# xxayt/MGSV

Measured on AMD Instinct MI355X. Metric: video-music pairs/s fwd+bwd at B=64 (full training step); sub-objects: retrieval sim-matrix GB/s, eval forward pairs/s, higher is better.
Workload: dtype bf16; 1 GPU; BASELINE.json configs[2]: B=64/GPU, T_v=30, T_a=512, D=512, train mode (dropout on), f32 master weights + Adam, f32 gradient accumulation; global_batch=64, launch=tape

## Files before the change

include/made_hip.h:

```cpp
#ifndef MADE_HIP_H
#define MADE_HIP_H

#include <stdint.h>

#ifdef __cplusplus
extern "C" {
#endif

#define MADE_ABI_VERSION 8

enum MadeDtype { MADE_F32 = 0, MADE_BF16 = 1 };

enum MadeAct {
    MADE_ACT_NONE = 0,
    MADE_ACT_RELU = 1,
    MADE_ACT_GELU = 2,
    MADE_ACT_QUICKGELU = 3,
    MADE_ACT_SIGMOID = 4
};

enum MadeGate {
    MADE_GATE_NONE = 0,
    MADE_GATE_RELU_OUT = 1,
    MADE_GATE_GELU_Z = 2,
// ... 425 lines not shown
                       float* dgamma, float* dbeta, int64_t rows, int64_t D, float eps, const float* row_skip, void* stream);

int made_pool_bwd(const float* mean, const float* dvec, const float* mask,
                  const void* in1, int32_t in1_dtype, int64_t in1_bs, int64_t in1_ld,
                  const void* in2, int32_t in2_dtype, int64_t in2_bs, int64_t in2_ld,
                  void* out, int32_t out_dtype, int64_t out_bs, int64_t out_ld,
                  int64_t B, int64_t T, int64_t D, float eps, void* stream);

int made_l2norm_bwd(const void* x, int32_t x_dtype, int64_t ldx, const float* dy, int64_t lddy, int64_t dy_rows_per,
                    float* dx, int64_t lddx, int32_t accumulate, void* dx_alt, int32_t alt_dtype, int64_t lddxa,
                    int64_t rows, int64_t D, float eps, void* stream);

int made_clip_loss_bwd(const float* sims, int64_t ld, int64_t n, const float* logit_scale, float weight,
                       const float* upstream, float* lse_ws, float* dsims, float* dsims_t, int32_t accumulate,
                       float* d_logit_scale, const float* row_exclude, void* stream);

int made_xpool_tail_bwd(const void* y, int32_t y_dtype, int64_t ldy, const float* gamma, const float* beta,
                        const float* video, int64_t ld_video, const float* dsims, int64_t ld_dsims,
                        void* dy, int32_t dy_dtype, int64_t lddy, void* dy_drop, const MadeDropout* drop,
                        float* dgamma, float* dbeta, float* dvideo, int64_t ld_dvideo,
                        const float* dpool, int64_t ld_dpool, float dpool_scale,
                        int64_t Nm, int64_t Nv, int64_t D, float eps, void* stream);

int made_softmax_bwd(const float* S, int64_t ld_s, const float* dP, int64_t ld_dp, const float* mask, int64_t rows_per_mask,
                     const float* extra, float scale, const MadeDropout* drop,
                     void* Pd, void* dS, void* dSt, int32_t out_dtype, int64_t ldo, int64_t ldt,
                     int64_t out_batch_stride, int64_t t_batch_stride,
                     int64_t rows, int64_t rows_per_batch, int64_t L, void* stream);

int made_head_bias(void* x, int32_t x_dtype, int64_t ldx, const float* s, const float* bias, int64_t rows, int64_t H, int64_t hd,
                   void* stream);
int made_head_bias_bwd(const void* dy, int32_t dtype, int64_t ld, const float* s, const float* bias, float* dbias, float* ds,
                       int64_t rows, int64_t H, int64_t hd, void* stream);

int made_layernorm_bwd2(const void* xa, const float* gamma_a, int64_t ldxa, const void* xb, const float* gamma_b, int64_t ldxb,
                        const void* dy, int64_t lddy, const void* add, int64_t ld_add, void* dx, int64_t lddx,
                        void* dx_drop, int64_t lddxd, const MadeDropout* drop, int64_t drop_ld, int32_t dtype,
                        float* dgamma_a, float* dbeta_a, float* dgamma_b, float* dbeta_b, int64_t rows, int64_t D, float eps,
                        void* stream);

int made_gate_rows(const void* x, int32_t x_dtype, int64_t ldx, const void* G, int32_t g_dtype, int64_t ldg, int32_t gate,
                   float scale, const MadeDropout* drop, int64_t drop_ld, int64_t drop_col_div, void* out, int32_t out_dtype, int64_t ldo,
                   const float* row_skip, int64_t rows, int64_t cols, void* stream);
int made_add3(void* out, int32_t out_dtype, const void* a, int32_t a_dtype, const void* b, int32_t b_dtype,
              const void* c, int32_t c_dtype, int64_t n, int64_t b_mod, void* stream);
int made_colsum(const void* x, int32_t dtype, int64_t ld, int64_t rows, int64_t cols, float* out, void* stream);

int made_posbn_relu_fwd(const void* x, int32_t x_dtype, int64_t ldx, const float* weight, const float* bias,
                        float* running_mean, float* running_var, float momentum, float eps, int32_t batch_stats,
                        float* save_mean, float* save_rstd, void* y, int32_t y_dtype, int64_t ldy,
                        int64_t B, int64_t T, int64_t F, void* stream);
int made_posbn_relu_bwd(const void* x, int32_t x_dtype, int64_t ldx, const void* y, int32_t y_dtype, int64_t ldy,
                        const void* dy, int32_t dy_dtype, int64_t lddy, const float* weight, const float* save_mean,
                        const float* save_rstd, int32_t batch_stats, void* dx, int32_t dx_dtype, int64_t lddx,
                        float* dweight, float* dbias, int64_t B, int64_t T, int64_t F, void* stream);

int made_set_criterion_bwd(const float* pred_logits, const float* pred_spans, const float* targets,
                           const int64_t* pred_idx, const int64_t* tgt_idx, const int32_t* count,
                           const float* proj_queries, const float* vid_sum, const float* empty_weight,
                           int64_t n_layers, int64_t B, int64_t Q, int64_t G, int64_t Dc, int32_t fg_label,
                           float temperature, const float* weights, const float* upstream,
                           float* d_logits, float* d_spans, int64_t ld_out, int32_t through_sigmoid,
                           float* d_proj_queries, float* d_vid_sum, void* stream);

#define MADE_ADAM_MAX_GROUPS 4
#define MADE_ADAM_NORM_BLOCKS 1024
typedef struct MadeAdamGroup { int64_t begin, end; float lr; float max_norm; } MadeAdamGroup;
int made_adam_step(float* param, const float* grad, float* exp_avg, float* exp_avg_sq, int64_t n,
                   const MadeAdamGroup* groups, int32_t n_groups, float beta1, float beta2, float eps, int64_t step,
                   float grad_scale, float* norm_ws, void* stream);

typedef struct MadeAdamDeviceState { int64_t step; float lr[MADE_ADAM_MAX_GROUPS]; float bc1, bc2_sqrt; } MadeAdamDeviceState;
int made_adam_step_device(float* param, const float* grad, float* exp_avg, float* exp_avg_sq, int64_t n,
                          const MadeAdamGroup* groups, int32_t n_groups, float beta1, float beta2, float eps,
                          MadeAdamDeviceState* state_device, int32_t advance_state, float grad_scale, float* norm_ws, void* stream);

typedef struct MadeRepackDesc {
    const float* src; void* w; void* wt;
    int64_t rows, cols, wt_ld, tile_begin;
    int32_t dtype; int32_t _pad;
} MadeRepackDesc;
int made_repack(const MadeRepackDesc* descs_device, int32_t n_desc, int64_t total_tiles, void* stream);


int made_recall_ranks(const float* sims, int64_t ld, const int32_t* group_id, const int32_t* gt_group, int64_t Nv, int64_t Nm,
                      int64_t n_groups, int32_t* rank_out, int32_t* top1_out, void* stream);

int made_span_iou(const float* pred_logits, const float* pred_spans, const float* gt_moment, const float* m_duration,
                  int64_t N, int64_t Q, int32_t fg_label, float max_m_duration, float* iou_out, float* pred_out, void* stream);

int made_concat_cols(const float* a, int64_t cols_a, const float* c, int64_t cols_c, float* out, int64_t rows, void* stream);


int made_pooled_cosine(const float* anchor, int64_t lda, const void* pooled, int32_t pooled_dtype, float* out, int64_t sa, int64_t sp,
                       int64_t A, int64_t P, int64_t D, void* stream);
int made_scale_exp(const float* x, const float* logit_scale, float* out, int64_t n, void* stream);
int made_span_convert(const float* in, float* out, int64_t N, int32_t mode, void* stream);
int made_span_pairwise(const float* spans1, const float* spans2, float* iou, float* uni, float* giou, float* inter_over_2,
                       int64_t N, int64_t M, void* stream);
int made_span_iou_se(const float* pred_se, const float* gt_moment, const float* m_duration, int64_t N, float max_m_duration,
                     int32_t clamp_to_max, int32_t discounted, float* iou_out, void* stream);


int64_t made_topk_groups_ws_bytes(int64_t Nv, int64_t Nm, int64_t K);
int made_topk_groups(const float* sims, int64_t ld, const int32_t* group_id, int64_t Nv, int64_t Nm, int64_t n_groups,
                     int64_t K, int32_t* idx_out, float* score_out, void* ws, int64_t ws_bytes, void* stream);

int made_gather_pairs(const int32_t* vi, const int32_t* mi, int64_t P, int64_t Nv, int64_t Nm,
                      const void* v_tok, int64_t v_tok_stride, const float* v_mask, int64_t v_mask_stride,
                      const float* v_vec, int64_t v_vec_stride,
                      const void* m_tok, int64_t m_tok_stride, const float* m_mask, int64_t m_mask_stride,
                      const float* m_vec, int64_t m_vec_stride, int64_t Tv, int64_t Ta, int64_t D, int32_t dtype,
                      void* frame_out, int64_t frame_out_stride, void* seg_out, int64_t seg_out_stride,
                      float* fmask_out, float* smask_out, float* video_out, float* music_out, void* stream);


#define MADE_FRAMES_MAX (1 << 20)

typedef struct MadeFrameDesc {
    int64_t offset;
    int64_t coef;
    int32_t H, W;
    int32_t kh, kv;
} MadeFrameDesc;

int made_frames_preprocess(const uint8_t* frames, int64_t frames_bytes, const MadeFrameDesc* desc, int64_t n_frames,
                           const int32_t* coef, int64_t n_coef, void* patches, int32_t patch_dtype, int64_t ld_patch,
                           uint8_t* crop_out, void* stream);


#define MADE_AUDIO_TRACKS_MAX (1 << 16)
#define MADE_AUDIO_SEGS_MAX (1 << 20)
#define MADE_RESAMPLE_TILE 1024
#define MADE_RESAMPLE_SLAB 12288
#define MADE_AUDIO_ROWS 1024
#define MADE_AUDIO_MELS 128

typedef struct MadeResampleDesc {
    int64_t offset;
    int64_t n;
    int64_t taps;
    int32_t o, m;
    int32_t width;
    int32_t _pad;
} MadeResampleDesc;

int made_audio_resample(const float* pcm, int64_t pcm_len, const MadeResampleDesc* desc, int64_t n_tracks, const float* taps,
                        int64_t n_taps, float* out, int64_t out_len, void* stream);

typedef struct MadeAudioSegDesc {
    int64_t first;
    int64_t count;
} MadeAudioSegDesc;

int made_audio_fbank(const float* pcm, int64_t pcm_len, const MadeAudioSegDesc* segs, int64_t n_segs, const float* window,
                     const float* twiddle, const float* mel, int32_t mel_ld, float* spec, void* stream);

int made_ast_patches(const float* spec, int64_t n_segs, void* patches, int32_t patch_dtype, int64_t ld_patch, void* stream);

#ifdef __cplusplus
}
#endif
#endif
```

mgsv_amd/_lib.py:

```python
from __future__ import annotations

import ctypes as C
import os

_HERE = os.path.dirname(os.path.abspath(__file__))


def variant_env(name: str, default: str = "") -> str:
    if os.environ.get("MADE_DEBUG_VARIANTS", "0") in ("", "0"):
        return default
    return os.environ.get(name, default)


LIB_PATH = os.environ.get("MADE_LIB_PATH") or os.path.join(_HERE, "libmade_hip.so")
ABI_VERSION = 8

F32, BF16 = 0, 1
ACT_NONE, ACT_RELU, ACT_GELU, ACT_QUICKGELU, ACT_SIGMOID = 0, 1, 2, 3, 4
GATE_NONE, GATE_RELU_OUT, GATE_GELU_Z, GATE_QUICKGELU_Z, GATE_SIGMOID_OUT = 0, 1, 2, 3, 4

vp, i64, i32, f32 = C.c_void_p, C.c_int64, C.c_int32, C.c_float

WIDE_PLAN_HEAD, WIDE_PLAN_SAMPLE, WIDE_PLAN_SLOT, WIDE_PLAN_SLOT_BITS = 4, 4, 16, 8

# ... 80 lines not shown
                ("B", i64), ("H", i64), ("Lq", i64), ("Lk", i64),
                ("q_bs", i64), ("ldq", i64), ("k_bs", i64), ("ldk", i64), ("v_bs", i64), ("ldv", i64), ("o_bs", i64), ("ldo", i64),
                ("do_bs", i64), ("lddo", i64), ("dq_bs", i64), ("lddq", i64), ("dk_bs", i64), ("lddk", i64), ("dv_bs", i64), ("lddv", i64),
                ("key_mask", vp), ("q_skip_mask", vp), ("scale", f32), ("_pad", i32), ("drop", MadeDropout),
                ("batch_order", vp), ("keep_bits", vp), ("ld_bits", i64)]


class MadeXpoolFusedArgs(C.Structure):
    _fields_ = [("Q", vp), ("ldq", i64), ("K", vp), ("U", vp), ("k_bs", i64), ("ldk", i64), ("u_bs", i64), ("ldu", i64),
                ("key_mask", vp), ("ln2_g", vp), ("ln2_b", vp), ("Wl", vp), ("ldw", i64), ("bl", vp), ("ln3_g", vp), ("ln3_b", vp),
                ("vn", vp), ("ldvn", i64), ("sims", vp), ("ld_sims", i64),
                ("Nv", i64), ("Nm", i64), ("S", i64), ("D", i64), ("scale", f32), ("eps", f32), ("ws", vp), ("prepare_ws", i32), ("_pad", i32)]


class MadeXpoolAttnArgs(C.Structure):
    _fields_ = [("Q", vp), ("ldq", i64), ("K", vp), ("U", vp), ("k_bs", i64), ("ldk", i64), ("u_bs", i64), ("ldu", i64),
                ("key_mask", vp), ("out", vp), ("ldo", i64), ("Nv", i64), ("Nm", i64), ("S", i64), ("D", i64),
                ("scale", f32), ("eps", f32), ("normalize", i32), ("_pad", i32), ("ws", vp)]


class MadeXpoolSimsArgs(C.Structure):
    _fields_ = [("Q", vp), ("ldq", i64), ("K", vp), ("UU", vp), ("k_bs", i64), ("ldk", i64), ("u_bs", i64), ("ldu", i64),
                ("key_mask", vp), ("av", vp), ("bv", vp), ("ln3_g", vp), ("ln3_b", vp), ("vn", vp), ("ldvn", i64),
                ("sims", vp), ("ld_sims", i64), ("Nv", i64), ("Nm", i64), ("S", i64), ("D", i64),
                ("scale", f32), ("eps", f32), ("ws", vp), ("prepare_ws", i32), ("_pad", i32)]


class MadeXpoolInbatchArgs(C.Structure):
    _fields_ = [("Q", vp), ("ldq", i64), ("K", vp), ("U", vp), ("k_bs", i64), ("ldk", i64), ("u_bs", i64), ("ldu", i64),
                ("key_mask", vp), ("out", vp), ("out_dtype", i32), ("_pad", i32), ("o_bs", i64), ("ldo", i64),
                ("Nv", i64), ("Nm", i64), ("S", i64), ("D", i64), ("scale", f32), ("_pad2", i32), ("ws", vp)]


class MadeWideAttnArgs(C.Structure):
    _fields_ = [("Q", vp), ("K", vp), ("Kadd", vp), ("V", vp), ("O", vp), ("key_mask", vp),
                ("dtype", i32), ("o_dtype", i32),
                ("B", i64), ("NQ1", i64), ("NQ2", i64), ("L", i64), ("D", i64),
                ("q_bs", i64), ("q_s1", i64), ("q_s2", i64), ("k_bs", i64), ("ldk", i64), ("kadd_bs", i64), ("ldkadd", i64),
                ("v_bs", i64), ("ldv", i64), ("o_bs", i64), ("o_s1", i64), ("o_s2", i64),
                ("scale", f32), ("_pad", i32),
                ("n_split", i64), ("part_o", vp), ("part_ml", vp), ("drop", MadeDropout), ("sum_out", vp),
                ("lse_out", vp)]


class MadeWideAttnBwdArgs(C.Structure):
    _fields_ = ([(k, vp) for k in ("Q", "dO", "O", "K", "V", "key_mask", "lse", "ssum", "extra", "dattc")] + [("ld_dattc", i64), ("vbias", vp), ("hd", i64),
                ("Pd", vp), ("dS", vp), ("p_bs", i64), ("ld_p", i64), ("dQ", vp), ("dq_bs", i64), ("ld_dq", i64)] +
                [(k, i64) for k in ("B", "NQ", "L", "D", "q_bs", "ld_q", "do_bs", "ld_do", "o_bs", "ld_o", "k_bs", "ldk", "v_bs", "ldv")] +
                [("scale", f32), ("_pad", i32), ("n_split", i64), ("part_dq", vp), ("drop", MadeDropout)])


class MadeGemmTNArgs(C.Structure):
    _fields_ = [("A", vp), ("B", vp), ("C", vp), ("ab_dtype", i32), ("c_dtype", i32),
                ("M", i64), ("N", i64), ("K", i64), ("lda", i64), ("ldb", i64), ("ldc", i64),
                ("batch1", i64), ("batch2", i64),
                ("a_zs1", i64), ("a_zs2", i64), ("b_zs1", i64), ("b_zs2", i64), ("c_zs1", i64), ("c_zs2", i64),
                ("row_mask", vp), ("mask_zs1", i64), ("mask_zs2", i64),
                ("alpha", f32), ("accumulate", i32), ("split_m", i64),
                ("colsum", vp), ("colsum_zs1", i64), ("colsum_zs2", i64), ("row_group_valid", vp),
                ("row_index", vp), ("n_rows", vp)]


class MadeGemmTNProblem(C.Structure):
    _fields_ = [("A", vp), ("B", vp), ("C", vp), ("colsum", vp), ("N", i64), ("K", i64), ("lda", i64), ("ldb", i64), ("ldc", i64)]


class MadeGemmTNGroup(C.Structure):
    _fields_ = [("n_problems", i32), ("alpha", f32), ("M", i64), ("split_m", i64), ("row_index", vp), ("n_rows", vp),
                ("p", MadeGemmTNProblem * 8), ("tile_end", i32 * 8), ("tile_size", i32), ("_pad", i32),
                ("workspace", vp), ("workspace_bytes", i64)]


class MadeAdamGroup(C.Structure):
    _fields_ = [("begin", i64), ("end", i64), ("lr", f32), ("max_norm", f32)]


class MadeAdamDeviceState(C.Structure):
    _fields_ = [("step", i64), ("lr", f32 * 4), ("bc1", f32), ("bc2_sqrt", f32)]


class MadeRepackDesc(C.Structure):
    _fields_ = [("src", vp), ("w", vp), ("wt", vp), ("rows", i64), ("cols", i64), ("wt_ld", i64), ("tile_begin", i64),
                ("dtype", i32), ("_pad", i32)]


class MadeFrameDesc(C.Structure):
    _fields_ = [("offset", i64), ("coef", i64), ("H", i32), ("W", i32), ("kh", i32), ("kv", i32)]


class MadeResampleDesc(C.Structure):
    _fields_ = [("offset", i64), ("n", i64), ("taps", i64), ("o", i32), ("m", i32), ("width", i32), ("_pad", i32)]


class MadeAudioSegDesc(C.Structure):
    _fields_ = [("first", i64), ("count", i64)]


SIGNATURES = {
    "made_abi_version": (C.c_int, []),
    "made_set_f32_products": (C.c_int, [C.c_int]),
    "made_get_f32_products": (C.c_int, []),
    "made_last_error": (C.c_char_p, []),
    "made_device_info": (C.c_int, [C.c_char_p, C.c_int, C.POINTER(C.c_int), C.POINTER(C.c_int)]),
    "made_tape_begin": (C.c_int, []),
    "made_tape_end": (C.c_int, [C.POINTER(C.c_uint64)]),
    "made_tape_replay": (C.c_int, [C.c_uint64]),
    "made_tape_free": (C.c_int, [C.c_uint64]),
    "made_tape_interleave": (C.c_int, [C.c_uint64, i32]),
    "made_tape_count": (C.c_int, [C.c_uint64, C.POINTER(i64), C.POINTER(i64), C.POINTER(i64)]),
    "made_tape_replay_range": (C.c_int, [C.c_uint64, i64, i64]),
    "made_tape_op": (C.c_int, [C.c_uint64, i64, C.POINTER(i32), C.POINTER(C.c_uint64), C.POINTER(C.c_uint64), C.POINTER(C.c_uint32)]),
    "made_stream_wait": (C.c_int, [vp, vp]),
    "made_tape_event": (C.c_int, [i32, i32, vp]),
    "made_tape_callback": (C.c_int, [C.CFUNCTYPE(C.c_int, vp), vp]),
    "made_memset_async": (C.c_int, [vp, i32, i64, vp]),
    "made_copy_async": (C.c_int, [vp, vp, i64, vp]),
    "made_store_words": (C.c_int, [vp, vp, i32, vp]),
    "made_linear": (C.c_int, [C.POINTER(MadeLinearArgs), vp]),
    "made_splitk_finish": (C.c_int, [C.POINTER(MadeFinishArgs), vp]),
    "made_dec_stage": (C.c_int, [C.POINTER(MadeDecStageArgs), vp]),
    "made_dec_stage_bwd": (C.c_int, [C.POINTER(MadeDecStageBwdArgs), vp]),
    "made_attention": (C.c_int, [C.POINTER(MadeAttnArgs), vp]),
    "made_attention_wide": (C.c_int, [C.POINTER(MadeWideAttnArgs), vp]),
    "made_attention_wide_bwd": (C.c_int, [C.POINTER(MadeWideAttnBwdArgs), vp]),
    "made_wide_slice_plan": (C.c_int, [vp, i64, i64, i32, i32, vp, vp, i64, vp]),
    "made_attention_wide_planned": (C.c_int, [C.POINTER(MadeWideAttnArgs), vp, i32, vp]),
    "made_attention_wide_bwd_planned": (C.c_int, [C.POINTER(MadeWideAttnBwdArgs), vp, i32, vp]),
    "made_layernorm": (C.c_int, [vp, i32, i64, i64, i64, vp, vp, vp, i32, i64, i64, i64, f32, vp, vp]),
    "made_layernorm_add": (C.c_int, [vp, i32, i64, vp, vp, vp, i32, i64, vp, i32, i64, vp, i64, i64, i64, f32, vp, vp]),
    "made_cast_mask_rows": (C.c_int, [vp, i64, vp, vp, i32, i64, i64, i64, vp]),
    "made_pack_music_records": (C.c_int, [vp, i32, i64, vp, i64, vp, i64, vp, i32, i64, i64, i64, i64, i64, vp]),
    "made_masked_mean": (C.c_int, [vp, i32, i64, i64, vp, vp, i64, i64, i64, vp]),
    "made_l2norm_rows": (C.c_int, [vp, i32, i64, vp, vp, i32, i64, i64, i64, f32, vp]),
    "made_sine_pe": (C.c_int, [vp, vp, vp, i32, i64, i64, i64, vp]),
    "made_masked_softmax": (C.c_int, [vp, i64, vp, i64, vp, i32, i64, i64, i64, i64, i64, f32, vp]),
    "made_xpool_tail": (C.c_int, [vp, i32, i64, vp, vp, vp, i64, vp, vp, i64, i64, i64, i64, f32, vp]),
    "made_clip_loss": (C.c_int, [vp, i64, i64, vp, f32, i32, vp, vp, vp]),
    "made_hungarian_match": (C.c_int, [vp, vp, vp, i64, i64, i64, i64, i32, f32, f32, f32, vp, i32, vp, vp, vp, vp, vp]),
    "made_attention_bwd": (C.c_int, [C.POINTER(MadeAttnBwdArgs), vp]),
    "made_layernorm_bwd": (C.c_int, [vp, i32, i64, i64, i64, vp, vp, i32, i64, vp, i32, i64, vp, i32, i64, vp, i64,
                                     C.POINTER(MadeDropout), i64, vp, vp, i64, i64, f32, vp, vp]),
    "made_layernorm_bwd2": (C.c_int, [vp, vp, i64, vp, vp, i64, vp, i64, vp, i64, vp, i64, vp, i64, C.POINTER(MadeDropout), i64, i32,
                                      vp, vp, vp, vp, i64, i64, f32, vp]),
    "made_pool_bwd": (C.c_int, [vp, vp, vp, vp, i32, i64, i64, vp, i32, i64, i64, vp, i32, i64, i64, i64, i64, i64, f32, vp]),
    "made_l2norm_bwd": (C.c_int, [vp, i32, i64, vp, i64, i64, vp, i64, i32, vp, i32, i64, i64, i64, f32, vp]),
    "made_clip_loss_bwd": (C.c_int, [vp, i64, i64, vp, f32, vp, vp, vp, vp, i32, vp, vp, vp]),
    "made_xpool_tail_bwd": (C.c_int, [vp, i32, i64, vp, vp, vp, i64, vp, i64, vp, i32, i64, vp, C.POINTER(MadeDropout),
                                      vp, vp, vp, i64, vp, i64, f32, i64, i64, i64, f32, vp]),
    "made_softmax_bwd": (C.c_int, [vp, i64, vp, i64, vp, i64, vp, f32, C.POINTER(MadeDropout), vp, vp, vp, i32, i64, i64,
                                   i64, i64, i64, i64, i64, vp]),
    "made_head_bias": (C.c_int, [vp, i32, i64, vp, vp, i64, i64, i64, vp]),
    "made_head_bias_bwd": (C.c_int, [vp, i32, i64, vp, vp, vp, vp, i64, i64, i64, vp]),
    "made_add3": (C.c_int, [vp, i32, vp, i32, vp, i32, vp, i32, i64, i64, vp]),
    "made_colsum": (C.c_int, [vp, i32, i64, i64, i64, vp, vp]),
    "made_posbn_relu_fwd": (C.c_int, [vp, i32, i64, vp, vp, vp, vp, C.c_float, C.c_float, i32, vp, vp, vp, i32, i64, i64, i64, i64, vp]),
    "made_posbn_relu_bwd": (C.c_int, [vp, i32, i64, vp, i32, i64, vp, i32, i64, vp, vp, vp, i32, vp, i32, i64, vp, vp, i64, i64, i64, vp]),
    "made_set_criterion_bwd": (C.c_int, [vp, vp, vp, vp, vp, vp, vp, vp, vp, i64, i64, i64, i64, i64, i32, f32, vp, vp,
                                         vp, vp, i64, i32, vp, vp, vp]),
    "made_adam_step": (C.c_int, [vp, vp, vp, vp, i64, C.POINTER(MadeAdamGroup), i32, f32, f32, f32, i64, f32, vp, vp]),
    "made_adam_step_device": (C.c_int, [vp, vp, vp, vp, i64, C.POINTER(MadeAdamGroup), i32, f32, f32, f32, vp, i32, f32, vp, vp]),
    "made_repack": (C.c_int, [vp, i32, i64, vp]),
    "made_row_groups": (C.c_int, [vp, i64, vp, vp]),
    "made_row_index": (C.c_int, [vp, i64, vp, vp, vp]),
    "made_linear_variant": (C.c_int, [C.POINTER(MadeLinearArgs)]),
    "made_row_affine": (C.c_int, [vp, i32, i64, vp, vp, i64, i32, vp, i32, i64, i64, i64, vp]),
    "made_gate_rows": (C.c_int, [vp, i32, i64, vp, i32, i64, i32, f32, vp, i64, i64, vp, i32, i64, vp, i64, i64, vp]),
    "made_xpool_fused": (C.c_int, [C.POINTER(MadeXpoolFusedArgs), vp]),
    "made_xpool_attention": (C.c_int, [C.POINTER(MadeXpoolAttnArgs), vp]),
    "made_xpool_sims": (C.c_int, [C.POINTER(MadeXpoolSimsArgs), vp]),
    "made_xpool_sims_ws_bytes": (C.c_int64, [i64, i64, i64]),
    "made_xpool_inbatch": (C.c_int, [C.POINTER(MadeXpoolInbatchArgs), vp]),
    "made_xpool_inbatch_ws_bytes": (C.c_int64, [i64, i64]),
    "made_batch_order": (C.c_int, [vp, i64, i64, vp, vp]),
    "made_recall_ranks": (C.c_int, [vp, i64, vp, vp, i64, i64, i64, vp, vp, vp]),
    "made_span_iou": (C.c_int, [vp, vp, vp, vp, i64, i64, i32, f32, vp, vp, vp]),
    "made_gemm_tn": (C.c_int, [C.POINTER(MadeGemmTNArgs), vp]),
    "made_gemm_tn_grouped": (C.c_int, [C.POINTER(MadeGemmTNGroup), vp]),
    "made_gemm_tn_grouped_workspace": (i64, [C.POINTER(MadeGemmTNGroup)]),
    "made_concat_cols": (C.c_int, [vp, i64, vp, i64, vp, i64, vp]),
    "made_pooled_cosine": (C.c_int, [vp, i64, vp, i32, vp, i64, i64, i64, i64, i64, vp]),
    "made_scale_exp": (C.c_int, [vp, vp, vp, i64, vp]),
    "made_span_convert": (C.c_int, [vp, vp, i64, i32, vp]),
    "made_span_pairwise": (C.c_int, [vp, vp, vp, vp, vp, vp, i64, i64, vp]),
    "made_span_iou_se": (C.c_int, [vp, vp, vp, i64, f32, i32, i32, vp, vp]),
    "made_set_criterion": (C.c_int, [vp, vp, vp, vp, vp, vp, vp, vp, vp, i64, i64, i64, i64, i64, i32, f32, vp, vp, vp, vp]),
    "made_topk_groups_ws_bytes": (C.c_int64, [i64, i64, i64]),
    "made_topk_groups": (C.c_int, [vp, i64, vp, i64, i64, i64, i64, vp, vp, vp, i64, vp]),
    "made_gather_pairs": (C.c_int, [vp, vp, i64, i64, i64, vp, i64, vp, i64, vp, i64, vp, i64, vp, i64, vp, i64, i64, i64, i64, i32,
                                    vp, i64, vp, i64, vp, vp, vp, vp, vp]),
    "made_frames_preprocess": (C.c_int, [vp, i64, vp, i64, vp, i64, vp, i32, i64, vp, vp]),
    "made_audio_resample": (C.c_int, [vp, i64, vp, i64, vp, i64, vp, i64, vp]),
    "made_audio_fbank": (C.c_int, [vp, i64, vp, i64, vp, vp, vp, i32, vp, vp]),
    "made_ast_patches": (C.c_int, [vp, i64, vp, i32, i64, vp]),
}

_lib = None


class MadeError(RuntimeError):
    pass


def lib() -> C.CDLL:
    global _lib
    if _lib is None:
        if not os.path.isfile(LIB_PATH):
            raise MadeError(f"{LIB_PATH} not found: build the HIP library first (make -C mgsv_amd/csrc); "
                            "the MaDe hot path has no CPU fallback")
        l = C.CDLL(LIB_PATH)
        for name, (res, args) in SIGNATURES.items():
            fn = getattr(l, name)
            fn.restype = res
            fn.argtypes = args
        if l.made_abi_version() != ABI_VERSION:
            raise MadeError(f"ABI version mismatch: {LIB_PATH} is version {l.made_abi_version()}, this binding was written for {ABI_VERSION} "
                            "(rebuild: make -C mgsv_amd/csrc)")
        _lib = l
    return _lib


def check(status: int, what: str = "") -> None:
    if status != 0:
        msg = lib().made_last_error().decode("utf-8", "replace")
        raise MadeError(f"{what or 'libmade_hip'} failed (status {status}): {msg}")


def device_info():
    l = lib()
    name = C.create_string_buffer(64)
    cu, is950 = C.c_int(0), C.c_int(0)
    check(l.made_device_info(name, 64, C.byref(cu), C.byref(is950)), "made_device_info")
    return name.value.decode(), cu.value, bool(is950.value)
```

mgsv_amd/csrc/attention_wide.hip:

```cpp
#include "common.h"

#include <type_traits>

namespace {

constexpr int WQ = 32;
constexpr int WKEY = 32;
constexpr int NTHREADS = 256;

template <typename TC> struct Frag;
template <> struct Frag<float>  { typedef f32x4  type; };
template <> struct Frag<bf16_t> { typedef bf16x8 type; };


template <typename TC, int D, bool DB, int NSL, bool X3 = false, bool PLAN = false>
__global__ __launch_bounds__(NTHREADS) void attention_wide_kernel(const MadeWideAttnArgs a, const int32_t* __restrict__ plan) {
    static_assert(!PLAN || (DB && sizeof(TC) == 2 && NSL == 4 && !X3), "the planned launch: LDS-DMA variant, one query tile");
    typedef typename Frag<TC>::type frag_t;
    constexpr int SZ = (int)sizeof(TC);
    constexpr bool IS_BF16 = SZ == 2;
    constexpr int PER16 = 16 / SZ;
    constexpr int DS = D / NSL;
    constexpr int WQB = WQ * (4 / NSL);
    constexpr bool DMA = IS_BF16 && DB;
    constexpr int K_ROW = DMA ? D * SZ : D * SZ + 16;
    constexpr int V_ROW = DMA ? D * SZ : D * SZ + (IS_BF16 ? 64 : 16);
    constexpr int CPR = D * SZ / 16;
    constexpr int NCH = WKEY * CPR / NTHREADS;
    static_assert(WKEY * CPR % NTHREADS == 0, "staging split");
    constexpr int NQF = DS * SZ / 32;
    constexpr int NDT = DS / 32;
    constexpr int KV_STAGE = WKEY * K_ROW + WKEY * V_ROW;
    constexpr int NSTAGE = DB ? 2 : 1;

    extern __shared__ __attribute__((aligned(16))) unsigned char lds[];
    float* lds_s = (float*)(lds + NSTAGE * KV_STAGE);
    float* lds_bias_all = lds_s + 4 * 1024;
    uint32_t* lds_mbits = (uint32_t*)(lds_bias_all + NSTAGE * 32);

    const int tid = threadIdx.x, lane = tid & 63, wave = tid >> 6;
    const int r = lane & 31, hh = lane >> 5;
    const int sl = wave % NSL, qt = wave / NSL;
    int32_t pl[MADE_WIDE_PLAN_SLOT] = {};
    if constexpr (PLAN) {
        const u32x4* sp = (const u32x4*)(plan + MADE_WIDE_PLAN_HEAD + MADE_WIDE_PLAN_SAMPLE * a.B + (int64_t)MADE_WIDE_PLAN_SLOT * blockIdx.x);
#pragma unroll
        for (int i = 0; i < 4; ++i) {
            const u32x4 v = sp[i];
            pl[4 * i] = (int32_t)v[0]; pl[4 * i + 1] = (int32_t)v[1]; pl[4 * i + 2] = (int32_t)v[2]; pl[4 * i + 3] = (int32_t)v[3];
        }
        if (pl[0] < 0 || pl[0] >= a.B || pl[3] < 0 || pl[3] >= a.n_split || pl[1] < 0 || pl[2] < 0 || (int64_t)(pl[1] + pl[2]) * WKEY >= a.L + WKEY ||
            pl[4] < 0 || pl[4] >= a.L) return;
    }
    const bool batch_fast = gridDim.x == (unsigned)a.B && (a.NQ1 * a.NQ2 + WQB - 1) / WQB != (int64_t)a.B;
    const int64_t b = PLAN ? (int64_t)pl[0] : (batch_fast ? blockIdx.x : blockIdx.y);
    const int64_t nq_total = a.NQ1 * a.NQ2;
    const int64_t nq0 = PLAN ? (int64_t)qt * WQ : (int64_t)(batch_fast ? blockIdx.y : blockIdx.x) * WQB + qt * WQ;

    const TC* Kg = (const TC*)a.K + b * a.k_bs;
    const TC* Ag = a.Kadd ? (const TC*)a.Kadd + b * a.kadd_bs : nullptr;
    const TC* Vg = (const TC*)a.V + b * a.v_bs;
    const float* maskg = a.key_mask ? a.key_mask + b * a.L : nullptr;

    frag_t qf[NQF];
    int64_t my_q = nq0 + r;
    {
        int64_t q = my_q < nq_total ? my_q : nq_total - 1;
        const TC* qp = (const TC*)a.Q + b * a.q_bs + (q / a.NQ2) * a.q_s1 + (q % a.NQ2) * a.q_s2 + sl * DS;
#pragma unroll
        for (int ks = 0; ks < NQF; ++ks) qf[ks] = *(const frag_t*)(qp + ks * 2 * PER16 + hh * PER16);
    }

    frag_t rk[NCH], rv[NCH];
    int64_t rkey0 = 0;
    auto load_tile = [&](int64_t key0) __attribute__((always_inline)) {
        rkey0 = key0;
#pragma unroll
        for (int i = 0; i < NCH; ++i) {
            int c = tid + i * NTHREADS;
            int row = c / CPR, cc = c % CPR;
            int64_t key = key0 + row;
            const int64_t kcl = key < a.L ? key : a.L - 1;
            rk[i] = *(const frag_t*)(Kg + kcl * a.ldk + cc * PER16);
// ... 366 lines not shown
#pragma unroll
                    for (int j = 0; j < 4; ++j) acc[i][j] += t[sp][i][j] * w;
            }
        }
    } else {
        float M = -INFINITY;
        for (int64_t s = 0; s < ns; ++s) M = fmaxf(M, a.part_ml[((b * ns + s) * nq_total + q) * 4]);
        Muse = (M == -INFINITY) ? 0.f : M;
        for (int64_t s = 0; s < ns; ++s) {
            const int64_t prow = (b * ns + s) * nq_total + q;
            const float w = expf(a.part_ml[prow * 4] - Muse);
            Lsum += a.part_ml[prow * 4 + 1] * w;
            Dsum += a.part_ml[prow * 4 + 2] * w;
#pragma unroll
            for (int i = 0; i < 2; ++i) {
                int c = (i * 64 + lane) * 4;
                if (c < D) {
                    f32x4 tt = *(const f32x4*)(a.part_o + prow * D + c);
#pragma unroll
                    for (int j = 0; j < 4; ++j) acc[i][j] += tt[j] * w;
                }
            }
        }
    }
    const float inv = 1.f / Lsum;
    if (a.sum_out && lane == 0) a.sum_out[b * nq_total + q] = Dsum * inv;
    if (a.lse_out && lane == 0) a.lse_out[b * nq_total + q] = Muse + logf(Lsum);
    const int64_t obase = b * a.o_bs + (q / a.NQ2) * a.o_s1 + (q % a.NQ2) * a.o_s2;
#pragma unroll
    for (int i = 0; i < 2; ++i) {
        int c = (i * 64 + lane) * 4;
        if (c < D) {
            if (a.o_dtype == MADE_F32) {
                f32x4 pk; pk[0] = acc[i][0] * inv; pk[1] = acc[i][1] * inv; pk[2] = acc[i][2] * inv; pk[3] = acc[i][3] * inv;
                *(f32x4*)((float*)a.O + obase + c) = pk;
            } else {
                bf16x4 pk; pk[0] = (bf16_t)(acc[i][0] * inv); pk[1] = (bf16_t)(acc[i][1] * inv);
                pk[2] = (bf16_t)(acc[i][2] * inv); pk[3] = (bf16_t)(acc[i][3] * inv);
                *(bf16x4*)((bf16_t*)a.O + obase + c) = pk;
            }
        }
    }
}

template <typename TC, int D, bool DB, int NSL>
int launch_wide(const MadeWideAttnArgs& a, hipStream_t st) {
    constexpr int SZ = (int)sizeof(TC);
    constexpr bool DMA = SZ == 2 && DB;
    constexpr int K_ROW = DMA ? D * SZ : D * SZ + 16, V_ROW = DMA ? D * SZ : D * SZ + (SZ == 2 ? 64 : 16);
    constexpr int NSTAGE = DB ? 2 : 1;
    constexpr size_t kBase = (size_t)NSTAGE * (WKEY * K_ROW + WKEY * V_ROW) + 4 * 1024 * 4 + NSTAGE * 32 * 4;
    constexpr size_t kCap = kBase + 8192 < 160 * 1024 ? kBase + 8192 : 160 * 1024;
    const size_t lds_bytes = kBase + (size_t)((a.L + 63) / 64 * 2 + 2) * 4;
    if (lds_bytes > kCap) {
        made_set_error("made_attention_wide: L=%lld keys: the mask bit row does not fit in LDS beside the K / V stages", (long long)a.L);
        return MADE_ERR_UNSUPPORTED;
    }
    static bool attr_done = false;
    if (!attr_done) {
        hipError_t e = hipFuncSetAttribute((const void*)attention_wide_kernel<TC, D, DB, NSL>, hipFuncAttributeMaxDynamicSharedMemorySize, (int)kCap);
        if (e == hipSuccess && SZ == 4)
            e = hipFuncSetAttribute((const void*)attention_wide_kernel<TC, D, DB, NSL, SZ == 4>, hipFuncAttributeMaxDynamicSharedMemorySize, (int)kCap);
        if (e != hipSuccess) {
            made_set_error("made_attention_wide: cannot reserve %zu bytes of LDS: %s", kCap, hipGetErrorString(e));
            return MADE_ERR_HIP;
        }
        attr_done = true;
    }
    const int64_t nq = a.NQ1 * a.NQ2;
    const int64_t nsplit = a.n_split > 1 ? a.n_split : 1;
    constexpr int WQB = WQ * (4 / NSL);
    const int64_t qtiles = (nq + WQB - 1) / WQB;
    const bool batch_fast = qtiles > 1 && qtiles <= 8 && qtiles != a.B;
    dim3 grid((unsigned)(batch_fast ? a.B : qtiles), (unsigned)(batch_fast ? qtiles : a.B), (unsigned)nsplit), block(NTHREADS);
    if (SZ == 4 && g_made_f32_products) hipLaunchKernelGGL((attention_wide_kernel<TC, D, DB, NSL, SZ == 4>), grid, block, lds_bytes, st, a, (const int32_t*)nullptr);
    else hipLaunchKernelGGL((attention_wide_kernel<TC, D, DB, NSL>), grid, block, lds_bytes, st, a, (const int32_t*)nullptr);
    int rc = made_check_launch("made_attention_wide");
    if (rc != MADE_OK || nsplit == 1) return rc;
    const int64_t rows = a.B * nq;
    hipLaunchKernelGGL(attention_wide_combine_kernel, dim3((unsigned)((rows + 3) / 4)), dim3(NTHREADS), 0, st, a);
    return made_check_launch("made_attention_wide(combine)");
}

constexpr int PLAN_T = 1024;
__global__ __launch_bounds__(PLAN_T) void wide_slice_plan_kernel(const float* __restrict__ mask, int B, int L, int n_slots, int max_slices,
                                                                 const int32_t* __restrict__ order, int32_t* __restrict__ plan) {
    __shared__ int32_t s_tiles[PLAN_T], s_first[PLAN_T], s_ord[PLAN_T];
    __shared__ int32_t s_cap;
    extern __shared__ __attribute__((aligned(16))) unsigned char lds[];
    uint32_t* s_bits = (uint32_t*)lds;
    const int tid = threadIdx.x, lane = tid & 63, wave = tid >> 6;
    const int nch = (L + 63) / 64, wpr = 2 * nch;
    if (tid == 0) s_cap = 0x7fffffff;
    for (int b = wave; b < B; b += PLAN_T / 64) {
        const float* m = mask + (int64_t)b * L;
        int last = -1, first = -1;
        for (int c0 = 0; c0 < nch; c0 += 8) {
            float v[8];
#pragma unroll
            for (int j = 0; j < 8; ++j) {
                const int i = (c0 + j) * 64 + lane;
                v[j] = m[i < L ? i : L - 1];
            }
#pragma unroll
            for (int j = 0; j < 8; ++j) {
                const int i = (c0 + j) * 64 + lane;
                const unsigned long long bal = __ballot(i < L && v[j] != 0.f);
                if (c0 + j < nch) {
                    if (lane == 0) { s_bits[b * wpr + 2 * (c0 + j)] = (uint32_t)bal; s_bits[b * wpr + 2 * (c0 + j) + 1] = (uint32_t)(bal >> 32); }
                    if (bal) {
                        last = (c0 + j) * 64 + 63 - __clzll(bal);
                        if (first < 0) first = (c0 + j) * 64 + __ffsll(bal) - 1;
                    }
                }
            }
        }
        if (lane == 0) { s_tiles[b] = (last + 1 + 31) / 32; s_first[b] = first < 0 ? 0 : first; }
    }
    if (tid < B) {
        const int o = order ? order[tid] : tid;
        s_ord[tid] = o >= 0 && o < B ? o : tid;
    }
    __syncthreads();
    int tmax = 1;
    for (int b = 0; b < B; ++b) tmax = max(tmax, s_tiles[b]);
    for (int c = tid + 1; c <= tmax; c += PLAN_T) {
        const int n = made_wide_slice_count(s_tiles, 1, B, c, max_slices);
        if (n >= 0 && n <= n_slots) atomicMin(&s_cap, c);
    }
    __syncthreads();
    const int cap = s_cap <= tmax ? s_cap : tmax;
    int used = 0;
    for (int r = 0; r < B; ++r) { const int t = s_tiles[s_ord[r]]; used += t > cap ? (t + cap - 1) / cap : 1; }
    if (tid == 0) { plan[0] = cap; plan[1] = used; plan[2] = n_slots; plan[3] = max_slices; }
    int32_t* slots = plan + MADE_WIDE_PLAN_HEAD + MADE_WIDE_PLAN_SAMPLE * B;
    if (tid < B) {
        int slot0 = 0;
        for (int r = 0; r < tid; ++r) { const int t = s_tiles[s_ord[r]]; slot0 += t > cap ? (t + cap - 1) / cap : 1; }
        const int b = s_ord[tid], t = s_tiles[b], fv = s_first[b];
        const int n = t > cap ? (t + cap - 1) / cap : 1;
        int32_t* sm = plan + MADE_WIDE_PLAN_HEAD + MADE_WIDE_PLAN_SAMPLE * b;
        sm[0] = t; sm[1] = slot0; sm[2] = n; sm[3] = fv;
        for (int s = 0; s < n && slot0 + s < n_slots; ++s) {
            int32_t* sp = slots + (int64_t)MADE_WIDE_PLAN_SLOT * (slot0 + s);
            const int t0 = made_wide_slice_first(t, n, s), tn = made_wide_slice_len(t, n, s);
            sp[0] = b; sp[1] = t0; sp[2] = tn; sp[3] = s; sp[4] = fv; sp[5] = n; sp[6] = t; sp[7] = 0;
            for (int i = 0; i < MADE_WIDE_PLAN_SLOT_BITS; ++i) sp[8 + i] = i < tn ? (int32_t)s_bits[b * wpr + t0 + i] : 0;
        }
    }
    for (int w = used + tid; w < n_slots; w += PLAN_T) {
        int32_t* sp = slots + (int64_t)MADE_WIDE_PLAN_SLOT * w;
        sp[0] = -1;
        for (int i = 1; i < MADE_WIDE_PLAN_SLOT; ++i) sp[i] = 0;
    }
}

__global__ __launch_bounds__(NTHREADS) void attention_wide_combine_planned_kernel(const MadeWideAttnArgs a, const int32_t* __restrict__ plan) {
    constexpr int MAXS = 8;
    const int lane = threadIdx.x & 63;
    const int64_t nq_total = a.NQ1 * a.NQ2;
    const int64_t row = (int64_t)blockIdx.x * (NTHREADS / 64) + (threadIdx.x >> 6);
    if (row >= a.B * nq_total) return;
    const int64_t b = row / nq_total, q = row % nq_total;
    const int D = (int)a.D;
    const int cap = (int)a.n_split;
    int ns = plan[MADE_WIDE_PLAN_HEAD + MADE_WIDE_PLAN_SAMPLE * b + 2];
    ns = ns < 1 ? 1 : (ns > MAXS ? MAXS : ns);
    ns = ns > cap ? cap : ns;
    float Lsum = 0.f, Dsum = 0.f;
    f32x4 acc[2];
#pragma unroll
    for (int i = 0; i < 2; ++i) { acc[i][0] = acc[i][1] = acc[i][2] = acc[i][3] = 0.f; }
    f32x4 t[MAXS][2];
    float ml[MAXS][3];
#pragma unroll
    for (int sp = 0; sp < MAXS; ++sp) {
        const int64_t pr = (b * cap + (sp < ns ? sp : ns - 1)) * nq_total + q;
        ml[sp][0] = a.part_ml[pr * 4]; ml[sp][1] = a.part_ml[pr * 4 + 1]; ml[sp][2] = a.part_ml[pr * 4 + 2];
#pragma unroll
        for (int i = 0; i < 2; ++i) {
            const int c = (i * 64 + lane) * 4;
            t[sp][i] = *(const f32x4*)(a.part_o + pr * D + (c < D ? c : 0));
        }
    }
    float M = -INFINITY;
#pragma unroll
    for (int sp = 0; sp < MAXS; ++sp) if (sp < ns) M = fmaxf(M, ml[sp][0]);
    const float Muse = (M == -INFINITY) ? 0.f : M;
#pragma unroll
    for (int sp = 0; sp < MAXS; ++sp) {
        if (sp < ns) {
            const float w = expf(ml[sp][0] - Muse);
            Lsum += ml[sp][1] * w;
            Dsum += ml[sp][2] * w;
#pragma unroll
            for (int i = 0; i < 2; ++i)
#pragma unroll
                for (int j = 0; j < 4; ++j) acc[i][j] += t[sp][i][j] * w;
        }
    }
    const float inv = 1.f / Lsum;
    if (a.sum_out && lane == 0) a.sum_out[b * nq_total + q] = Dsum * inv;
    if (a.lse_out && lane == 0) a.lse_out[b * nq_total + q] = Muse + logf(Lsum);
    const int64_t obase = b * a.o_bs + (q / a.NQ2) * a.o_s1 + (q % a.NQ2) * a.o_s2;
#pragma unroll
    for (int i = 0; i < 2; ++i) {
        int c = (i * 64 + lane) * 4;
        if (c < D) {
            if (a.o_dtype == MADE_F32) {
                f32x4 pk; pk[0] = acc[i][0] * inv; pk[1] = acc[i][1] * inv; pk[2] = acc[i][2] * inv; pk[3] = acc[i][3] * inv;
                *(f32x4*)((float*)a.O + obase + c) = pk;
            } else {
                bf16x4 pk; pk[0] = (bf16_t)(acc[i][0] * inv); pk[1] = (bf16_t)(acc[i][1] * inv);
                pk[2] = (bf16_t)(acc[i][2] * inv); pk[3] = (bf16_t)(acc[i][3] * inv);
                *(bf16x4*)((bf16_t*)a.O + obase + c) = pk;
            }
        }
    }
}

template <int D>
int launch_wide_planned(const MadeWideAttnArgs& a, const int32_t* plan, int n_slots, hipStream_t st) {
    constexpr size_t kBase = (size_t)2 * (WKEY * D * 2 + WKEY * D * 2) + 4 * 1024 * 4 + 2 * 32 * 4;
    constexpr size_t kCap = kBase + 8192 < 160 * 1024 ? kBase + 8192 : 160 * 1024;
    const size_t lds_bytes = kBase + (size_t)((a.L + 63) / 64 * 2 + 2) * 4;
    if (lds_bytes > kCap) {
        made_set_error("made_attention_wide_planned: L=%lld keys: the mask bit row does not fit in LDS beside the K / V stages", (long long)a.L);
        return MADE_ERR_UNSUPPORTED;
    }
    static bool attr_done = false;
    if (!attr_done) {
        hipError_t e = hipFuncSetAttribute((const void*)attention_wide_kernel<bf16_t, D, true, 4, false, true>, hipFuncAttributeMaxDynamicSharedMemorySize, (int)kCap);
        if (e != hipSuccess) {
            made_set_error("made_attention_wide_planned: cannot reserve %zu bytes of LDS: %s", kCap, hipGetErrorString(e));
            return MADE_ERR_HIP;
        }
        attr_done = true;
// ... 86 lines not shown
```

mgsv_amd/csrc/gemm_tn.hip:

```cpp
#include "common.h"

namespace {

__device__ const float kOne = 1.f;

constexpr int TBN = 128, TBK = 128, TNT = 256;

template <typename TC> struct TnCfg;
template <> struct TnCfg<bf16_t> { static constexpr int BM = 64, ROW = 128 * 2 + 64, CPR = 16; typedef bf16x8 frag_t; };
template <> struct TnCfg<float>  { static constexpr int BM = 32, ROW = 128 * 4 + 128, CPR = 32; typedef f32x4 frag_t; };

template <typename TC, bool X3 = false>
__global__ __launch_bounds__(TNT) void gemm_tn_kernel(const MadeGemmTNArgs a) {
    typedef TnCfg<TC> Cfg;
    typedef typename Cfg::frag_t frag_t;
    constexpr int BM = Cfg::BM, ROW = Cfg::ROW, CPR = Cfg::CPR;
    constexpr int PER16 = 16 / (int)sizeof(TC);
    constexpr int NCH = BM * CPR / TNT;
    constexpr bool IS_BF16 = sizeof(TC) == 2;

    __shared__ __attribute__((aligned(16))) unsigned char lds[2 * BM * ROW];
    unsigned char* lds_a = lds;
    unsigned char* lds_b = lds + BM * ROW;

    const int tid = threadIdx.x, lane = tid & 63, wave = tid >> 6;
    const int r = lane & 31, hh = lane >> 5;
    const int wn = wave >> 1, wk = wave & 1;
    const int tiles_k = (int)((a.K + TBK - 1) / TBK);
    const int tile_n = blockIdx.x / tiles_k, tile_k = blockIdx.x % tiles_k;
    const int64_t n0 = (int64_t)tile_n * TBN, k0 = (int64_t)tile_k * TBK;
    const int64_t z = blockIdx.z, z1 = z / a.batch2, z2 = z % a.batch2;

    const TC* Ag = (const TC*)a.A + z1 * a.a_zs1 + z2 * a.a_zs2;
    const TC* Bg = (const TC*)a.B + z1 * a.b_zs1 + z2 * a.b_zs2;
    const float* maskg = a.row_mask ? a.row_mask + z1 * a.mask_zs1 + z2 * a.mask_zs2 : nullptr;

    int64_t Mv = a.M;
    if (a.n_rows) { const int64_t nv = *a.n_rows; Mv = nv < a.M ? nv : a.M; }
    const int64_t nslab = (Mv + BM - 1) / BM;
    const int64_t sstep = a.split_m;
    const int64_t s_begin = 0;
    const int64_t s_end = nslab > (int64_t)blockIdx.y ? (nslab - blockIdx.y + sstep - 1) / sstep : 0;
    if (s_begin >= s_end) return;
    auto gslab = [&](int64_t i) __attribute__((always_inline)) { return (int64_t)blockIdx.y + i * sstep; };

    uint64_t slab_bits = ~0ull;
    if (a.row_group_valid && (s_end - s_begin) <= 64 && a.batch1 * a.batch2 == 1) {
        const int64_t sl = lane < s_end ? gslab(lane) : nslab;
        bool any = false;
        if (lane < s_end) {
            constexpr int GP = BM / 32;
            const int64_t ngroups = (a.M + 31) / 32;
#pragma unroll
            for (int g = 0; g < GP; ++g) {
                const int64_t gi = sl * GP + g;
                any = any || (gi < ngroups && a.row_group_valid[gi] != 0.f);
            }
        }
        slab_bits = __ballot(any);
    }
    auto slab_live = [&](int64_t i) __attribute__((always_inline)) { return i >= 64 || ((slab_bits >> i) & 1ull) != 0; };

    frag_t ra[NCH], rb[NCH];
    int64_t prow[NCH];
    auto load_rows = [&](int64_t slab) __attribute__((always_inline)) {
#pragma unroll
        for (int i = 0; i < NCH; ++i) {
            const int c = tid + i * TNT;
            const int64_t m = slab * BM + c / CPR;
            const int64_t ml = m < Mv ? m : Mv - 1;
            prow[i] = a.row_index ? (int64_t)a.row_index[ml] : ml;
        }
    };
    float rmk[NCH];
    int64_t rslab = 0;
    const float* mrow = maskg ? maskg : &kOne;
    const int64_t mstride = maskg ? 1 : 0;
    auto load_slab = [&](int64_t slab) __attribute__((always_inline)) {
        rslab = slab;
#pragma unroll
        for (int i = 0; i < NCH; ++i) {
            const int c = tid + i * TNT;
            const int cc = c % CPR;
// ... 157 lines not shown
    }
    if (!active) return;
    const int64_t co = z1 * a.c_zs1 + z2 * a.c_zs2 + n * a.ldc + k;
    if (a.c_dtype == MADE_F32) {
        if (a.accumulate) unsafeAtomicAdd((float*)a.C + co, acc * a.alpha); else ((float*)a.C)[co] = acc * a.alpha;
    } else {
        ((bf16_t*)a.C)[co] = (bf16_t)(acc * a.alpha);
    }
    if (a.colsum && k == 0) unsafeAtomicAdd(a.colsum + z1 * a.colsum_zs1 + z2 * a.colsum_zs2 + n, cs * a.alpha);
}

}

int made_gemm_tn_fast(const MadeGemmTNArgs& a, hipStream_t st);

extern "C" int made_gemm_tn(const MadeGemmTNArgs* args, void* stream) {
    MADE_REQUIRE(args != nullptr, "made_gemm_tn: null args");
    MadeGemmTNArgs a = *args;
    MADE_REQUIRE(a.A && a.B && a.C, "made_gemm_tn: null tensor");
    MADE_REQUIRE(a.M >= 0 && a.N > 0 && a.K > 0, "made_gemm_tn: bad dims");
    MADE_REQUIRE(a.ab_dtype == MADE_F32 || a.ab_dtype == MADE_BF16, "made_gemm_tn: bad operand dtype %d", a.ab_dtype);
    MADE_REQUIRE(a.c_dtype == MADE_F32 || a.c_dtype == a.ab_dtype, "made_gemm_tn: C must be f32 or the operand dtype");
    if (a.batch1 <= 0) a.batch1 = 1;
    if (a.batch2 <= 0) a.batch2 = 1;
    if (a.split_m <= 0) a.split_m = 1;
    const int64_t nz = a.batch1 * a.batch2;
    MADE_REQUIRE(a.split_m == 1 || a.accumulate, "made_gemm_tn: split_m > 1 needs accumulate = 1 (partials are added atomically)");
    MADE_REQUIRE(!a.accumulate || a.c_dtype == MADE_F32, "made_gemm_tn: accumulation needs an f32 C");
    MADE_UNSUPPORTED(nz < 65536 && a.split_m < 65536, "made_gemm_tn: batch / split too large for the grid");
    MADE_REQUIRE(a.row_group_valid == nullptr || a.row_mask != nullptr, "made_gemm_tn: row_group_valid without row_mask");
    MADE_REQUIRE((a.row_index == nullptr) == (a.n_rows == nullptr), "made_gemm_tn: row_index and n_rows come together");
    MADE_UNSUPPORTED(a.row_index == nullptr || nz == 1, "made_gemm_tn: row gather is for unbatched calls");
    if (a.row_index) a.row_group_valid = nullptr;
    if (a.M == 0) return MADE_OK;
    hipStream_t st = (hipStream_t)stream;
    const int per16 = a.ab_dtype == MADE_F32 ? 4 : 8;
    const int64_t n_up = (a.N + per16 - 1) / per16 * per16, k_up = (a.K + per16 - 1) / per16 * per16;
    const bool aligned = a.lda % per16 == 0 && a.ldb % per16 == 0 && n_up <= a.lda && k_up <= a.ldb &&
                         a.a_zs1 % per16 == 0 && a.a_zs2 % per16 == 0 && a.b_zs1 % per16 == 0 && a.b_zs2 % per16 == 0 &&
                         ((uintptr_t)a.A % 16) == 0 && ((uintptr_t)a.B % 16) == 0;
    if (!aligned) {
        MADE_UNSUPPORTED(a.N * a.K <= (1 << 20), "made_gemm_tn: unaligned operands are only supported for small outputs");
        int sy = (int)a.split_m;
        if (!a.accumulate) sy = 1;
        dim3 grid((unsigned)((a.N * a.K + 255) / 256), (unsigned)sy, (unsigned)nz);
        hipLaunchKernelGGL(gemm_tn_small_kernel, grid, dim3(256), 0, st, a);
        return made_check_launch("made_gemm_tn(small)");
    }
    const int64_t tiles = ((a.N + TBN - 1) / TBN) * ((a.K + TBK - 1) / TBK);
    MADE_UNSUPPORTED(tiles < (1LL << 31), "made_gemm_tn: too many tiles");
    {
        const int rc = made_gemm_tn_fast(a, st);
        if (rc != 1) return rc;
    }
    dim3 grid((unsigned)tiles, (unsigned)a.split_m, (unsigned)nz);
    if (a.ab_dtype == MADE_BF16) hipLaunchKernelGGL(gemm_tn_kernel<bf16_t>, grid, dim3(TNT), 0, st, a);
    else if (g_made_f32_products) hipLaunchKernelGGL((gemm_tn_kernel<float, true>), grid, dim3(TNT), 0, st, a);
    else hipLaunchKernelGGL(gemm_tn_kernel<float>, grid, dim3(TNT), 0, st, a);
    return made_check_launch("made_gemm_tn");
}

namespace {
__global__ __launch_bounds__(256) void row_groups_kernel(const float* mask, int64_t M, float* out) {
    const int lane = threadIdx.x & 63;
    const int64_t g = ((int64_t)blockIdx.x * 256 + threadIdx.x) >> 5;
    const int64_t ngroups = (M + 31) / 32;
    const int64_t row = g * 32 + (lane & 31);
    const bool v = g < ngroups && row < M && mask[row] != 0.f;
    const uint64_t bal = __ballot(v);
    const uint32_t half = (lane >> 5) ? (uint32_t)(bal >> 32) : (uint32_t)bal;
    if ((lane & 31) == 0 && g < ngroups) out[g] = half != 0 ? 1.f : 0.f;
}
}

extern "C" int made_row_groups(const float* mask, int64_t M, float* out, void* stream) {
    MADE_REQUIRE(mask && out && M > 0, "made_row_groups: bad arguments");
    const int64_t ngroups = (M + 31) / 32;
    hipLaunchKernelGGL(row_groups_kernel, dim3((unsigned)((ngroups * 32 + 255) / 256)), dim3(256), 0, (hipStream_t)stream, mask, M, out);
    return made_check_launch("made_row_groups");
}

namespace {
__global__ __launch_bounds__(1024) void row_index_kernel(const float* mask, int64_t M, int32_t* row_index, int32_t* n_rows) {
    constexpr int NB = 16;
    __shared__ int wsum[16];
    __shared__ int wlast[16];
    const int lane = threadIdx.x & 63, wave = threadIdx.x >> 6;
    const int64_t per = ((M + 15) / 16 + 63) / 64 * 64;
    const int64_t b = (int64_t)wave * per, e = b + per < M ? b + per : M;
    uint64_t bal[NB];
    auto ballots = [&](int64_t i0) __attribute__((always_inline)) {
        float v[NB];
        const float* p = mask + i0 + lane;
        if (i0 + NB * 64 <= e) {
#pragma unroll
            for (int j = 0; j < NB; ++j) v[j] = p[j * 64];
        } else {
#pragma unroll
            for (int j = 0; j < NB; ++j) v[j] = i0 + j * 64 + lane < e ? p[j * 64] : 0.f;
        }
#pragma unroll
        for (int j = 0; j < NB; ++j) bal[j] = __ballot(v[j] != 0.f);
    };
    int cnt = 0, last = -1;
    for (int64_t i0 = b; i0 < e; i0 += NB * 64) {
        ballots(i0);
#pragma unroll
        for (int j = 0; j < NB; ++j) {
            cnt += __popcll(bal[j]);
            if (bal[j]) last = (int)(i0 + j * 64) + 63 - __clzll(bal[j]);
        }
    }
    if (lane == 0) { wsum[wave] = cnt; wlast[wave] = last; }
    __syncthreads();
    int base = 0, total = 0, lastv = 0;
    for (int w = 0; w < 16; ++w) {
        if (w < wave) base += wsum[w];
        total += wsum[w];
        if (wlast[w] >= 0) lastv = wlast[w];
    }
    for (int64_t i0 = b; i0 < e; i0 += NB * 64) {
        ballots(i0);
#pragma unroll
        for (int j = 0; j < NB; ++j) {
            if ((bal[j] >> lane) & 1ull) row_index[base + __popcll(bal[j] & ((1ull << lane) - 1ull))] = (int32_t)(i0 + j * 64 + lane);
            base += __popcll(bal[j]);
        }
    }
    if (threadIdx.x == 0) n_rows[0] = total;
    for (int64_t i = total + threadIdx.x; i < M; i += 1024) row_index[i] = lastv;
}

__global__ __launch_bounds__(1024) void batch_order_kernel(const float* mask, int B, int64_t T, int32_t* order) {
    __shared__ int len[8192];
    const int lane = threadIdx.x & 63, wave = threadIdx.x >> 6;
    for (int b0 = wave; b0 < B; b0 += 64) {
        int cnt[4] = {0, 0, 0, 0};
        for (int64_t i0 = 0; i0 < T; i0 += 512) {
            float v[4][8];
#pragma unroll
            for (int s4 = 0; s4 < 4; ++s4) {
                const int b = b0 + 16 * s4;
                const float* m = mask + (int64_t)(b < B ? b : B - 1) * T;
#pragma unroll
                for (int j = 0; j < 8; ++j) {
                    const int64_t i = i0 + j * 64 + lane;
                    v[s4][j] = i < T ? m[i] : 0.f;
                }
            }
#pragma unroll
            for (int s4 = 0; s4 < 4; ++s4)
#pragma unroll
                for (int j = 0; j < 8; ++j) cnt[s4] += __popcll(__ballot(v[s4][j] != 0.f));
        }
#pragma unroll
        for (int s4 = 0; s4 < 4; ++s4)
            if (lane == 0 && b0 + 16 * s4 < B) len[b0 + 16 * s4] = cnt[s4];
    }
    __syncthreads();
    for (int b = threadIdx.x; b < B; b += 1024) {
        const int mine = len[b];
        int rank = 0;
        for (int j = 0; j < B; ++j) {
            const int l = len[j];
            rank += (l > mine || (l == mine && j < b)) ? 1 : 0;
        }
        order[rank] = b;
    }
}
}

extern "C" int made_batch_order(const float* mask, int64_t B, int64_t T, int32_t* order, void* stream) {
    MADE_REQUIRE(mask && order && B > 0 && T > 0, "made_batch_order: bad arguments");
    MADE_UNSUPPORTED(B <= 8192, "made_batch_order: B=%lld exceeds the single-workgroup table (8192)", (long long)B);
    hipLaunchKernelGGL(batch_order_kernel, dim3(1), dim3(1024), 0, (hipStream_t)stream, mask, (int)B, T, order);
    return made_check_launch("made_batch_order");
}

extern "C" int made_row_index(const float* mask, int64_t M, int32_t* row_index, int32_t* n_rows, void* stream) {
    MADE_REQUIRE(mask && row_index && n_rows && M > 0, "made_row_index: bad arguments");
    MADE_UNSUPPORTED(M <= (1 << 22), "made_row_index: M=%lld too large for the single-workgroup scan", (long long)M);
    hipLaunchKernelGGL(row_index_kernel, dim3(1), dim3(1024), 0, (hipStream_t)stream, mask, M, row_index, n_rows);
    return made_check_launch("made_row_index");
}
```

mgsv_amd/csrc/optimizer.hip:

```cpp
#include "common.h"

namespace {

constexpr int OT = 256;

struct AdamArgs {
    float* param; const float* grad; float* m; float* v; int64_t n;
    MadeAdamGroup g[MADE_ADAM_MAX_GROUPS]; int n_groups;
    float beta1, beta2, eps, bc1, bc2_sqrt, grad_scale;
    float* norm_sq;
    const MadeAdamDeviceState* st;
};

__device__ __forceinline__ int group_of(const AdamArgs& a, int64_t i) {
    int gi = -1;
#pragma unroll
    for (int k = 0; k < MADE_ADAM_MAX_GROUPS; ++k)
        if (k < a.n_groups && i >= a.g[k].begin && i < a.g[k].end) gi = k;
    return gi;
}

__global__ __launch_bounds__(OT) void grad_norm_kernel(const AdamArgs a) {
    __shared__ float red[MADE_ADAM_MAX_GROUPS][OT / 64];
    float acc[MADE_ADAM_MAX_GROUPS];
#pragma unroll
    for (int k = 0; k < MADE_ADAM_MAX_GROUPS; ++k) acc[k] = 0.f;
    for (int64_t i = ((int64_t)blockIdx.x * OT + threadIdx.x) * 4; i < a.n; i += (int64_t)gridDim.x * OT * 4) {
        if (group_of(a, i) < 0 && group_of(a, i + 3) < 0) continue;
        const f32x4 g4 = *(const f32x4*)(a.grad + i);
#pragma unroll
        for (int j = 0; j < 4; ++j) {
            const int gi = group_of(a, i + j);
            const float g = g4[j] * a.grad_scale;
#pragma unroll
            for (int k = 0; k < MADE_ADAM_MAX_GROUPS; ++k) acc[k] += (gi == k) ? g * g : 0.f;
        }
    }
    const int lane = threadIdx.x & 63, wave = threadIdx.x >> 6;
#pragma unroll
    for (int k = 0; k < MADE_ADAM_MAX_GROUPS; ++k) {
        const float s = wave_sum(acc[k]);
        if (lane == 0) red[k][wave] = s;
    }
    __syncthreads();
    if (threadIdx.x < MADE_ADAM_MAX_GROUPS) {
        float s = 0.f;
        for (int w = 0; w < OT / 64; ++w) s += red[threadIdx.x][w];
        a.norm_sq[MADE_ADAM_MAX_GROUPS + (int64_t)blockIdx.x * MADE_ADAM_MAX_GROUPS + threadIdx.x] = s;
    }
}

__global__ __launch_bounds__(OT) void norm_finish_kernel(float* norm_ws, int nblocks, MadeAdamDeviceState* st, float beta1, float beta2, int advance) {
    __shared__ float red[OT];
    if (st && advance && threadIdx.x == 0) {
        const int64_t step = ++st->step;
        st->bc1 = (float)(1.0 - pow((double)beta1, (double)step));
        st->bc2_sqrt = (float)sqrt(1.0 - pow((double)beta2, (double)step));
    }
    for (int k = 0; k < MADE_ADAM_MAX_GROUPS; ++k) {
        float s = 0.f;
        for (int b = threadIdx.x; b < nblocks; b += OT) s += norm_ws[MADE_ADAM_MAX_GROUPS + (int64_t)b * MADE_ADAM_MAX_GROUPS + k];
        red[threadIdx.x] = s;
        __syncthreads();
        for (int o = OT / 2; o > 0; o >>= 1) {
            if (threadIdx.x < o) red[threadIdx.x] += red[threadIdx.x + o];
            __syncthreads();
        }
        if (threadIdx.x == 0) norm_ws[k] = red[0];
        __syncthreads();
    }
}

__global__ __launch_bounds__(OT) void adam_update_kernel(const AdamArgs a) {
    float coef[MADE_ADAM_MAX_GROUPS];
#pragma unroll
    for (int k = 0; k < MADE_ADAM_MAX_GROUPS; ++k) {
        coef[k] = 1.f;
        if (k < a.n_groups && a.g[k].max_norm > 0.f) {
            const float c = a.g[k].max_norm / (sqrtf(a.norm_sq[k]) + 1e-6f);
            coef[k] = c < 1.f ? c : 1.f;
        }
    }
    float lrs[MADE_ADAM_MAX_GROUPS];
#pragma unroll
    for (int k = 0; k < MADE_ADAM_MAX_GROUPS; ++k) lrs[k] = a.st ? a.st->lr[k] : a.g[k].lr;
    const float bc1 = a.st ? a.st->bc1 : a.bc1, bc2_sqrt = a.st ? a.st->bc2_sqrt : a.bc2_sqrt;
    for (int64_t i = ((int64_t)blockIdx.x * OT + threadIdx.x) * 4; i < a.n; i += (int64_t)gridDim.x * OT * 4) {
        const int g0 = group_of(a, i), g3 = group_of(a, i + 3);
        if (g0 < 0 && g3 < 0) continue;
        f32x4 g4 = *(const f32x4*)(a.grad + i), m4 = *(const f32x4*)(a.m + i), v4 = *(const f32x4*)(a.v + i), p4 = *(const f32x4*)(a.param + i);
#pragma unroll
        for (int j = 0; j < 4; ++j) {
            const int gi = group_of(a, i + j);
            if (gi < 0) continue;
            float cf = 1.f, lr = 0.f;
#pragma unroll
            for (int k = 0; k < MADE_ADAM_MAX_GROUPS; ++k)
                if (gi == k) { cf = coef[k]; lr = lrs[k]; }
            const float g = g4[j] * a.grad_scale * cf;
            m4[j] = a.beta1 * m4[j] + (1.f - a.beta1) * g;
            v4[j] = a.beta2 * v4[j] + (1.f - a.beta2) * g * g;
            const float denom = sqrtf(v4[j]) / bc2_sqrt + a.eps;
            p4[j] -= (lr / bc1) * (m4[j] / denom);
        }
        *(f32x4*)(a.m + i) = m4; *(f32x4*)(a.v + i) = v4; *(f32x4*)(a.param + i) = p4;
    }
}

constexpr int RPT = 64;
__global__ __launch_bounds__(OT) void repack_kernel(const MadeRepackDesc* descs, int n_desc) {
    __shared__ float tile[RPT][RPT + 1];
    __shared__ int s_desc;
    const int64_t t = blockIdx.x;
    for (int i = threadIdx.x; i < n_desc; i += OT) {
        const int64_t b = descs[i].tile_begin;
        const int64_t e = i + 1 < n_desc ? descs[i + 1].tile_begin : INT64_MAX;
        if (b <= t && t < e) s_desc = i;
    }
    __syncthreads();
    const MadeRepackDesc d = descs[s_desc];
    const int64_t local = t - d.tile_begin;
    const int64_t tc_n = (d.cols + RPT - 1) / RPT;
    const int64_t r0 = (local / tc_n) * RPT, c0 = (local % tc_n) * RPT;
    const int tx = threadIdx.x & 15, ty = threadIdx.x >> 4;
    const bool bf = d.dtype == MADE_BF16;
#pragma unroll
    for (int k = 0; k < RPT / 16; ++k) {
        const int rr = ty + 16 * k;
        const int64_t r = r0 + rr, c = c0 + 4 * tx;
        float v[4] = {0.f, 0.f, 0.f, 0.f};
        if (r < d.rows && c < d.cols) {
            const float* sp = d.src + r * d.cols + c;
            if (c + 4 <= d.cols && (((uintptr_t)sp & 15) == 0)) {
                const f32x4 q = *(const f32x4*)sp;
                v[0] = q[0]; v[1] = q[1]; v[2] = q[2]; v[3] = q[3];
            } else {
#pragma unroll
                for (int j = 0; j < 4; ++j) if (c + j < d.cols) v[j] = sp[j];
            }
            if (d.w) {
                if (bf && c + 4 <= d.cols && (((r * d.cols + c) & 3) == 0)) {
                    bf16x4 o; o[0] = (bf16_t)v[0]; o[1] = (bf16_t)v[1]; o[2] = (bf16_t)v[2]; o[3] = (bf16_t)v[3];
                    *(bf16x4*)((bf16_t*)d.w + r * d.cols + c) = o;
                } else {
#pragma unroll
                    for (int j = 0; j < 4; ++j) if (c + j < d.cols) store_from_f32(d.w, d.dtype, r * d.cols + c + j, v[j]);
                }
            }
        }
#pragma unroll
        for (int j = 0; j < 4; ++j) tile[rr][4 * tx + j] = v[j];
    }
    __syncthreads();
    if (d.wt) {
#pragma unroll
        for (int k = 0; k < RPT / 16; ++k) {
            const int cc = ty + 16 * k;
            const int64_t c = c0 + cc, r = r0 + 4 * tx;
            if (c < d.cols && r < d.rows) {
                float v[4];
#pragma unroll
                for (int j = 0; j < 4; ++j) v[j] = tile[4 * tx + j][cc];
                if (bf && r + 4 <= d.rows && (((c * d.wt_ld + r) & 3) == 0)) {
                    bf16x4 o; o[0] = (bf16_t)v[0]; o[1] = (bf16_t)v[1]; o[2] = (bf16_t)v[2]; o[3] = (bf16_t)v[3];
                    *(bf16x4*)((bf16_t*)d.wt + c * d.wt_ld + r) = o;
                } else {
#pragma unroll
                    for (int j = 0; j < 4; ++j) if (r + j < d.rows) store_from_f32(d.wt, d.dtype, c * d.wt_ld + r + j, v[j]);
                }
            }
        }
    }
}

}

static int adam_launch(float* param, const float* grad, float* exp_avg, float* exp_avg_sq, int64_t n, const MadeAdamGroup* groups,
                       int32_t n_groups, float beta1, float beta2, float eps, int64_t step, MadeAdamDeviceState* state_device, int advance,
                       float grad_scale, float* norm_ws, void* stream, const char* what) {
    AdamArgs a;
    a.param = param; a.grad = grad; a.m = exp_avg; a.v = exp_avg_sq; a.n = n; a.n_groups = n_groups;
    for (int k = 0; k < MADE_ADAM_MAX_GROUPS; ++k) {
        if (k < n_groups) a.g[k] = groups[k];
        else { a.g[k].begin = a.g[k].end = 0; a.g[k].lr = 0.f; a.g[k].max_norm = 0.f; }
    }
    a.beta1 = beta1; a.beta2 = beta2; a.eps = eps; a.grad_scale = grad_scale;
    a.bc1 = state_device ? 1.f : (float)(1.0 - pow((double)beta1, (double)step));
    a.bc2_sqrt = state_device ? 1.f : (float)sqrt(1.0 - pow((double)beta2, (double)step));
    a.norm_sq = norm_ws;
    a.st = state_device;
    hipStream_t st = (hipStream_t)stream;
    int64_t nb = (n / 4 + OT - 1) / OT;
    if (nb > MADE_ADAM_NORM_BLOCKS) nb = MADE_ADAM_NORM_BLOCKS;
    hipLaunchKernelGGL(grad_norm_kernel, dim3((unsigned)nb), dim3(OT), 0, st, a);
    hipLaunchKernelGGL(norm_finish_kernel, dim3(1), dim3(OT), 0, st, norm_ws, (int)nb, state_device, beta1, beta2, advance);
    hipLaunchKernelGGL(adam_update_kernel, dim3((unsigned)nb), dim3(OT), 0, st, a);
    return made_check_launch(what);
}

extern "C" int made_adam_step(float* param, const float* grad, float* exp_avg, float* exp_avg_sq, int64_t n,
                              const MadeAdamGroup* groups, int32_t n_groups, float beta1, float beta2, float eps, int64_t step,
                              float grad_scale, float* norm_ws, void* stream) {
    MADE_REQUIRE(param && grad && exp_avg && exp_avg_sq && groups && norm_ws, "made_adam_step: null pointer");
    MADE_REQUIRE(n_groups >= 1 && n_groups <= MADE_ADAM_MAX_GROUPS, "made_adam_step: n_groups=%d out of range", n_groups);
    MADE_REQUIRE(n > 0 && n % 4 == 0 && step >= 1, "made_adam_step: n must be a positive multiple of 4 and step >= 1");
    return adam_launch(param, grad, exp_avg, exp_avg_sq, n, groups, n_groups, beta1, beta2, eps, step, nullptr, 0, grad_scale, norm_ws, stream,
                       "made_adam_step");
}

extern "C" int made_adam_step_device(float* param, const float* grad, float* exp_avg, float* exp_avg_sq, int64_t n,
                                     const MadeAdamGroup* groups, int32_t n_groups, float beta1, float beta2, float eps,
                                     MadeAdamDeviceState* state_device, int32_t advance_state, float grad_scale, float* norm_ws, void* stream) {
    MADE_REQUIRE(param && grad && exp_avg && exp_avg_sq && groups && norm_ws && state_device, "made_adam_step_device: null pointer");
    MADE_REQUIRE(n_groups >= 1 && n_groups <= MADE_ADAM_MAX_GROUPS, "made_adam_step_device: n_groups=%d out of range", n_groups);
    MADE_REQUIRE(n > 0 && n % 4 == 0, "made_adam_step_device: n must be a positive multiple of 4");
    return adam_launch(param, grad, exp_avg, exp_avg_sq, n, groups, n_groups, beta1, beta2, eps, 0, state_device, advance_state != 0, grad_scale, norm_ws, stream,
                       "made_adam_step_device");
}

extern "C" int made_repack(const MadeRepackDesc* descs_device, int32_t n_desc, int64_t total_tiles, void* stream) {
    MADE_REQUIRE(descs_device != nullptr && n_desc >= 1 && total_tiles >= 1, "made_repack: bad arguments");
    MADE_UNSUPPORTED(total_tiles < (1LL << 31), "made_repack: too many tiles");
    hipLaunchKernelGGL(repack_kernel, dim3((unsigned)total_tiles), dim3(OT), 0, (hipStream_t)stream, descs_device, (int)n_desc);
    return made_check_launch("made_repack");
}
```

mgsv_amd/ops.py:

```python
from __future__ import annotations

import ctypes as C
import math
from dataclasses import dataclass
from typing import NamedTuple, Optional, Sequence

import torch

from . import _lib, tape as _tape
from ._lib import (ACT_GELU, ACT_NONE, ACT_QUICKGELU, ACT_RELU, ACT_SIGMOID, BF16, F32,
                   MadeAttnArgs, MadeDecStageArgs, MadeFinishArgs, MadeLinearArgs, MadeLinearSeg, MadeWideAttnArgs, check, lib)

Tensor = torch.Tensor


def dt_of(t: Tensor) -> int:
    if t.dtype == torch.float32:
        return F32
    if t.dtype == torch.bfloat16:
        return BF16
    raise TypeError(f"unsupported dtype {t.dtype}")


def torch_dtype(code: int):
# ... 139 lines not shown
        a.a2_replace = 1 if a2_replace else 0
    a.a_row_mask = _p(_f32(a_row_mask, "a_row_mask"))
    a.W, a.ldw = _p(W), W.stride(0)
    a.bias = _p(_f32(bias, "bias"))
    a.M, a.N, a.K = M, N, K
    a.batch, a.a_z_stride, a.w_z_stride = batch, a_z_stride, w_z_stride
    a.act = act
    if R is not None:
        assert R.dim() == 2 and R.stride(1) == 1
        a.R, a.r_dtype, a.ldr, a.r_row_mod = _p(R), dt_of(R), R.stride(0), r_row_mod
    a.out_row_mask = _p(_f32(out_row_mask, "out_row_mask"))
    a.tile_skip_mask = _p(_f32(tile_skip_mask, "tile_skip_mask"))
    if gate:
        assert G is not None and G.dim() == 2 and G.stride(1) == 1
        a.G, a.g_dtype, a.gate, a.ldg, a.gate_scale = _p(G), dt_of(G), gate, G.stride(0), float(gate_scale)
    if Zout is not None:
        assert Zout.dim() == 2 and Zout.stride(1) == 1
        a.Zout, a.z_dtype, a.ldz = _p(Zout), dt_of(Zout), Zout.stride(0)
    if drop is not None and drop[2] > 0.0:
        set_drop(a.drop, drop)
        a.drop_ld = N if drop_ld is None else drop_ld
        a.drop_col_div = int(drop_col_div)
    if rows is not None:
        a.row_index, a.n_rows = _p(rows[0]), _p(rows[1])
    if bias_row_scale is not None:
        assert tuple(bias_row_scale.shape) == (M, batch)
        a.bias_row_scale, a.bias_z_stride = _p(_f32(bias_row_scale, "bias_row_scale")), bias_z_stride
    if segs is None:
        if out is None:
            out = torch.empty((M, N) if batch == 1 else (batch, M, N), device=A.device,
                              dtype=out_dtype or W.dtype)
        segs = [Seg(out=out, out_z_stride=(out.stride(0) if (batch > 1 and out.dim() == 3) else 0))]
    a.nseg = len(segs)
    for i, s in enumerate(segs):
        sg = a.seg[i]
        sg.col_begin, sg.out, sg.out_dtype = s.col_begin, _p(s.out), dt_of(s.out)
        sg.transposed = 1 if s.transposed else 0
        sg.ldo = s.ldo if s.ldo is not None else s.out.stride(-2)
        sg.rows_per_batch, sg.out_batch_stride, sg.out_z_stride = s.rows_per_batch, s.out_batch_stride, s.out_z_stride
        sg.use_a2 = 1 if s.use_a2 else 0
    esz = 4 if a.w_dtype == F32 else 2
    kind = "linear_" + ("f32" if a.w_dtype == F32 else ("bf16" if a.a_dtype == BF16 else "f32in_bf16"))
    if _timer is not None and kind == "linear_bf16":
        kind = LINEAR_VARIANTS[lib().made_linear_variant(C.byref(a))]
    elif _timer is not None and kind == "linear_f32" and lib().made_linear_variant(C.byref(a)) >= 11:
        kind = LINEAR_VARIANTS[lib().made_linear_variant(C.byref(a))]
    flops = 2.0 * M * N * K * batch
    nbytes = batch * (M * K * (4 if a.a_dtype == F32 else 2) + N * K * esz + M * N * esz)
    desc = f"M={M} N={N} K={K} z={batch} nseg={len(segs)} a2={int(A2 is not None)} R={int(R is not None)} act={act} tr={int(any(s_.transposed for s_ in segs))}"
    if LINEAR_LOG is not None:
        LINEAR_LOG.append((LINEAR_VARIANTS.get(lib().made_linear_variant(C.byref(a)), "?") if kind in ("linear_bf16", "linear_f32") else kind, M, N, K, batch,
                           f"nseg={len(segs)} a2={int(A2 is not None)}/{int(bool(a2_replace))} R={None if R is None else str(R.dtype)[6:]}/{r_row_mod} act={act} gate={gate} "
                           f"G={None if G is None else str(G.dtype)[6:]} Z={None if Zout is None else str(Zout.dtype)[6:]} "
                           f"drop={0 if drop is None else drop[2]}/{drop_col_div} rows={int(rows is not None)} orm={int(out_row_mask is not None)} "
                           f"arm={int(a_row_mask is not None)} out={str(segs[0].out.dtype)[6:]} rpb={segs[0].rows_per_batch} tr={int(any(s_.transposed for s_ in segs))}"))
    _timed(kind, flops, nbytes, lambda: check(lib().made_linear(C.byref(a), _stream()), "made_linear"),
           ("rows", rows[1], M) if rows is not None else ((desc, tile_skip_mask, 128) if tile_skip_mask is not None else desc))
    return segs[0].out


def row_index(mask: Tensor, out=None):
    m = mask.reshape(-1)
    M = m.numel()
    if out is not None:
        idx, n = out
        assert idx.dtype == torch.int32 and idx.numel() >= M and n.dtype == torch.int32
    else:
        idx = torch.empty(M, device=m.device, dtype=torch.int32)
        n = torch.empty(1, device=m.device, dtype=torch.int32)
    check(lib().made_row_index(_p(_f32(m, "mask")), M, _p(idx), _p(n), _stream()), "made_row_index")
    return idx, n


def batch_order(mask: Tensor, out: Optional[Tensor] = None) -> Tensor:
    assert mask.dim() == 2
    B, T = mask.shape
    if out is None:
        out = torch.empty(B, device=mask.device, dtype=torch.int32)
    assert out.dtype == torch.int32 and out.numel() == B
    check(lib().made_batch_order(_p(_f32(mask.contiguous(), "mask")), B, T, _p(out), _stream()), "made_batch_order")
    return out


def linear_splitk(A: Tensor, W: Tensor, bias: Optional[Tensor], ws: Tensor, split_k: int, *, A2: Optional[Tensor] = None,
                  a2_row_mod: int = 0, act: int = ACT_NONE, R: Optional[Tensor] = None, r_row_mod: int = 0,
                  out: Optional[Tensor] = None, ln1=None, ln1_out: Optional[Tensor] = None, ln2=None,
                  ln2_out: Optional[Tensor] = None, eps: float = 1e-5) -> None:
    assert A.dim() == 2 and W.dim() == 2 and A.stride(1) == 1 and W.stride(1) == 1
    M, K = A.shape
    N = W.shape[0]
    assert ws.dtype == torch.float32 and ws.is_contiguous() and ws.numel() >= split_k * M * N
    a = MadeLinearArgs()
    a.A, a.a_dtype, a.w_dtype, a.lda = _p(A), dt_of(A), dt_of(W), A.stride(0)
    use_a2 = A2 is not None
    if use_a2:
        a.A2, a.lda2, a.a2_row_mod = _p(A2), A2.stride(0), a2_row_mod
    a.W, a.ldw = _p(W), W.stride(0)
    a.M, a.N, a.K = M, N, K
    a.batch = 1
    a.nseg, a.split_k, a.split_ws = 1, max(split_k, 2), _p(ws)
    sg = a.seg[0]
    sg.col_begin, sg.out, sg.out_dtype, sg.ldo, sg.use_a2 = 0, _p(ws), F32, N, 1 if use_a2 else 0
    esz = 4 if a.w_dtype == F32 else 2
    _timed("linear_splitk_f32" if a.w_dtype == F32 else "linear_kernel<bf16,bf16>", 2.0 * M * N * K, M * K * esz + N * K * esz + M * N * 4 * a.split_k,
           lambda: check(lib().made_linear(C.byref(a), _stream()), "made_linear(split_k)"), f"M={M} N={N} K={K} split={a.split_k}")
    splitk_finish(ws, a.split_k, M, N, bias, act=act, R=R, r_row_mod=r_row_mod, out=out, ln1=ln1, ln1_out=ln1_out, ln2=ln2, ln2_out=ln2_out,
                  eps=eps)


def splitk_finish(ws: Tensor, split_k: int, M: int, N: int, bias: Optional[Tensor], *, act: int = ACT_NONE, R: Optional[Tensor] = None,
                  r_row_mod: int = 0, out: Optional[Tensor] = None, ln1=None, ln1_out: Optional[Tensor] = None, ln2=None,
                  ln2_out: Optional[Tensor] = None, eps: float = 1e-5) -> None:
    assert ws.dtype == torch.float32 and ws.is_contiguous() and ws.numel() >= split_k * M * N
    f = MadeFinishArgs()
    f.ws, f.split_k, f.M, f.N = _p(ws), split_k, M, N
    f.bias, f.act = _p(_f32(bias, "bias")), act
    if R is not None:
        assert R.dim() == 2 and R.stride(1) == 1
        f.R, f.r_dtype, f.ldr, f.r_row_mod = _p(R), dt_of(R), R.stride(0), r_row_mod
    if out is not None:
        f.out, f.out_dtype, f.ldo = _p(out), dt_of(out), out.stride(0)
    if ln1 is not None:
        f.ln1_g, f.ln1_b = _p(_f32(ln1[0], "ln1.g")), _p(_f32(ln1[1], "ln1.b"))
        if ln1_out is not None:
            f.ln1_out, f.ln1_dtype, f.ln1_ld = _p(ln1_out), dt_of(ln1_out), ln1_out.stride(0)
    if ln2 is not None:
        f.ln2_g, f.ln2_b = _p(_f32(ln2[0], "ln2.g")), _p(_f32(ln2[1], "ln2.b"))
        f.ln2_out, f.ln2_dtype, f.ln2_ld = _p(ln2_out), dt_of(ln2_out), ln2_out.stride(0)
    f.eps = eps
    check(lib().made_splitk_finish(C.byref(f), _stream()), "made_splitk_finish")


def dec_stage(Zin: Tensor, W: Tensor, bias: Optional[Tensor], out: Tensor, *, ln=None, ln2=None, x2_out: Optional[Tensor] = None,
              add: Optional[Tensor] = None, x_out: Optional[Tensor] = None, R: Optional[Tensor] = None, res_from_x: bool = False,
              act: int = ACT_NONE, eps: float = 1e-5, a_out: Optional[Tensor] = None, drop=None, drop_ld: Optional[int] = None,
              drop_col_div: int = 1) -> Tensor:
    assert Zin.dim() == 2 and W.dim() == 2 and out.dim() == 2 and W.dtype == torch.bfloat16
    assert Zin.stride(1) == 1 and W.stride(1) == 1 and out.stride(1) == 1
    M, K = Zin.shape
    N = W.shape[0]
    assert W.shape[1] == K and tuple(out.shape) == (M, N)
    a = MadeDecStageArgs()
    a.Zin, a.ldz, a.zin_dtype = _p(Zin), Zin.stride(0), dt_of(Zin)
    if ln is not None:
        a.ln_g, a.ln_b = _p(_f32(ln[0], "ln.g")), _p(_f32(ln[1], "ln.b"))
    if ln2 is not None:
        assert x2_out is not None and x2_out.dtype == torch.bfloat16 and x2_out.stride(1) == 1
        a.ln2_g, a.ln2_b, a.x2_out, a.ldx2 = _p(_f32(ln2[0], "ln2.g")), _p(_f32(ln2[1], "ln2.b")), _p(x2_out), x2_out.stride(0)
    if add is not None:
        assert add.dim() == 2 and add.dtype == torch.bfloat16 and add.is_contiguous() and add.shape[1] == K
        a.add, a.add_row_mod = _p(add), add.shape[0]
    if x_out is not None:
        assert x_out.dtype == torch.bfloat16 and x_out.stride(1) == 1 and tuple(x_out.shape) == (M, K)
        a.x_out, a.ldx = _p(x_out), x_out.stride(0)
    if a_out is not None:
        assert a_out.dtype == torch.bfloat16 and a_out.stride(1) == 1 and tuple(a_out.shape) == (M, K) and Zin.dtype == torch.bfloat16
        a.a_out, a.lda_out = _p(a_out), a_out.stride(0)
    if drop is not None and drop[2] > 0.0:
        assert Zin.dtype == torch.bfloat16
        set_drop(a.drop, drop)
        a.drop_ld = N if drop_ld is None else drop_ld
        a.drop_col_div = int(drop_col_div)
    a.W, a.ldw, a.bias = _p(W), W.stride(0), _p(_f32(bias, "bias"))
    if R is not None:
        assert R.dtype == torch.bfloat16 and R.stride(1) == 1 and tuple(R.shape) == (M, N)
        a.R, a.ldr = _p(R), R.stride(0)
# ... 532 lines not shown
```

mgsv_amd/trainer.py:

```python
from __future__ import annotations

import math
import os
from typing import Dict, List, Optional, Tuple

import numpy as np
import torch

from . import _lib, dropout as dr, ops, ops_train as tr, tape as _tape
from .config import MadeConfig
from .engine import MadeEngine
from .ops import Seg, round_up

WIDE_SLICES = 8

Tensor = torch.Tensor
XA = "video_guided_to_music_pooling_cross_transformer"


HEAD_PAD = 64


class MadeTrainer(MadeEngine):
    def __init__(self, cfg: MadeConfig, state_dict: Dict[str, object], device="cuda:0", dtype: str = "f32"):
        if dtype == "f32x3":
            raise ValueError('dtype "f32x3" (split-bf16 products) is an inference mode: it meets the forward\'s 1e-4 gate, its gradients do not meet '
                             'the f32 training path\'s (measured up to 3e-2 relative per tensor); train in "f32" or "bf16"')
        super().__init__(cfg, state_dict, device, dtype)
        self._check_train_supported()
        self._init_master(state_dict)
        self.repack()
        self._tws: Dict[tuple, Dict[str, Tensor]] = {}
        self.generation = 0
        self.seed = 0
        self.training_dropout = True
        self._bits = dtype == "bf16" and _lib.variant_env("MADE_ATTN_BITS", "1") != "0"

    def _check_train_supported(self):
        c = self.cfg
        bad = []
        if "concat" not in c.mml_fusion and "CA" not in c.mml_fusion:
            bad.append(f"mml_fusion={c.mml_fusion}")
        if c.moment_query_type not in ("video", "music", "zero", "random", "xpool"):
            bad.append(f"moment_query_type={c.moment_query_type}")
        if c.moment_query_type == "xpool" and "music" not in c.vmr_fusion:
            bad.append("moment_query_type=xpool without the music-pooling tower (the reference fails there too)")
        if c.vmr_fusion not in ("XA-music", "XA-video", "XA-video-music", "XA-music-video"):
            bad.append(f"vmr_fusion={c.vmr_fusion}")
        if c.vmr_loss == "dual_single_feature_fuse" and "music" not in c.vmr_fusion:
            bad.append("vmr_loss=dual_single_feature_fuse without the music-pooling tower (the reference fails there too)")
        if c.agg_module != "mlp" and c.with_cls_token and (c.video_transformer_depth < 1 or c.audio_transformer_depth < 1):
            bad.append("with_cls_token without a temporal block")
        if "detr" not in c.mml_localization and "regression" not in c.mml_localization:
            bad.append(f"mml_localization={c.mml_localization}")
        if c.audio_short_cut and c.contrastive_align_loss and c.contrastive_hdim != c.D:
            bad.append("audio_short_cut with contrastive_dim != D (the reference's own add would not broadcast)")
        if c.D not in (128, 256, 512):
            bad.append(f"dim_input={c.D} (the kernels are built for 128, 256 and 512; 128 trains through the chain of separate launches)")
        if bad:
            raise NotImplementedError("MadeTrainer (HIP training path) does not cover yet: " + "; ".join(bad))

    def _towers(self) -> List[Tuple[str, str]]:
        t = []
        if "music" in self.cfg.vmr_fusion:
            t.append(("xa", XA))
        if "video" in self.cfg.vmr_fusion:
            t.append(("xav", "music_guided_to_video_pooling_cross_transformer"))
        return t

    def _mlp_towers(self):
        c = self.cfg
        return (("video_mlp", "Video_encoder_projection", c.max_v_frames), ("audio_mlp", "Music_encoder_projection", c.max_snippet_num))

    def _table(self) -> Tuple[List[Tuple[str, object]], List[Tuple[str, object]]]:
        c = self.cfg
        mats: List[Tuple[str, object]] = []
        vecs: List[Tuple[str, object]] = []

        def lin(key, name):
            mats.append((key + ".w", name + ".weight")); vecs.append((key + ".b", name + ".bias"))

        def ln(key, name):
            vecs.append((key + ".g", name + ".weight")); vecs.append((key + ".b", name + ".bias"))

        lin("vit_proj", "vit_proj"); lin("ast_proj", "ast_proj")
        if c.with_cls_token and c.agg_module != "mlp":
            vecs.append(("cls_video", "video_cls_token")); vecs.append(("cls_audio", "audio_cls_token"))
        share = bool(c.transformer_is_share) and c.video_transformer_depth == c.audio_transformer_depth and c.video_transformer_depth > 0
        if c.agg_module == "mlp":
            for key, mod, _ in self._mlp_towers():
                lin(key + ".0", mod + ".net.0"); lin(key + ".3", mod + ".net.3"); lin(key + ".6", mod + ".net.6")
                for bn in ("1", "4"):
                    vecs.append((f"{key}.{bn}.g", f"{mod}.net.{bn}.weight")); vecs.append((f"{key}.{bn}.beta", f"{mod}.net.{bn}.bias"))
        for mod, depth in (() if c.agg_module == "mlp" else (("video_transformer", c.video_transformer_depth), ("audio_transformer", c.audio_transformer_depth))):
            src = "share_transformer" if share else mod
            for l in range(depth):
                p, q = f"{mod}.layers.{l}", f"{src}.layers.{l}"
                ln(p + ".ln1", q + ".0")
                mats.append((p + ".in.w", q + ".1.in_proj_weight")); vecs.append((p + ".in.b", q + ".1.in_proj_bias"))
                lin(p + ".out", q + ".1.out_proj"); ln(p + ".ln2", q + ".2")
                lin(p + ".ff1", q + ".3.0"); lin(p + ".ff2", q + ".3.3")
            lin(mod + ".final", src + ".final_linear")
        for key, xa in self._towers():
# ... 27 lines not shown
        ln("dec.norm", "detr_transformer.decoder.norm")
        mats.append(("query_embed", "decoder_query_embed.weight"))
        if "regression" in c.mml_localization:
            for i in range(3):
                lin(f"reg_mlp.{i}", f"reg_mlp.layers.{i}")
            return mats, vecs
        lin("class_embed", "class_embed")
        for i in range(3):
            lin(f"span_embed.{i}", f"span_embed.layers.{i}")
        if c.contrastive_align_loss:
            lin("proj_q", "contrastive_align_projection_query"); lin("proj_v", "contrastive_align_projection_vid")
        if c.moment_loss:
            for i in range(3):
                lin(f"moment_embed.{i}", f"moment_embed.layers.{i}")
        return mats, vecs

    def _init_master(self, sd: Dict[str, object]):
        dev = self.device
        BUF = (".running_mean", ".running_var", ".num_batches_tracked")
        names = [k for k in sd if not k.endswith(".pe") and k != "criterion.empty_weight" and not k.endswith(BUF)]
        self.buffers: Dict[str, Tensor] = {}
        for k in sd:
            if k.endswith(BUF):
                t = sd[k].detach() if isinstance(sd[k], torch.Tensor) else torch.from_numpy(np.asarray(sd[k]))
                self.buffers[k] = t.to(dev, torch.int64 if k.endswith(".num_batches_tracked") else torch.float32).clone()
        XAV = "music_guided_to_video_pooling_cross_transformer"
        pair_after = {}
        for xa in (XA, XAV):
            pair_after[xa + ".cross_attn.k_proj.weight"] = xa + ".cross_attn.v_proj.weight"
            pair_after[xa + ".cross_attn.k_proj.bias"] = xa + ".cross_attn.v_proj.bias"
        def group_of(k: str) -> int:
            if k.startswith(("vit_proj.", "ast_proj.", "video_transformer.", "audio_transformer.", "share_transformer.",
                             "video_cls_token", "audio_cls_token", "Video_encoder_projection.", "Music_encoder_projection.")):
                return 0
            if k.startswith((XA + ".", XAV + ".")) or k == "logit_scale":
                return 1
            if "regression" in self.cfg.mml_localization:
                if k.startswith(("video_music_fusion_cross_transformer.", "reg_mlp.")):
                    return 2
                return 3
            if k.startswith(("detr_transformer.", "span_embed.", "class_embed.", "contrastive_align_projection_", "moment_embed.",
                             "video_music_fusion_cross_transformer.")):
                return 2
            return 3
        names = sorted(names, key=group_of)
        order: List[str] = []
        for k in names:
            if k in pair_after.values():
                continue
            order.append(k)
            if k in pair_after:
                order.append(pair_after[k])
        shapes = {k: tuple(np.asarray(sd[k].detach().cpu() if isinstance(sd[k], torch.Tensor) else sd[k]).shape) for k in order}
        offs, off = {}, 0
        for k in order:
            offs[k] = off
            n = int(np.prod(shapes[k])) if len(shapes[k]) else 1
            off += n if k in pair_after else round_up(n, 64)
            if k in pair_after:
                assert n % 64 == 0
        self.flat_param = torch.zeros(off, device=dev, dtype=torch.float32)
        self.flat_grad = torch.zeros(off, device=dev, dtype=torch.float32)
        self.master: Dict[str, Tensor] = {}
        self.grad: Dict[str, Tensor] = {}
        for k in order:
            n = int(np.prod(shapes[k])) if len(shapes[k]) else 1
            self.master[k] = self.flat_param[offs[k]:offs[k] + n].view(shapes[k])
            self.grad[k] = self.flat_grad[offs[k]:offs[k] + n].view(shapes[k])
            v = sd[k]
            t = v.detach() if isinstance(v, torch.Tensor) else torch.from_numpy(np.asarray(v))
            self.master[k].copy_(t.to(dev, torch.float32))
        self.param_names = order
        self._offs = offs
        self.group_ranges = []
        for gi in range(3):
            ks = [k for k in order if group_of(k) == gi]
            b = offs[ks[0]]
            last = ks[-1]
            e = offs[last] + round_up(int(np.prod(shapes[last])) if len(shapes[last]) else 1, 64)
            self.group_ranges.append((b, e))
        self.exp_avg = torch.zeros_like(self.flat_param)
        self.exp_avg_sq = torch.zeros_like(self.flat_param)
        self.opt_step = 0
        self._norm_ws = torch.zeros(2 * 4 * (1 + 1024), device=dev, dtype=torch.float32)

    def _view(self, store: Dict[str, Tensor], ref) -> Tensor:
        if isinstance(ref, tuple):
            a, b = store[ref[0]], store[ref[1]]
            flat = self.flat_param if store is self.master else self.flat_grad
            o = self._offs[ref[0]]
            rows = a.shape[0] + b.shape[0]
            return flat[o:o + a.numel() + b.numel()].view((rows,) + tuple(a.shape[1:]))
        return store[ref]

    def repack(self, part: Optional[str] = None):
        import ctypes as C
        if getattr(self, "_pack_desc", None) is None:
            P, tc, dev = self.P, self.tc, self.device
            mats, vecs = self._table()
            self.G: Dict[str, Tensor] = {}
            for key, ref in vecs:
                v = self._view(self.master, ref)
                P[key] = v.view(-1) if v.dim() != 1 else v
                g = self._view(self.grad, ref)
                self.G[key] = g.view(-1) if g.dim() != 1 else g
            descs = []
            tiles = 0
            cut = self.group_ranges[0][1]
            part_of = []
            for key, ref in mats:
                m = self._view(self.master, ref)
                self.G[key] = self._view(self.grad, ref)
                rows, cols = m.shape
                w = None
                if tc == torch.float32:
                    P[key] = m
                else:
                    w = torch.empty(rows, cols, device=dev, dtype=tc)
                    P[key] = w
                wt = None
                if key not in ("query_embed", "vit_proj.w", "ast_proj.w"):
                    base = key[:-2] if key.endswith(".w") else key
                    wt = torch.zeros(cols, max(rows, HEAD_PAD), device=dev, dtype=tc)
                    P[base + ".wt"] = wt
                if w is None and wt is None:
                    continue
                d = _lib.MadeRepackDesc()
                d.src, d.w, d.wt = m.data_ptr(), (w.data_ptr() if w is not None else None), (wt.data_ptr() if wt is not None else None)
                d.rows, d.cols, d.wt_ld, d.tile_begin = rows, cols, (wt.shape[1] if wt is not None else 0), tiles
                d.dtype = ops.dt_of(wt if wt is not None else w)
                tiles += ((rows + 63) // 64) * ((cols + 63) // 64)
                descs.append(d)
                part_of.append("rest" if (m.data_ptr() - self.flat_param.data_ptr()) // 4 < cut else "early")

            def pack(ds):
                t0, out = 0, []
                for d in ds:
                    e = _lib.MadeRepackDesc()
                    C.memmove(C.byref(e), C.byref(d), C.sizeof(e))
                    e.tile_begin = t0
                    t0 += ((e.rows + 63) // 64) * ((e.cols + 63) // 64)
                    out.append(e)
                if not out:
                    return None
                arr = (_lib.MadeRepackDesc * len(out))(*out)
                return torch.from_numpy(np.frombuffer(bytes(arr), dtype=np.uint8).copy()).to(dev), len(out), t0
            self._pack_desc = {None: pack(descs), "early": pack([d for d, q in zip(descs, part_of) if q == "early"]),
                               "rest": pack([d for d, q in zip(descs, part_of) if q == "rest"])}
        pk = self._pack_desc[part]
        if pk is not None:
            _lib.check(_lib.lib().made_repack(pk[0].data_ptr(), pk[1], pk[2], torch.cuda.current_stream().cuda_stream), "made_repack")
        if self.cfg.agg_module == "mlp" and part != "early":
            P = self.P
            for key, mod, _ in self._mlp_towers():
                for bn in ("1", "4"):
                    sc, sh = P[f"{key}.{bn}.scale"], P[f"{key}.{bn}.shift"]
                    torch.add(self.buffers[f"{mod}.net.{bn}.running_var"], 1e-5, out=sc)
                    sc.rsqrt_().mul_(P[f"{key}.{bn}.g"])
                    torch.mul(self.buffers[f"{mod}.net.{bn}.running_mean"], sc, out=sh)
                    sh.neg_().add_(P[f"{key}.{bn}.beta"])

    def optimizer_step(self, lr_temporal: float, lr_matching: float, lr_detection: float, max_grad_norm: float = 1.0,
                       betas=(0.9, 0.999), eps: float = 1e-8, grad_scale: float = 1.0, device_state: Optional[Tensor] = None,
                       part: Optional[str] = None) -> None:
        import ctypes as C
        assert part in (None, "early", "rest")
        if part != "rest":
            self.opt_step += 1
            self.generation += 1
        groups = (_lib.MadeAdamGroup * 3)()
        for i, lr in enumerate((lr_temporal, lr_matching, lr_detection)):
            groups[i].begin, groups[i].end = self.group_ranges[i]
            if (part == "early" and i == 0) or (part == "rest" and i != 0):
                groups[i].end = groups[i].begin
            groups[i].lr, groups[i].max_norm = float(lr), float(max_grad_norm)
        ws = self._norm_ws[:self._norm_ws.numel() // 2] if part != "early" else self._norm_ws[self._norm_ws.numel() // 2:]
        if device_state is not None:
            _lib.check(_lib.lib().made_adam_step_device(self.flat_param.data_ptr(), self.flat_grad.data_ptr(), self.exp_avg.data_ptr(),
                                                        self.exp_avg_sq.data_ptr(), self.flat_param.numel(), groups, 3, float(betas[0]),
                                                        float(betas[1]), float(eps), device_state.data_ptr(), 0 if part == "rest" else 1,
                                                        float(grad_scale), ws.data_ptr(), torch.cuda.current_stream().cuda_stream),
                       "made_adam_step_device")
            self.repack(part)
            return
        _lib.check(_lib.lib().made_adam_step(self.flat_param.data_ptr(), self.flat_grad.data_ptr(), self.exp_avg.data_ptr(),
                                             self.exp_avg_sq.data_ptr(), self.flat_param.numel(), groups, 3, float(betas[0]), float(betas[1]),
                                             float(eps), self.opt_step, float(grad_scale), ws.data_ptr(),
                                             torch.cuda.current_stream().cuda_stream), "made_adam_step")
        self.repack(part)

    def train_step(self, frame_feats, segment_feats, frame_masks, segment_masks, spans_target, seed: int, lrs=(1e-4, 1e-4, 1e-4),
                   max_grad_norm: float = 1.0, w_ret: Optional[Tensor] = None, w_loc: Optional[Tensor] = None, dist=None,
                   music_ids=None, v_duration: Optional[Tensor] = None) -> Dict[str, Tensor]:
        self._zero_grad_in_forward = True
        try:
            out = self.forward_train(frame_feats, segment_feats, frame_masks, segment_masks, spans_target, seed=seed, music_ids=music_ids,
                                     v_duration=v_duration)
        finally:
            self._zero_grad_in_forward = False
        scale = 1.0
        if dist is not None and dist.get_world_size() > 1:
            cut = self.group_ranges[0][1]
            works = []
            self.backward(w_ret, w_loc, grad_sync=lambda: works.append(dist.all_reduce(self.flat_grad[cut:], async_op=True)))
            works.append(dist.all_reduce(self.flat_grad[:cut], async_op=True))
            for w in works:
                w.wait()
            scale = 1.0 / dist.get_world_size()
        elif self._early_opt_ok():
            self.backward(w_ret, w_loc, early_opt=lambda: self.optimizer_step(*lrs, max_grad_norm=max_grad_norm, part="early"))
            self.optimizer_step(*lrs, max_grad_norm=max_grad_norm, part="rest")
            return out
        else:
            self.backward(w_ret, w_loc)
        self.optimizer_step(*lrs, max_grad_norm=max_grad_norm, grad_scale=scale)
        return out

    def _early_opt_ok(self) -> bool:
        return _lib.variant_env("MADE_EARLY_OPT", "0") == "1" and "regression" not in self.cfg.mml_localization

    def capture_train_step(self, frame_feats, segment_feats, frame_masks, segment_masks, spans_target, *, max_grad_norm: float = 1.0,
                           music_ids=None, v_duration: Optional[Tensor] = None, dist=None, mode: str = "graph") -> "TrainStepGraph":
        return TrainStepGraph(self, frame_feats, segment_feats, frame_masks, segment_masks, spans_target, max_grad_norm=max_grad_norm,
                              music_ids=music_ids, v_duration=v_duration, dist=dist, mode=mode)

    def state_dict_numpy(self) -> Dict[str, np.ndarray]:
        sd = {k: v.detach().cpu().numpy().copy() for k, v in self.master.items()}
        sd.update({k: v.detach().cpu().numpy().copy() for k, v in self.buffers.items()})
        return sd

    def grads_numpy(self) -> Dict[str, np.ndarray]:
        torch.cuda.synchronize()
        return {k: v.detach().cpu().numpy().copy() for k, v in self.grad.items()}

    def _drop(self, site: str, p: float):
        if not self.training_dropout or p <= 0.0:
            return None
        seed_dev = getattr(self, "_seed_dev", None)
        return (seed_dev if seed_dev is not None else self.seed, dr.site_id(site), float(p))

    def _train_buffers(self, B: int, Tv: int, Ta: int) -> Dict[str, Tensor]:
        key = (B, Tv, Ta)
        ws = self._tws.get(key)
        if ws is not None:
            return ws
        c, dev, tc = self.cfg, self.device, self.tc
        concat = "concat" in c.mml_fusion
        D, L, Q, H = c.D, (Tv + Ta if concat else Ta), c.num_moment_queries, c.detr_nheads
        Ft, Fd, nd, ne = c.temporal_ffn_dim, c.detr_dim_feedforward, c.detr_dec_layers, c.detr_enc_layers
        Hh = c.SA_temporal_heads
        f32 = torch.float32

        def E(*shape, dtype=None):
            return torch.empty(shape, device=dev, dtype=dtype or tc)

        def Z(*shape, dtype=None):
            return torch.zeros(shape, device=dev, dtype=dtype or tc)

        ws = {}
# ... 50 lines not shown
            h1=E(nd * B * Q, D), h2=E(nd * B * Q, D), hg1=E(nd * B * Q, D), hg2=E(nd * B * Q, D),
            dlogsp=Z(2, nd * B * Q, HEAD_PAD, dtype=f32), dlogsp_c=Z(2, nd * B * Q, HEAD_PAD),
        )
        ws["dlog"], ws["dsp"], ws["dlog_c"], ws["dsp_c"] = ws["dlogsp"][0], ws["dlogsp"][1], ws["dlogsp_c"][0], ws["dlogsp_c"][1]
        ws["dvideo"], ws["dmusic"] = ws["dclip"][:B * D].view(B, D), ws["dclip"][B * D:2 * B * D].view(B, D)
        if "video" in c.vmr_fusion:
            Svp = round_up(Tv, 8)
            ws.update(
                yv1=E(B, D), yq=E(B, D), ys1=E(B * Tv, D), yk=E(B * Tv, D), yu=E(B * Tv, D), yo=E(B * B, D), ya2=E(B * B, D),
                ya3=E(B * B, D), yy=E(B * B, D), yg1=E(B * B, D), yg2=E(B * B, D), yg3=E(B * B, D),
                yS=E(B * B, Svp, dtype=f32), ydP=E(B * B, Svp, dtype=f32), yP=E(B * B, Svp), ydS=E(B * B, Svp), ydSt=E(B, Tv, B),
                ydkv=E(B * Tv, 2 * D), yds1=E(B * Tv, D), ydseg=E(B * Tv, D), ydq32=E(B, D, dtype=f32), ydq=E(B, D), ydv1=E(B, D),
                dframe_sum=E(B * Tv, D))
        for l in range(ne):
            ws.update({f"e.{l}.src": E(rows, D), f"e.{l}.srcpos": E(rows, D), f"e.{l}.qkv": E(rows, 3 * D), f"e.{l}.att": E(rows, D),
                       f"e.{l}.lse": E(B * H * L, dtype=f32), f"e.{l}.kbits": E(*ops.attention_bits_shape(B, H, L, L), dtype=torch.int32), f"e.{l}.x": E(rows, D), f"e.{l}.s1": E(rows, D), f"e.{l}.h": E(rows, Fd),
                       f"e.{l}.x2": E(rows, D)})
        ws.update(mem=E(rows, D), mempos=E(rows, D))
        if not concat:
            inner, ra, rv = c.ca_heads * c.ca_dim_head, B * Ta, B * Tv
            ws.update(c_nx=E(ra, D), c_nc=E(rv, D), c_q=E(ra, inner), c_kv=E(rv, 2 * inner), c_att=E(ra, inner), c_lse=E(B * c.ca_heads * Ta, dtype=f32),
                      c_ax=E(ra, D), c_nf=E(ra, D), c_z1=E(ra, c.ca_ffn_dim), c_h=E(ra, c.ca_ffn_dim), c_y=E(ra, D),
                      c_g1=E(ra, D), c_g2=E(ra, D), c_g3=E(ra, D), c_gf=E(ra, c.ca_ffn_dim), c_gq=E(ra, inner), c_gkv=E(rv, 2 * inner),
                      c_gatt=E(ra, inner), c_delta=E(B * c.ca_heads * Ta, dtype=f32), c_dseg=E(ra, D), c_dframe=E(rv, D), c_gnc=E(rv, D))
        i32 = torch.int32
        ws.update(rows_v=(E(B * Tv, dtype=i32), E(1, dtype=i32)), rows_a=(E(B * Ta, dtype=i32), E(1, dtype=i32)), rows_f=(E(rows, dtype=i32), E(1, dtype=i32)),
                  order_v=E(B, dtype=i32), order_a=E(B, dtype=i32), order_f=E(B, dtype=i32))
        ws.update(wide_plan=E(_lib.wide_plan_words(B, self._wide_slots()), dtype=i32))
        BQ = B * Q
        stacks = dict(tgt=E(nd + 1, BQ, D), tq=E(nd + 1, BQ, D), qkv=E(nd, BQ, 3 * D), att=E(nd, BQ, D), t_a=E(nd, BQ, D), t1=E(nd, BQ, D),
                      t1q=E(nd, BQ, D), qc=E(nd, BQ, D), pooled=E(nd, BQ, H * D), attc=E(nd, BQ, D), t_b=E(nd, BQ, D), t2=E(nd, BQ, D),
                      h=E(nd, BQ, Fd), t_c=E(nd, BQ, D),
                      **({"n1": E(nd, BQ, D)} if c.detr_pre_norm else {}),
                      g_ffn=E(nd, BQ, D), g_z=E(nd, BQ, Fd), g_ca=E(nd, BQ, D), g_attc=E(nd, BQ, D), g_q=E(nd, B, HQ, D), g_qc=E(nd, BQ, D),
                      g_sa=E(nd, BQ, D), g_qkv=E(nd, BQ, 3 * D), dt1q=E(nd, BQ, D))
        ws["dstack"] = stacks
        ws["s_stack"] = E(nd, BQ, H, dtype=f32)
        ws["ca_lse"] = E(nd, B * HQ, dtype=f32)
        for l in range(nd):
            ws.update({f"d.{l}.{k}": v[l] for k, v in stacks.items() if not k.startswith("g_")})
            ws.update({f"d.{l}.lse": E(B * H * Q, dtype=f32), f"d.{l}.s": ws["s_stack"][l], f"d.{l}.t3": stacks["tgt"][l + 1]})
        if c.contrastive_align_loss:
            Dc = c.contrastive_hdim
            if c.audio_short_cut:
                ws.update(pq_n0=E(nd * B * Q, Dc, dtype=f32), pq_s1=E(nd * B * Q, Dc, dtype=f32), pq_s2=E(nd * B * Q, Dc, dtype=f32),
                          dpq_s=E(nd * B * Q, Dc, dtype=f32), dpq_s2=E(nd * B * Q, Dc, dtype=f32))
            ws.update(dpq=E(nd * B * Q, Dc, dtype=f32), dvid_sum=ws["dclip"][2 * B * D:2 * B * D + B * Dc].view(B, Dc), dpq_raw=E(nd * B * Q, Dc), dpv_raw=E(B * Tv, Dc),
                      dframe_x=E(B * Tv, D))
        self._tws[key] = ws
        return ws

    @torch.no_grad()
    def same_music_exclusion(self, music_ids) -> Optional[Tensor]:
        c = self.cfg
        if music_ids is None or c.vmr_loss != "dual_single_loss_fuse":
            return None
        ids = list(music_ids)
        code = {}
        idx = torch.tensor([code.setdefault(str(i), len(code)) for i in ids])
        ex = (idx[:, None] == idx[None, :]).float()
        ex.fill_diagonal_(0.0)
        return ex.to(self.device)

    def forward_train(self, frame_feats: Tensor, segment_feats: Tensor, frame_masks: Tensor, segment_masks: Tensor,
                      spans_target: Tensor, seed: int = 0, music_ids=None, v_duration: Optional[Tensor] = None) -> Dict[str, Tensor]:
        c, P = self.cfg, self.P
        self._set_products()
        if c.predict_center == 1 and v_duration is None:
            raise ValueError("predict_center=1 needs v_duration (reference model/model_Uni.py:280-282)")
        self.seed = int(seed)
        B, Tv, _ = frame_feats.shape
        Ta = segment_feats.shape[1]
        concat = "concat" in c.mml_fusion
        D, L, Q, nd, H = c.D, (Tv + Ta if concat else Ta), c.num_moment_queries, c.detr_dec_layers, c.detr_nheads
        ws, tw = self._buffers(B, Tv, Ta), self._train_buffers(B, Tv, Ta)
        fm, sm = frame_masks.contiguous(), segment_masks.contiguous()
        pd = float(c.detr_dropout)
        self._shape = (B, Tv, Ta)
        self._inputs = (frame_feats.contiguous(), segment_feats.contiguous(), fm, sm, spans_target.contiguous())

        fus, fus_mask = ws["fus"], ws["fus_mask"]
        self._groups = {}
        cur, side = torch.cuda.current_stream(), self._side_stream()
        side.wait_stream(cur)
        self._rows = {sm.data_ptr(): ops.row_index(sm, out=tw["rows_a"])}
        self._order = {sm.data_ptr(): ops.batch_order(sm, out=tw["order_a"])}
        with torch.cuda.stream(side):
            ops.concat_cols(fm if concat else None, sm, fus_mask)
            self._rows[fm.data_ptr()] = ops.row_index(fm, out=tw["rows_v"])
            self._order[fm.data_ptr()] = ops.batch_order(fm, out=tw["order_v"])
            self._rows[fus_mask.data_ptr()] = ops.row_index(fus_mask, out=tw["rows_f"])
            self._order[fus_mask.data_ptr()] = ops.batch_order(fus_mask, out=tw["order_f"])
            self._wide_plan = (ops.wide_slice_plan(fus_mask, n_slots=self._wide_slots(), max_slices=WIDE_SLICES,
                                                   order=self._order[fus_mask.data_ptr()], out=tw["wide_plan"])
                               if "regression" not in c.mml_localization and self._wide_planned_ok(B, H * Q, D) else None)
            pos = ops.sine_pe(fus_mask, P["dim_t"], out=ws["pos"])
            self._encode_train(self._inputs[0], fm, "video", ws, tw, 0)
        self._encode_train(self._inputs[1], sm, "audio", ws, tw, Tv)
        cur.wait_stream(side)
        rows_f = self._rows[fus_mask.data_ptr()]
        if concat:
            frame, seg = fus[:, :Tv], fus[:, Tv:]
        else:
            frame, seg = ws["frame_buf"], ws["seg_buf"]
            self._ca_fusion_train(ws, tw, frame, seg, fm, sm, B, Tv, Ta)
        self._views = (frame, seg)
        video, music = ws["video"], ws["music"]
        out: Dict[str, Tensor] = dict(video_feats=video, music_feats=music, frame_feats=frame, segment_feats=seg)

        qp = P["query_embed"]
        hd = D // H
        ca_scale = 1.0 / math.sqrt(hd)
        GQ = tw.get("GQ")
        regression = "regression" in c.mml_localization

        def dec_fill_tgt() -> None:
            tgt = tw["d.0.tgt"]
            if c.moment_query_type in ("video", "music", "xpool"):
                if c.moment_query_type == "xpool":
                    cur.wait_stream(side)
                src_vec = video if c.moment_query_type == "video" else (music if c.moment_query_type == "music" else tw["xpool_q"])
                if Q == 1:
                    tr.add3(tgt, src_vec)
                else:
                    tgt.view(B, Q, D).copy_(src_vec[:, None, :].expand(B, Q, D))
            else:
                _tape.zero_(tgt)
            if Q > 1 and not c.detr_pre_norm:
                tr.add3(tw["d.0.tq"], tgt, qp, b_mod=Q * D)

        stage = self._dec_stage_chain()

        def dec_query_side(l: int) -> None:
            p, d = f"detr_transformer.decoder.layers.{l}", f"d.{l}"
            tgt, tq = tw[d + ".tgt"], tw[d + ".tq"]
            qkv = tw[d + ".qkv"]
            Win, bin_ = P[p + ".ca.in.w"], P[p + ".ca.in.b"]
            Wt = P[p + ".ca.in.wt"]
            if c.detr_pre_norm:
                n1 = tw[d + ".n1"]
                qp_rows = qp.expand(B * Q, D) if Q == 1 else qp.repeat(B, 1)
                if Q == 1:
                    Wsa, bsa = P[p + ".sa.in.w"], P[p + ".sa.in.b"]
                    ops.layernorm(tgt, P[p + ".ln1.g"], P[p + ".ln1.b"], out=n1)
                    ops.linear(n1, Wsa[2 * D:], bsa[2 * D:], out=tw[d + ".att"], drop=self._drop(f"dec.{l}" + ".sa_attn", pd), drop_ld=H, drop_col_div=hd)
                else:
                    ops.layernorm_add(tgt, P[p + ".ln1.g"], P[p + ".ln1.b"], qp_rows, n1, tq)
                    ops.linear(n1, P[p + ".sa.in.w"], P[p + ".sa.in.b"], A2=tq, a2_replace=True,
                               segs=[Seg(out=qkv, col_begin=0, use_a2=True), Seg(out=qkv[:, 2 * D:], col_begin=2 * D, ldo=qkv.stride(0))])
                    q3 = qkv.view(B, Q, 3 * D)
                    ops.attention(q3[:, :, :D], q3[:, :, D:2 * D], q3[:, :, 2 * D:], tw[d + ".att"].view(B, Q, D), H, lse=tw[d + ".lse"],
                                  drop=self._drop(f"dec.{l}" + ".sa_attn", pd))
                ta = ops.linear(tw[d + ".att"], P[p + ".sa.out.w"], P[p + ".sa.out.b"], R=tgt, out=tw[d + ".t_a"], drop=self._drop(f"dec.{l}" + ".drop1", pd))
                ops.layernorm_add(ta, P[p + ".ln2.g"], P[p + ".ln2.b"], qp_rows, tw[d + ".t1"], tw[d + ".t1q"])
                qc = ops.linear(tw[d + ".t1q"], Win[:D], bin_[:D], out=tw[d + ".qc"])
            elif stage:
                Wsa, bsa = P[p + ".sa.in.w"], P[p + ".sa.in.b"]
                sa_drop = dict(drop=self._drop(f"dec.{l}" + ".sa_attn", pd), drop_ld=H, drop_col_div=hd)
                if l == 0:
                    ops.dec_stage(tgt, Wsa[2 * D:], bsa[2 * D:], tw[d + ".att"], **sa_drop)
                else:
                    q_ = f"detr_transformer.decoder.layers.{l - 1}"
                    ops.dec_stage(tw[f"d.{l - 1}.t_c"], Wsa[2 * D:], bsa[2 * D:], tw[d + ".att"], ln=(P[q_ + ".ln3.g"], P[q_ + ".ln3.b"]),
                                  x_out=tgt, **sa_drop)
                ta = ops.linear(tw[d + ".att"], P[p + ".sa.out.w"], P[p + ".sa.out.b"], R=tgt, out=tw[d + ".t_a"], drop=self._drop(f"dec.{l}" + ".drop1", pd))
                qc = ops.dec_stage(ta, Win[:D], bin_[:D], tw[d + ".qc"], ln=(P[p + ".ln1.g"], P[p + ".ln1.b"]), add=qp,
                                   x_out=tw[d + ".t1"], a_out=tw[d + ".t1q"])
            else:
                if Q == 1:
                    Wsa, bsa = P[p + ".sa.in.w"], P[p + ".sa.in.b"]
                    ops.linear(tgt, Wsa[2 * D:], bsa[2 * D:], out=tw[d + ".att"], drop=self._drop(f"dec.{l}" + ".sa_attn", pd), drop_ld=H, drop_col_div=hd)
                else:
                    ops.linear(tgt, P[p + ".sa.in.w"], P[p + ".sa.in.b"], A2=tq, a2_replace=True,
                               segs=[Seg(out=qkv, col_begin=0, use_a2=True), Seg(out=qkv[:, 2 * D:], col_begin=2 * D, ldo=qkv.stride(0))])
                    q3 = qkv.view(B, Q, 3 * D)
                    ops.attention(q3[:, :, :D], q3[:, :, D:2 * D], q3[:, :, 2 * D:], tw[d + ".att"].view(B, Q, D), H, lse=tw[d + ".lse"],
                                  drop=self._drop(f"dec.{l}" + ".sa_attn", pd))
                ta = ops.linear(tw[d + ".att"], P[p + ".sa.out.w"], P[p + ".sa.out.b"], R=tgt, out=tw[d + ".t_a"], drop=self._drop(f"dec.{l}" + ".drop1", pd))
# ... 432 lines not shown
        inv_keep = 1.0 / (1.0 - pd) if (self.training_dropout and pd > 0) else 1.0
        fus, fus_mask = ws["fus"], ws["fus_mask"]
        fskip = fus_mask.view(-1)
        qskip = fus_mask
        regression = "regression" in c.mml_localization
        if regression:
            fskip = qskip = None
        rows = B * L
        if zero_grad and not getattr(self, "_grads_zeroed", False):
            _tape.zero_(self.flat_grad)
        self._grads_zeroed = False
        dvideo, dmusic = tw["dvideo"], tw["dmusic"]
        _tape.zero_(tw["dclip"])
        video, music = ws["video"], ws["music"]
        frame, seg_view = self._views
        cur, side = torch.cuda.current_stream(), self._side_stream()
        xq = c.moment_query_type == "xpool" and not regression
        side.wait_stream(cur)
        ret_done = None
        ret_gen = None
        if not xq:
            ret_main = _lib.variant_env("MADE_RET_BWD_MAIN", "0") == "1"
            ret_split = (_lib.variant_env("MADE_RET_SPLIT", "1") != "0" and not ret_main and not regression
                         and _lib.variant_env("MADE_RET_HANDOFF", "") == "" and _lib.variant_env("MADE_RET_HANDOFF_REV", "") == "")
            with torch.cuda.stream(cur if ret_main else side):
                self._ret_main_stream = cur
                try:
                    self._ret_ck(0)
                    if ret_split:
                        ret_gen = self._retrieval_bwd_gen(ws, tw, g_ret, B, Ta, sm)
                        if next(ret_gen, "done") == "done":
                            ret_gen = None
                    else:
                        self._retrieval_bwd(ws, tw, g_ret, B, Ta, sm)
                    on_main = torch.cuda.current_stream() == cur
                finally:
                    self._ret_main_stream = None
                if ret_gen is None:
                    ret_done = torch.cuda.Event()
                    ret_done.record(cur if on_main else side)

        if regression:
            dmem, dtgt0 = self._regression_bwd(ws, tw, g_loc, B, L), None
        else:
            logits, spans = ws["logits"], ws["spans"]
            pi, ti, cnt = self._match
            pq = ws["pq"] if c.contrastive_align_loss else None
            vid_sum = ws["vid_sum"] if c.contrastive_align_loss else None
            tr.set_criterion_bwd(logits, spans, tg, pi, ti, cnt, pq, vid_sum, P["empty_weight"], c.foreground_label, P["crit_weights"], g_loc,
                                 tw["dlog"], tw["dsp"], tw["dpq"] if pq is not None else None, tw["dvid_sum"] if pq is not None else None,
                                 ld_out=HEAD_PAD, through_sigmoid=True)
            hs2 = ws["hs"].view(nd * B * Q, D)
            dhs = tw["dhs"]
            dlog, dsp = tw["dlog"], tw["dsp"]
            if self.tc != torch.float32:
                tr.add3(tw["dlogsp_c"], tw["dlogsp"])
                dlog, dsp = tw["dlog_c"], tw["dsp_c"]
            heads_dw: list = []
            heads_dw.append(lambda: tr.gemm_tn(dlog[:, :2], hs2, G["class_embed.w"], accumulate=True, colsum=G["class_embed.b"]))
            ops.linear(dlog, P["class_embed.wt"], None, out=dhs)
            n_span = 1 if c.predict_center == 1 else 2
            heads_dw.append(lambda: tr.gemm_tn(dsp[:, :n_span], tw["h2"], G["span_embed.2.w"], accumulate=True, colsum=G["span_embed.2.b"]))
            dz2 = ops.linear(dsp, P["span_embed.2.wt"], None, out=tw["hg1"], gate=_lib.GATE_RELU_OUT, G=tw["h2"])
            dz1 = self._lin_bwd(dz2, tw["h1"], "span_embed.1", dx_out=tw["hg2"], gate=_lib.GATE_RELU_OUT, G=tw["h1"], later=heads_dw)
            self._lin_bwd(dz1, hs2, "span_embed.0", dx_out=dhs, R=dhs, later=heads_dw)
            if c.contrastive_align_loss:
                Dc = pq.shape[-1]
                dn = tw["dpq"]
                if c.audio_short_cut:
                    if c.aux_loss and nd > 1:
                        n_aux = (nd - 1) * B * Q
                        ds2 = tw["dpq_s2"][:n_aux]
                        tr.l2norm_bwd(tw["pq_s2"][:n_aux], dn[:n_aux], dx=ds2)
                        dmusic.add_(ds2.view(nd - 1, B, Q, D).sum((0, 2)))
                        dn[:n_aux].copy_(ds2)
                    tr.l2norm_bwd(tw["pq_s1"], dn, dx=tw["dpq_s"])
                    dmusic.add_(tw["dpq_s"].view(nd, B, Q, D).sum((0, 2)))
                    dn = tw["dpq_s"]
                tr.l2norm_bwd(ws["pq_raw"], dn, dx_alt=tw["dpq_raw"])
                self._lin_bwd(tw["dpq_raw"], hs2, "proj_q", dx_out=dhs, R=dhs, later=heads_dw)
                tr.l2norm_bwd(ws["pv_raw"], tw["dvid_sum"], dx_alt=tw["dpv_raw"], dy_rows_per=Tv)
                heads_dw.append(lambda: tr.gemm_tn(tw["dpv_raw"][:Tv], frame[0], G["proj_v.w"], accumulate=True, colsum=G["proj_v.b"], batch=(B, 1),
                                                   a_zs=(Tv * Dc, 0), b_zs=(frame.stride(0), 0), colsum_zs=(0, 0)))
                ops.linear(tw["dpv_raw"], P["proj_v.wt"], None, out=tw["dframe_x"])

            qp = P["query_embed"]
            mem3, mempos3 = tw["mem"].view(B, L, D), tw["mempos"].view(B, L, D)
            Lp = tw["PdS"].shape[-1]
            GQ, PdS = tw["GQ"], tw["PdS"]
            ca_scale = 1.0 / math.sqrt(hd)
            st = tw["dstack"]
            dtgt = None
            stage = self._dec_stage_chain()
            pre = bool(c.detr_pre_norm)
            S_all = tw["dS_S"]
            if not stage:
                ops.linear(GQ[0, 1].reshape(nd * HQ, D), mempos3[0], None, M=nd * HQ, N=L, K=D, batch=B, a_z_stride=GQ.stride(0), w_z_stride=L * D,
                           segs=[Seg(out=S_all, ldo=Lp, rows_per_batch=HQ, out_batch_stride=B * HQ * Lp, out_z_stride=HQ * Lp)])
            n_split_b = int(_lib.variant_env("MADE_WIDE_NSPLIT", "0")) or max(1, min(8, 256 // max(B, 1)))
            wplan = self._wide_plan if HQ <= 8 and _lib.variant_env("MADE_WIDE_PLANNED", "1") != "0" else None
            if wplan is not None:
                n_split_b = WIDE_SLICES
            if stage:
                gN = tw["dgN"]
                tr.layernorm_bwd(tw["dstack"]["tgt"][1:].reshape(nd * B * Q, D), P["dec.norm.g"], dhs, gN, dgamma=G["dec.norm.g"], dbeta=G["dec.norm.b"])
            for l in range(nd - 1, -1, -1):
                p, d = f"detr_transformer.decoder.layers.{l}", f"d.{l}"
                g1, g2, g4 = tw["dg1"], tw["dg2"], tw["dg4"]
                if stage and _lib.variant_env("MADE_CHAIN_BUFS", "1") != "0":
                    ch = tw["dchain"][l]
                    g1a, g1b, g2a, g2b, g2c, dt_out = ch[0], ch[1], ch[2], ch[3], ch[4], ch[5]
                else:
                    g1a = g1b = g1
                    g2a = g2b = g2c = g2
                    dt_out = tw["dtgt"]
                Win, Wt = P[p + ".ca.in.w"], P[p + ".ca.in.wt"]
                g_ffn, g_z, g_ca, g_attc, g_q, g_qc, g_sa, gqkv = (st[k][l] for k in ("g_ffn", "g_z", "g_ca", "g_attc", "g_q", "g_qc", "g_sa", "g_qkv"))
                if stage:
                    tr.dec_stage_bwd(tw[d + ".t_c"], P[p + ".ln3.g"], gN[l * B * Q:(l + 1) * B * Q], P[p + ".ff2.wt"], g_z,
                                     dgamma_a=G[p + ".ln3.g"], dbeta_a=G[p + ".ln3.b"], add=dtgt, dx_out=g2a, a_out=g_ffn,
                                     drop_a=self._drop(f"dec.{l}" + ".drop3", pd), G=tw[d + ".h"], gate_scale=inv_keep)
                elif pre:
                    tr.layernorm_bwd(tw[d + ".t3"], P["dec.norm.g"], dhs[l * B * Q:(l + 1) * B * Q], g1, dgamma=G["dec.norm.g"], dbeta=G["dec.norm.b"], add=dtgt)
                    tr.gate_rows(g1, g_ffn, drop=self._drop(f"dec.{l}" + ".drop3", pd))
                else:
                    tr.layernorm_bwd(tw[d + ".t3"], P["dec.norm.g"], dhs[l * B * Q:(l + 1) * B * Q], g1, dgamma=G["dec.norm.g"], dbeta=G["dec.norm.b"], add=dtgt)
                    tr.layernorm_bwd(tw[d + ".t_c"], P[p + ".ln3.g"], g1, g2, dgamma=G[p + ".ln3.g"], dbeta=G[p + ".ln3.b"],
                                     dx_drop=g_ffn, drop=self._drop(f"dec.{l}" + ".drop3", pd))
                if not stage:
                    ops.linear(g_ffn, P[p + ".ff2.wt"], None, out=g_z, gate=_lib.GATE_RELU_OUT, G=tw[d + ".h"], gate_scale=inv_keep)
                if pre:
                    dn3 = ops.linear(g_z, P[p + ".ff1.wt"], None, out=g4)
                    tr.layernorm_bwd(tw[d + ".t_b"], P[p + ".ln3.g"], dn3, g2, dgamma=G[p + ".ln3.g"], dbeta=G[p + ".ln3.b"], add=g1,
                                     dx_drop=g_ca, drop=self._drop(f"dec.{l}" + ".drop2", pd))
                    dattc = ops.linear(g_ca, P[p + ".ca.out.wt"], None, out=g_attc)
                else:
                    dt2 = ops.linear(g_z, P[p + ".ff1.wt"], None, out=g1a, R=g2a)
                if pre:
                    pass
                elif stage:
                    dattc = tr.dec_stage_bwd(tw[d + ".t_b"], P[p + ".ln2.g"], dt2, P[p + ".ca.out.wt"], g_attc, dgamma_a=G[p + ".ln2.g"],
                                             dbeta_a=G[p + ".ln2.b"], dx_out=g2b, a_out=g_ca, drop_a=self._drop(f"dec.{l}" + ".drop2", pd))
                else:
                    tr.layernorm_bwd(tw[d + ".t_b"], P[p + ".ln2.g"], dt2, g2, dgamma=G[p + ".ln2.g"], dbeta=G[p + ".ln2.b"],
                                     dx_drop=g_ca, drop=self._drop(f"dec.{l}" + ".drop2", pd))
                    dattc = ops.linear(g_ca, P[p + ".ca.out.wt"], None, out=g_attc)
                dpooled = GQ[:, 0, l]
                qprime = GQ[:, 1, l]
                if stage:
                    ops.linear(dattc[:, :hd], Wt[:, 2 * D:2 * D + hd], None, M=B * Q, N=D, K=hd, batch=H, a_z_stride=hd, w_z_stride=hd,
                               segs=[Seg(out=dpooled, ldo=D, rows_per_batch=Q, out_batch_stride=dpooled.stride(0), out_z_stride=Q * D)])
                    tr.attention_wide_bwd(qprime, dpooled, tw[d + ".pooled"].view(B, HQ, D), mempos3, mem3, tw["ca_lse"][l].view(B, HQ),
                                          PdS[:, 0, l], PdS[:, 1, l], g_q, scale=ca_scale, key_mask=fus_mask, ssum=tw[d + ".s"].view(B, HQ),
                                          dattc=dattc, vbias=P[p + ".ca.in.b"][2 * D:], hd=hd, drop=self._drop(f"dec.{l}" + ".ca_attn", pd),
                                          n_split=n_split_b, part_dq=ws["part_o"], plan=wplan)
                else:
                    tr.head_bias_bwd(dattc, tw[d + ".s"], P[p + ".ca.in.b"][2 * D:], G[p + ".ca.in.b"][2 * D:], tw["d_ds"], H)
                    d_ds = tw["d_ds"]
                    if Q > 1:
                        tw["dds_raw"].view(B, H, Q).copy_(d_ds.view(B, Q, H).permute(0, 2, 1))
                        d_ds = tw["dds_raw"]
                    ops.linear(dattc[:, :hd], Wt[:, 2 * D:2 * D + hd], None, M=B * Q, N=D, K=hd, batch=H, a_z_stride=hd, w_z_stride=hd,
                               segs=[Seg(out=dpooled, ldo=D, rows_per_batch=Q, out_batch_stride=dpooled.stride(0), out_z_stride=Q * D)])
                    S, dP = S_all[l], tw["dS_dP"]
                    ops.linear(dpooled[0], mem3[0], None, M=HQ, N=L, K=D, batch=B, a_z_stride=dpooled.stride(0), w_z_stride=L * D,
                               segs=[Seg(out=dP, ldo=Lp, out_z_stride=HQ * Lp)])
                    tr.softmax_bwd(S, dP, fus_mask, HQ, ca_scale, PdS[:, 0, l], PdS[:, 1, l], tw["dSt"], HQ, L, extra=d_ds.view(-1),
# ... 148 lines not shown
                    pend.append((gq[:, :2 * D], n1pos, gW[:2 * D], gb[:2 * D]))
                    pend.append((gq[:, 2 * D:], n1, gW[2 * D:], gb[2 * D:]))
                else:
                    tr.gemm_tn(gq[:, :2 * D], n1pos, gW[:2 * D], accumulate=True, colsum=gb[:2 * D], rows=self._rw(fskip))
                    tr.gemm_tn(gq[:, 2 * D:], n1, gW[2 * D:], accumulate=True, colsum=gb[2 * D:], rows=self._rw(fskip))
                dn1 = ops.linear(gq, P[p + ".in.wt"], None, out=g2, rows=self._rw(fskip))
                nxt = tw["dfus"] if dx is tw["eg1"] else tw["eg1"]
                dsrc = tr.layernorm_bwd(xin, P[p + ".ln1.g"], dn1, nxt, dgamma=G[p + ".ln1.g"], dbeta=G[p + ".ln1.b"], add=dx, row_skip=fskip)
                if enc_dw_side:
                    side.wait_stream(cur)
                    with torch.cuda.stream(side):
                        self._flush_dw(pend, fskip)
                        enc_dw_done[l & 1] = torch.cuda.Event()
                        enc_dw_done[l & 1].record(side)
                else:
                    self._flush_dw(pend, fskip)
                continue
            src = fus.view(rows, D) if l == 0 else tw[e + ".src"]
            srcpos = tw[e + ".srcpos"]
            tr.layernorm_bwd(tw[e + ".x2"], P[p + ".ln2.g"], dsrc, g2, dgamma=G[p + ".ln2.g"], dbeta=G[p + ".ln2.b"], dx_drop=g3,
                             drop=self._drop(f"enc.{l}" + ".drop2", pd), row_skip=fskip)
            dz = self._lin_bwd(g3, tw[e + ".h"], p + ".ff2", dx_out=gf, row_mask=fskip, skip=fskip, gate=_lib.GATE_RELU_OUT, G=tw[e + ".h"],
                               gate_scale=inv_keep, defer=pend)
            ds1 = self._lin_bwd(dz, tw[e + ".s1"], p + ".ff1", dx_out=g3b, row_mask=fskip, skip=fskip, R=g2, defer=pend)
            dx = tw["eg1"] if dsrc is not tw["eg1"] else tw["dfus"]
            tr.layernorm_bwd(tw[e + ".x"], P[p + ".ln1.g"], ds1, dx, dgamma=G[p + ".ln1.g"], dbeta=G[p + ".ln1.b"], dx_drop=g2b,
                             drop=self._drop(f"enc.{l}" + ".drop1", pd), row_skip=fskip)
            datt = self._lin_bwd(g2b, tw[e + ".att"], p + ".out", dx_out=g3c, row_mask=fskip, skip=fskip, defer=pend)
            qkv = tw[e + ".qkv"]
            q3, gq3 = qkv.view(B, L, 3 * D), gq.view(B, L, 3 * D)
            tr.attention_bwd(q3[:, :, :D], q3[:, :, D:2 * D], q3[:, :, 2 * D:], tw[e + ".att"].view(B, L, D), datt.view(B, L, D),
                             gq3[:, :, :D], gq3[:, :, D:2 * D], gq3[:, :, 2 * D:], tw[e + ".lse"], tw["e_delta"], H,
                             key_mask=fus_mask, q_skip_mask=qskip, drop=self._drop(f"enc.{l}" + ".attn", pd),
                             order=self._order[fus_mask.data_ptr()], keep_bits=tw[e + ".kbits"] if self._bits else None)
            gW, gb = G[p + ".in.w"], G[p + ".in.b"]
            if self._groupable(gq, srcpos, gW[:2 * D]) and self._rw(fskip) is not None:
                pend.append((gq[:, :2 * D], srcpos, gW[:2 * D], gb[:2 * D]))
                pend.append((gq[:, 2 * D:], src, gW[2 * D:], gb[2 * D:]))
            else:
                tr.gemm_tn(gq[:, :2 * D], srcpos, gW[:2 * D], accumulate=True, colsum=gb[:2 * D], rows=self._rw(fskip))
                tr.gemm_tn(gq[:, 2 * D:], src, gW[2 * D:], accumulate=True, colsum=gb[2 * D:], rows=self._rw(fskip))
            nxt = tw["dfus"] if dx is tw["eg1"] else tw["eg1"]
            dsrc = ops.linear(gq, P[p + ".in.wt"], None, R=dx, out=nxt, rows=self._rw(fskip))
            if enc_dw_side:
                side.wait_stream(cur)
                with torch.cuda.stream(side):
                    self._flush_dw(pend, fskip)
                    enc_dw_done[l & 1] = torch.cuda.Event()
                    enc_dw_done[l & 1].record(side)
            else:
                self._flush_dw(pend, fskip)
        dfus = dsrc.view(B, L, D)
        if concat:
            dl_v, dl_a = dfus[:, :Tv], dfus[:, Tv:]
        else:
            self._ca_fusion_bwd(ws, tw, dsrc, frame, seg_view, fm, sm, B, Tv, Ta)
            dl_v, dl_a = tw["c_dframe"].view(B, Tv, D), tw["c_dseg"].view(B, Ta, D)

        if ret_done is not None and grad_sync is None and _lib.variant_env("MADE_BWD_EVENT_JOIN", "1") != "0":
            cur.wait_event(ret_done)
        else:
            cur.wait_stream(side)
        if xq:
            dq = tw["dxpool_q"]
            tr.add3(dq, dtgt0.view(B, D) if Q == 1 else dtgt0.view(B, Q, D).float().sum(dim=1).contiguous())
            self._retrieval_bwd(ws, tw, g_ret, B, Ta, sm, dpool=dq)
        if c.moment_query_type in ("video", "music") and not regression:
            dq_vec = dvideo if c.moment_query_type == "video" else dmusic
            tr.add3(dq_vec, dq_vec, dtgt0.view(B, D) if Q == 1 else dtgt0.view(B, Q, D).float().sum(dim=1))

        if grad_sync is not None:
            grad_sync()
        opt_st = None
        if early_opt is not None:
            opt_st = self._opt_stream()
            e_main, e_side = torch.cuda.Event(), torch.cuda.Event()
            e_main.record(cur); e_side.record(side)
            opt_st.wait_event(e_main); opt_st.wait_event(e_side)
            with torch.cuda.stream(opt_st):
                early_opt()
        side.wait_stream(cur)
        with torch.cuda.stream(side):
            dxv = tw["dframe_x"] if (c.contrastive_align_loss and not regression) else None
            if "video" in c.vmr_fusion:
                dxv = tw["ydseg"] if dxv is None else tr.add3(tw["dframe_sum"], dxv, tw["ydseg"])
            self._encode_bwd("video", ws, tw, dl_v, dxv.view(B, Tv, D) if dxv is not None else None, dvideo, fm, feats_v)
        self._encode_bwd("audio", ws, tw, dl_a, tw["xdseg"].view(B, Ta, D), dmusic, sm, feats_a,
                         dw_stream=side if _lib.variant_env("MADE_AUDIO_DW_SIDE", "0") != "0" else None)
        cur.wait_stream(side)
        if opt_st is not None:
            cur.wait_stream(opt_st)

    def _regression_train(self, out, ws, tw, mem3: Tensor, fus_mask: Tensor, v_duration, cur, side) -> Dict[str, Tensor]:
        c, P = self.cfg, self.P
        B = mem3.shape[0]
        cnt = fus_mask.sum(dim=1, keepdim=True)
        fx = (ops.masked_mean(mem3, None) / cnt).to(self.tc)
        h1 = ops.linear(fx, P["reg_mlp.0.w"], P["reg_mlp.0.b"], act=ops.ACT_RELU)
        h2 = ops.linear(h1, P["reg_mlp.1.w"], P["reg_mlp.1.b"], act=ops.ACT_RELU)
        spans = torch.empty(B, 2, device=self.device, dtype=torch.float32)
        if c.predict_center == 1:
            ops.linear(h2, P["reg_mlp.2.w"], P["reg_mlp.2.b"], act=ops.ACT_SIGMOID, segs=[Seg(out=spans, ldo=2)])
            spans[:, 1] = v_duration.to(self.device, torch.float32) / c.max_m_duration
        else:
            ops.linear(h2, P["reg_mlp.2.w"], P["reg_mlp.2.b"], act=ops.ACT_SIGMOID, out=spans)
        tg = self._inputs[4].to(torch.float32)
        assert tg.shape == (B, 1, 2), f"spans_target.shape {tuple(tg.shape)} must equal to src_spans.shape {(B, 1, 2)}"
        l1 = (spans.view(B, 1, 2) - tg).abs().mean()
        self._reg = (fx, h1, h2, spans, cnt, tg)
        out.update(pred_spans=spans.view(B, 1, 2), regression_loss_span=l1, localization_loss=(l1 * 20).view(1))
        cur.wait_stream(side)
        return out

    def _regression_bwd(self, ws, tw, g_loc: Optional[Tensor], B: int, L: int) -> Tensor:
        c, P, G, D = self.cfg, self.P, self.G, self.cfg.D
        fx, h1, h2, spans, cnt, tg = self._reg
        n = 1 if c.predict_center == 1 else 2
        scale = 20.0 / (B * 2)
        g = torch.sign(spans - tg.view(B, 2)) * scale
        if g_loc is not None:
            g = g * g_loc.to(torch.float32).view(())
        dz = torch.zeros(B, HEAD_PAD, device=self.device, dtype=self.tc)
        dz[:, :n] = (g * spans * (1.0 - spans))[:, :n].to(self.tc)
        tr.gemm_tn(dz[:, :n], h2, G["reg_mlp.2.w"], accumulate=True, colsum=G["reg_mlp.2.b"])
        dh2 = ops.linear(dz, P["reg_mlp.2.wt"], None, out=torch.empty_like(h2), gate=_lib.GATE_RELU_OUT, G=h2)
        dh1 = self._lin_bwd(dh2, h1, "reg_mlp.1", dx_out=torch.empty_like(h1), gate=_lib.GATE_RELU_OUT, G=h1)
        dfx = self._lin_bwd(dh1, fx, "reg_mlp.0", dx_out=torch.empty(B, D, device=self.device, dtype=self.tc))
        dmem = tw["eg1"]
        dmem.view(B, L, D).copy_((dfx.float() / cnt)[:, None, :].expand(B, L, D))
        return dmem

    def _retrieval_bwd(self, *a, **k) -> None:
        for _ in self._retrieval_bwd_gen(*a, **k):
            pass

    def _retrieval_bwd_gen(self, ws, tw, g_ret: Optional[Tensor], B: int, S: int, sm: Tensor, dpool: Optional[Tensor] = None):
        c, P, G, D = self.cfg, self.P, self.G, self.cfg.D
        video, music = ws["video"], ws["music"]
        dvideo, dmusic = tw["dvideo"], tw["dmusic"]
        ls, gls = P["logit_scale"], G["logit_scale"]
        wgt = float(c.dual_single_loss_weight)
        ds_s, ds_d, ds_dt, cws = tw["dsims_s"], tw["dsims_d"], tw["dsims_dt"], tw["clip_ws"]
        ds_st = tw["dsims_st"] if "video" in c.vmr_fusion else None
        single = dual = False
        fuse_dz = None
        if c.vmr_loss == "dual":
            tr.clip_loss_bwd(ws["sims_dual"], ls, wgt, g_ret, cws, ds_d, ds_dt, gls); dual = True
        elif c.vmr_loss == "single":
            tr.clip_loss_bwd(ws["sims_single"], ls, wgt, g_ret, cws, ds_s, ds_st, gls); single = True
        elif c.vmr_loss == "dual_single_loss_fuse":
            tr.clip_loss_bwd(ws["sims_dual"], ls, 1.0, g_ret, cws, ds_d, ds_dt, gls, row_exclude=getattr(self, "_row_exclude", None))
            tr.clip_loss_bwd(ws["sims_single"], ls, 1.0, g_ret, cws, ds_s, ds_st, gls)
            single = dual = True
        elif c.vmr_loss == "dual_single_feature_fuse":
            fused, fn, vn = ws["ff_fused"], ws["ff_fn"], ws["ff_vn"]
            tr.clip_loss_bwd(ws["sims_fused"], ls, wgt, g_ret, cws, ds_s, None, gls)
            dfn = (ds_s.t().reshape(B * B, 1) * vn.repeat(B, 1)).contiguous()
            dvn = torch.einsum("nm,mnd->nd", ds_s, fn.view(B, B, D)).contiguous()
            dfused = torch.empty(B * B, D, device=self.device, dtype=torch.float32)
            tr.l2norm_bwd(fused, dfn, dfused)
            tr.l2norm_bwd(video, dvn, dvideo, accumulate=True)
            dmusic.add_(dfused.view(B, B, D).sum(dim=1))
            fuse_dz = dfused
        else:
            both = tr.add3(tw["sims_both"], ws["sims_dual"], ws["sims_single"])
            tr.clip_loss_bwd(both, ls, wgt, g_ret, cws, ds_d, ds_dt, gls)
# ... 434 lines not shown
```

Before: 14120 pairs/s.

## Fuse mask prep into one batched kernel, fuse Adam with repack, defer proj_v dx

Replaces the separate row_index, batch_order and wide_slice_plan launches for the audio, video and fused masks with a single multi-job batch_prep kernel, one block per job, reading the split masks directly. Adds a fused Adam+repack kernel that updates params and writes the bf16/transposed weight copies in the same pass, with optional norm folding. It also moves the proj_v dx GEMM onto the side stream next to the video encoder backward. The aim is fewer launches and less memory traffic, at the cost of more complex kernels and a serial single-block prep.

```diff
diff --git a/include/made_hip.h b/include/made_hip.h
--- a/include/made_hip.h
+++ b/include/made_hip.h
@@ -531,6 +531,27 @@
 } MadeRepackDesc;
 int made_repack(const MadeRepackDesc* descs_device, int32_t n_desc, int64_t total_tiles, void* stream);
 
+#define MADE_PREP_ROWS 0
+#define MADE_PREP_ORDER 1
+#define MADE_PREP_PLAN 2
+#define MADE_BATCH_PREP_MAX_JOBS 8
+typedef struct MadeBatchPrepJob {
+    int32_t kind, n_slots, max_slices, _pad;
+    const float* mask1; const float* mask2;
+    int64_t B, T1, T;
+    int32_t* out; int32_t* out2;
+    int64_t out_words;
+} MadeBatchPrepJob;
+int made_batch_prep(const MadeBatchPrepJob* jobs, int32_t n_jobs, void* stream);
+
+#define MADE_ADAM_WS_FLOATS (MADE_ADAM_MAX_GROUPS * (1 + MADE_ADAM_NORM_BLOCKS) + 4)
+typedef struct MadeAdamVecDesc { int64_t begin, end, chunk_begin; } MadeAdamVecDesc;
+int made_adam_repack_step(float* param, const float* grad, float* exp_avg, float* exp_avg_sq, int64_t n,
+                          const MadeAdamGroup* groups, int32_t n_groups, float beta1, float beta2, float eps, int64_t step,
+                          MadeAdamDeviceState* state_device, int32_t advance_state, float grad_scale, float* norm_ws,
+                          const MadeRepackDesc* descs_device, int32_t n_desc, int64_t total_tiles,
+                          const MadeAdamVecDesc* vecs_device, int32_t n_vec, int64_t total_chunks, int32_t fold_finish, void* stream);
+
 
 int made_recall_ranks(const float* sims, int64_t ld, const int32_t* group_id, const int32_t* gt_group, int64_t Nv, int64_t Nm,
                       int64_t n_groups, int32_t* rank_out, int32_t* top1_out, void* stream);
diff --git a/mgsv_amd/_lib.py b/mgsv_amd/_lib.py
--- a/mgsv_amd/_lib.py
+++ b/mgsv_amd/_lib.py
@@ -186,6 +186,21 @@
 class MadeRepackDesc(C.Structure):
     _fields_ = [("src", vp), ("w", vp), ("wt", vp), ("rows", i64), ("cols", i64), ("wt_ld", i64), ("tile_begin", i64),
                 ("dtype", i32), ("_pad", i32)]
+
+
+ADAM_WS_FLOATS = 4 * (1 + 1024) + 4
+
+
+class MadeAdamVecDesc(C.Structure):
+    _fields_ = [("begin", i64), ("end", i64), ("chunk_begin", i64)]
+
+
+PREP_ROWS, PREP_ORDER, PREP_PLAN, BATCH_PREP_MAX_JOBS = 0, 1, 2, 8
+
+
+class MadeBatchPrepJob(C.Structure):
+    _fields_ = [("kind", i32), ("n_slots", i32), ("max_slices", i32), ("_pad", i32), ("mask1", vp), ("mask2", vp),
+                ("B", i64), ("T1", i64), ("T", i64), ("out", vp), ("out2", vp), ("out_words", i64)]
 
 
 class MadeFrameDesc(C.Structure):
@@ -264,6 +279,9 @@
     "made_adam_step": (C.c_int, [vp, vp, vp, vp, i64, C.POINTER(MadeAdamGroup), i32, f32, f32, f32, i64, f32, vp, vp]),
     "made_adam_step_device": (C.c_int, [vp, vp, vp, vp, i64, C.POINTER(MadeAdamGroup), i32, f32, f32, f32, vp, i32, f32, vp, vp]),
     "made_repack": (C.c_int, [vp, i32, i64, vp]),
+    "made_batch_prep": (C.c_int, [C.POINTER(MadeBatchPrepJob), i32, vp]),
+    "made_adam_repack_step": (C.c_int, [vp, vp, vp, vp, i64, C.POINTER(MadeAdamGroup), i32, f32, f32, f32, i64, vp, i32, f32, vp,
+                                        vp, i32, i64, vp, i32, i64, i32, vp]),
     "made_row_groups": (C.c_int, [vp, i64, vp, vp]),
     "made_row_index": (C.c_int, [vp, i64, vp, vp, vp]),
     "made_linear_variant": (C.c_int, [C.POINTER(MadeLinearArgs)]),
diff --git a/mgsv_amd/csrc/attention_wide.hip b/mgsv_amd/csrc/attention_wide.hip
--- a/mgsv_amd/csrc/attention_wide.hip
+++ b/mgsv_amd/csrc/attention_wide.hip
@@ -1,4 +1,5 @@
 #include "common.h"
+#include "batch_prep.h"
 
 #include <type_traits>
 
@@ -531,77 +532,14 @@
     return made_check_launch("made_attention_wide(combine)");
 }
 
-constexpr int PLAN_T = 1024;
+constexpr int PLAN_T = made_prep::PREP_T;
 __global__ __launch_bounds__(PLAN_T) void wide_slice_plan_kernel(const float* __restrict__ mask, int B, int L, int n_slots, int max_slices,
                                                                  const int32_t* __restrict__ order, int32_t* __restrict__ plan) {
-    __shared__ int32_t s_tiles[PLAN_T], s_first[PLAN_T], s_ord[PLAN_T];
+    __shared__ int32_t s_tiles[PLAN_T], s_first[PLAN_T], s_ord[PLAN_T], s_len[PLAN_T];
     __shared__ int32_t s_cap;
     extern __shared__ __attribute__((aligned(16))) unsigned char lds[];
-    uint32_t* s_bits = (uint32_t*)lds;
-    const int tid = threadIdx.x, lane = tid & 63, wave = tid >> 6;
-    const int nch = (L + 63) / 64, wpr = 2 * nch;
-    if (tid == 0) s_cap = 0x7fffffff;
-    for (int b = wave; b < B; b += PLAN_T / 64) {
-        const float* m = mask + (int64_t)b * L;
-        int last = -1, first = -1;
-        for (int c0 = 0; c0 < nch; c0 += 8) {
-            float v[8];
-#pragma unroll
-            for (int j = 0; j < 8; ++j) {
-                const int i = (c0 + j) * 64 + lane;
-                v[j] = m[i < L ? i : L - 1];
-            }
-#pragma unroll
-            for (int j = 0; j < 8; ++j) {
-                const int i = (c0 + j) * 64 + lane;
-                const unsigned long long bal = __ballot(i < L && v[j] != 0.f);
-                if (c0 + j < nch) {
-                    if (lane == 0) { s_bits[b * wpr + 2 * (c0 + j)] = (uint32_t)bal; s_bits[b * wpr + 2 * (c0 + j) + 1] = (uint32_t)(bal >> 32); }
-                    if (bal) {
-                        last = (c0 + j) * 64 + 63 - __clzll(bal);
-                        if (first < 0) first = (c0 + j) * 64 + __ffsll(bal) - 1;
-                    }
-                }
-            }
-        }
-        if (lane == 0) { s_tiles[b] = (last + 1 + 31) / 32; s_first[b] = first < 0 ? 0 : first; }
-    }
-    if (tid < B) {
-        const int o = order ? order[tid] : tid;
-        s_ord[tid] = o >= 0 && o < B ? o : tid;
-    }
-    __syncthreads();
-    int tmax = 1;
-    for (int b = 0; b < B; ++b) tmax = max(tmax, s_tiles[b]);
-    for (int c = tid + 1; c <= tmax; c += PLAN_T) {
-        const int n = made_wide_slice_count(s_tiles, 1, B, c, max_slices);
-        if (n >= 0 && n <= n_slots) atomicMin(&s_cap, c);
-    }
-    __syncthreads();
-    const int cap = s_cap <= tmax ? s_cap : tmax;
-    int used = 0;
-    for (int r = 0; r < B; ++r) { const int t = s_tiles[s_ord[r]]; used += t > cap ? (t + cap - 1) / cap : 1; }
-    if (tid == 0) { plan[0] = cap; plan[1] = used; plan[2] = n_slots; plan[3] = max_slices; }
-    int32_t* slots = plan + MADE_WIDE_PLAN_HEAD + MADE_WIDE_PLAN_SAMPLE * B;
-    if (tid < B) {
-        int slot0 = 0;
-        for (int r = 0; r < tid; ++r) { const int t = s_tiles[s_ord[r]]; slot0 += t > cap ? (t + cap - 1) / cap : 1; }
-        const int b = s_ord[tid], t = s_tiles[b], fv = s_first[b];
-        const int n = t > cap ? (t + cap - 1) / cap : 1;
-        int32_t* sm = plan + MADE_WIDE_PLAN_HEAD + MADE_WIDE_PLAN_SAMPLE * b;
-        sm[0] = t; sm[1] = slot0; sm[2] = n; sm[3] = fv;
-        for (int s = 0; s < n && slot0 + s < n_slots; ++s) {
-            int32_t* sp = slots + (int64_t)MADE_WIDE_PLAN_SLOT * (slot0 + s);
-            const int t0 = made_wide_slice_first(t, n, s), tn = made_wide_slice_len(t, n, s);
-            sp[0] = b; sp[1] = t0; sp[2] = tn; sp[3] = s; sp[4] = fv; sp[5] = n; sp[6] = t; sp[7] = 0;
-            for (int i = 0; i < MADE_WIDE_PLAN_SLOT_BITS; ++i) sp[8 + i] = i < tn ? (int32_t)s_bits[b * wpr + t0 + i] : 0;
-        }
-    }
-    for (int w = used + tid; w < n_slots; w += PLAN_T) {
-        int32_t* sp = slots + (int64_t)MADE_WIDE_PLAN_SLOT * w;
-        sp[0] = -1;
-        for (int i = 1; i < MADE_WIDE_PLAN_SLOT; ++i) sp[i] = 0;
-    }
+    made_prep::wide_slice_plan_body(made_prep::PlainMask{mask, L}, B, L, n_slots, max_slices, order, false, plan,
+                                    made_prep::PlanLds{s_tiles, s_first, s_ord, s_len, &s_cap, (uint32_t*)lds});
 }
 
 __global__ __launch_bounds__(NTHREADS) void attention_wide_combine_planned_kernel(const MadeWideAttnArgs a, const int32_t* __restrict__ plan) {
diff --git a/mgsv_amd/csrc/batch_prep.h b/mgsv_amd/csrc/batch_prep.h
--- /dev/null
+++ b/mgsv_amd/csrc/batch_prep.h
@@ -0,0 +1,201 @@
+#pragma once
+#include "common.h"
+
+namespace made_prep {
+
+constexpr int PREP_T = 1024;
+
+struct PlainMask {
+    const float* m; int64_t T;
+    __device__ __forceinline__ float flat(int64_t idx) const { return m[idx]; }
+    __device__ __forceinline__ float row(int b, int64_t i) const { return m[(int64_t)b * T + i]; }
+};
+
+struct SplitMask {
+    const float* m1; const float* m2; int T1, T;
+    __device__ __forceinline__ float row(int b, int64_t i) const {
+        return i < T1 ? m1[(int64_t)b * T1 + i] : m2[(int64_t)b * (T - T1) + (i - T1)];
+    }
+    __device__ __forceinline__ float flat(int64_t idx) const {
+        const int b = (int)((uint32_t)idx / (uint32_t)T);
+        return row(b, (int)idx - b * T);
+    }
+};
+
+template <typename MV>
+__device__ __forceinline__ void row_index_body(const MV mask, int64_t M, int32_t* row_index, int32_t* n_rows, int* wsum, int* wlast) {
+    constexpr int NB = 16;
+    const int lane = threadIdx.x & 63, wave = threadIdx.x >> 6;
+    const int64_t per = ((M + 15) / 16 + 63) / 64 * 64;
+    const int64_t b = (int64_t)wave * per, e = b + per < M ? b + per : M;
+    uint64_t bal[NB];
+    auto ballots = [&](int64_t i0) __attribute__((always_inline)) {
+        float v[NB];
+        const int64_t p = i0 + lane;
+        if (i0 + NB * 64 <= e) {
+#pragma unroll
+            for (int j = 0; j < NB; ++j) v[j] = mask.flat(p + j * 64);
+        } else {
+#pragma unroll
+            for (int j = 0; j < NB; ++j) v[j] = i0 + j * 64 + lane < e ? mask.flat(p + j * 64) : 0.f;
+        }
+#pragma unroll
+        for (int j = 0; j < NB; ++j) bal[j] = __ballot(v[j] != 0.f);
+    };
+    int cnt = 0, last = -1;
+    for (int64_t i0 = b; i0 < e; i0 += NB * 64) {
+        ballots(i0);
+#pragma unroll
+        for (int j = 0; j < NB; ++j) {
+            cnt += __popcll(bal[j]);
+            if (bal[j]) last = (int)(i0 + j * 64) + 63 - __clzll(bal[j]);
+        }
+    }
+    if (lane == 0) { wsum[wave] = cnt; wlast[wave] = last; }
+    __syncthreads();
+    int base = 0, total = 0, lastv = 0;
+    for (int w = 0; w < 16; ++w) {
+        if (w < wave) base += wsum[w];
+        total += wsum[w];
+        if (wlast[w] >= 0) lastv = wlast[w];
+    }
+    for (int64_t i0 = b; i0 < e; i0 += NB * 64) {
+        ballots(i0);
+#pragma unroll
+        for (int j = 0; j < NB; ++j) {
+            if ((bal[j] >> lane) & 1ull) row_index[base + __popcll(bal[j] & ((1ull << lane) - 1ull))] = (int32_t)(i0 + j * 64 + lane);
+            base += __popcll(bal[j]);
+        }
+    }
+    if (threadIdx.x == 0) n_rows[0] = total;
+    for (int64_t i = total + threadIdx.x; i < M; i += PREP_T) row_index[i] = lastv;
+}
+
+template <typename MV>
+__device__ __forceinline__ void batch_order_body(const MV mask, int B, int64_t T, int32_t* order, int* len) {
+    const int lane = threadIdx.x & 63, wave = threadIdx.x >> 6;
+    for (int b0 = wave; b0 < B; b0 += 64) {
+        int cnt[4] = {0, 0, 0, 0};
+        for (int64_t i0 = 0; i0 < T; i0 += 512) {
+            float v[4][8];
+#pragma unroll
+            for (int s4 = 0; s4 < 4; ++s4) {
+                const int b = b0 + 16 * s4;
+                const int bc = b < B ? b : B - 1;
+#pragma unroll
+                for (int j = 0; j < 8; ++j) {
+                    const int64_t i = i0 + j * 64 + lane;
+                    v[s4][j] = i < T ? mask.row(bc, i) : 0.f;
+                }
+            }
+#pragma unroll
+            for (int s4 = 0; s4 < 4; ++s4)
+#pragma unroll
+                for (int j = 0; j < 8; ++j) cnt[s4] += __popcll(__ballot(v[s4][j] != 0.f));
+        }
+#pragma unroll
+        for (int s4 = 0; s4 < 4; ++s4)
+            if (lane == 0 && b0 + 16 * s4 < B) len[b0 + 16 * s4] = cnt[s4];
+    }
+    __syncthreads();
+    for (int b = threadIdx.x; b < B; b += PREP_T) {
+        const int mine = len[b];
+        int rank = 0;
+        for (int j = 0; j < B; ++j) {
+            const int l = len[j];
+            rank += (l > mine || (l == mine && j < b)) ? 1 : 0;
+        }
+        order[rank] = b;
+    }
+}
+
+struct PlanLds { int32_t* s_tiles; int32_t* s_first; int32_t* s_ord; int32_t* s_len; int32_t* s_cap; uint32_t* s_bits; };
+
+template <typename MV>
+__device__ __forceinline__ void wide_slice_plan_body(const MV mask, int B, int L, int n_slots, int max_slices, const int32_t* order,
+                                                     bool own_order, int32_t* plan, const PlanLds s) {
+    int32_t* s_tiles = s.s_tiles; int32_t* s_first = s.s_first; int32_t* s_ord = s.s_ord;
+    uint32_t* s_bits = s.s_bits;
+    const int tid = threadIdx.x, lane = tid & 63, wave = tid >> 6;
+    const int nch = (L + 63) / 64, wpr = 2 * nch;
+    if (tid == 0) *s.s_cap = 0x7fffffff;
+    for (int b = wave; b < B; b += PREP_T / 64) {
+        int last = -1, first = -1, cnt = 0;
+        for (int c0 = 0; c0 < nch; c0 += 8) {
+            float v[8];
+#pragma unroll
+            for (int j = 0; j < 8; ++j) {
+                const int i = (c0 + j) * 64 + lane;
+                v[j] = mask.row(b, i < L ? i : L - 1);
+            }
+#pragma unroll
+            for (int j = 0; j < 8; ++j) {
+                const int i = (c0 + j) * 64 + lane;
+                const unsigned long long bal = __ballot(i < L && v[j] != 0.f);
+                if (c0 + j < nch) {
+                    if (lane == 0) { s_bits[b * wpr + 2 * (c0 + j)] = (uint32_t)bal; s_bits[b * wpr + 2 * (c0 + j) + 1] = (uint32_t)(bal >> 32); }
+                    cnt += __popcll(bal);
+                    if (bal) {
+                        last = (c0 + j) * 64 + 63 - __clzll(bal);
+                        if (first < 0) first = (c0 + j) * 64 + __ffsll(bal) - 1;
+                    }
+                }
+            }
+        }
+        if (lane == 0) { s_tiles[b] = (last + 1 + 31) / 32; s_first[b] = first < 0 ? 0 : first; s.s_len[b] = cnt; }
+    }
+    if (own_order) {
+        __syncthreads();
+        if (tid < B) {
+            const int mine = s.s_len[tid];
+            int rank = 0;
+            for (int j = 0; j < B; ++j) {
+                const int l = s.s_len[j];
+                rank += (l > mine || (l == mine && j < tid)) ? 1 : 0;
+            }
+            s_ord[rank] = tid;
+        }
+    } else if (tid < B) {
+        const int o = order ? order[tid] : tid;
+        s_ord[tid] = o >= 0 && o < B ? o : tid;
+    }
+    __syncthreads();
+    int tmax = 1;
+    for (int b = 0; b < B; ++b) tmax = max(tmax, s_tiles[b]);
+    for (int c = tid + 1; c <= tmax; c += PREP_T) {
+        const int n = made_wide_slice_count(s_tiles, 1, B, c, max_slices);
+        if (n >= 0 && n <= n_slots) atomicMin(s.s_cap, c);
+    }
+    __syncthreads();
+    const int cap = *s.s_cap <= tmax ? *s.s_cap : tmax;
+    int used = 0;
+    for (int r = 0; r < B; ++r) { const int t = s_tiles[s_ord[r]]; used += t > cap ? (t + cap - 1) / cap : 1; }
+    if (tid == 0) { plan[0] = cap; plan[1] = used; plan[2] = n_slots; plan[3] = max_slices; }
+    int32_t* slots = plan + MADE_WIDE_PLAN_HEAD + MADE_WIDE_PLAN_SAMPLE * B;
+    if (tid < B) {
+        int slot0 = 0;
+        for (int r = 0; r < tid; ++r) { const int t = s_tiles[s_ord[r]]; slot0 += t > cap ? (t + cap - 1) / cap : 1; }
+        const int b = s_ord[tid], t = s_tiles[b], fv = s_first[b];
+        const int n = t > cap ? (t + cap - 1) / cap : 1;
+        int32_t* sm = plan + MADE_WIDE_PLAN_HEAD + MADE_WIDE_PLAN_SAMPLE * b;
+        sm[0] = t; sm[1] = slot0; sm[2] = n; sm[3] = fv;
+        for (int sl = 0; sl < n && slot0 + sl < n_slots; ++sl) {
+            int32_t* sp = slots + (int64_t)MADE_WIDE_PLAN_SLOT * (slot0 + sl);
+            const int t0 = made_wide_slice_first(t, n, sl), tn = made_wide_slice_len(t, n, sl);
+            sp[0] = b; sp[1] = t0; sp[2] = tn; sp[3] = sl; sp[4] = fv; sp[5] = n; sp[6] = t; sp[7] = 0;
+            for (int i = 0; i < MADE_WIDE_PLAN_SLOT_BITS; ++i) sp[8 + i] = i < tn ? (int32_t)s_bits[b * wpr + t0 + i] : 0;
+        }
+    }
+    for (int w = used + tid; w < n_slots; w += PREP_T) {
+        int32_t* sp = slots + (int64_t)MADE_WIDE_PLAN_SLOT * w;
+        sp[0] = -1;
+        for (int i = 1; i < MADE_WIDE_PLAN_SLOT; ++i) sp[i] = 0;
+    }
+}
+
+constexpr int64_t ROW_INDEX_MAX = 1 << 22;
+constexpr int64_t ORDER_MAX_B = 8192;
+constexpr int64_t PLAN_BITS_MAX = 40 * 1024;
+__host__ __device__ inline int64_t plan_bits_bytes(int64_t B, int64_t L) { return B * ((L + 63) / 64 * 2) * 4; }
+
+}
diff --git a/mgsv_amd/csrc/batch_prep.hip b/mgsv_amd/csrc/batch_prep.hip
--- /dev/null
+++ b/mgsv_amd/csrc/batch_prep.hip
@@ -0,0 +1,57 @@
+#include "common.h"
+#include "batch_prep.h"
+
+namespace {
+using namespace made_prep;
+
+struct PrepJobs { MadeBatchPrepJob j[MADE_BATCH_PREP_MAX_JOBS]; };
+
+__global__ __launch_bounds__(PREP_T) void batch_prep_kernel(const PrepJobs jobs) {
+    extern __shared__ __attribute__((aligned(16))) unsigned char lds[];
+    const MadeBatchPrepJob& j = jobs.j[blockIdx.x];
+    const SplitMask mv{j.mask1, j.mask2, (int)j.T1, (int)j.T};
+    int32_t* w = (int32_t*)lds;
+    if (j.kind == MADE_PREP_ROWS) {
+        row_index_body(mv, j.B * j.T, j.out, j.out2, w, w + 16);
+    } else if (j.kind == MADE_PREP_ORDER) {
+        batch_order_body(mv, (int)j.B, j.T, j.out, w);
+    } else {
+        wide_slice_plan_body(mv, (int)j.B, (int)j.T, j.n_slots, j.max_slices, nullptr, true, j.out,
+                             PlanLds{w, w + PREP_T, w + 2 * PREP_T, w + 3 * PREP_T, w + 4 * PREP_T, (uint32_t*)(w + 4 * PREP_T + 4)});
+    }
+}
+}
+
+extern "C" int made_batch_prep(const MadeBatchPrepJob* jobs, int32_t n_jobs, void* stream) {
+    MADE_REQUIRE(jobs && n_jobs >= 1 && n_jobs <= MADE_BATCH_PREP_MAX_JOBS, "made_batch_prep: n_jobs=%d out of range", n_jobs);
+    PrepJobs pj;
+    memset(&pj, 0, sizeof(pj));
+    size_t lds = 0;
+    for (int i = 0; i < n_jobs; ++i) {
+        const MadeBatchPrepJob& j = jobs[i];
+        MADE_REQUIRE(j.mask2 && j.out && j.B > 0 && j.T > 0 && j.T1 >= 0 && j.T1 < j.T && (j.T1 == 0 || j.mask1) && j.T <= (1 << 22),
+                     "made_batch_prep: job %d: bad mask", i);
+        size_t need = 0;
+        if (j.kind == MADE_PREP_ROWS) {
+            MADE_REQUIRE(j.out2 != nullptr, "made_batch_prep: job %d: the row list needs its count word", i);
+            MADE_UNSUPPORTED(j.B * j.T <= ROW_INDEX_MAX, "made_batch_prep: job %d: %lld rows too many for the single-workgroup scan", i, (long long)(j.B * j.T));
+            need = 32 * 4;
+        } else if (j.kind == MADE_PREP_ORDER) {
+            MADE_UNSUPPORTED(j.B <= ORDER_MAX_B, "made_batch_prep: job %d: B=%lld exceeds the single-workgroup table (8192)", i, (long long)j.B);
+            need = (size_t)j.B * 4;
+        } else if (j.kind == MADE_PREP_PLAN) {
+            MADE_REQUIRE(j.n_slots > 0 && j.max_slices > 0 && j.out_words >= made_wide_plan_words(j.B, j.n_slots) && ((uintptr_t)j.out % 16) == 0,
+                         "made_batch_prep: job %d: bad plan arguments", i);
+            MADE_UNSUPPORTED(j.B <= j.n_slots && j.n_slots <= PREP_T && j.max_slices <= 8, "made_batch_prep: job %d: plan of B=%lld samples over %d slots", i,
+                             (long long)j.B, j.n_slots);
+            MADE_UNSUPPORTED(j.T <= 32768 && plan_bits_bytes(j.B, j.T) <= PLAN_BITS_MAX, "made_batch_prep: job %d: the valid-key bits do not fit one workgroup's LDS", i);
+            need = (size_t)(4 * PREP_T + 4) * 4 + (size_t)plan_bits_bytes(j.B, j.T);
+        } else {
+            MADE_REQUIRE(false, "made_batch_prep: job %d: kind=%d", i, j.kind);
+        }
+        lds = need > lds ? need : lds;
+        pj.j[i] = j;
+    }
+    hipLaunchKernelGGL(batch_prep_kernel, dim3((unsigned)n_jobs), dim3(PREP_T), lds, (hipStream_t)stream, pj);
+    return made_check_launch("made_batch_prep");
+}
diff --git a/mgsv_amd/csrc/gemm_tn.hip b/mgsv_amd/csrc/gemm_tn.hip
--- a/mgsv_amd/csrc/gemm_tn.hip
+++ b/mgsv_amd/csrc/gemm_tn.hip
@@ -1,4 +1,5 @@
 #include "common.h"
+#include "batch_prep.h"
 
 namespace {
 
@@ -322,91 +323,14 @@
 
 namespace {
 __global__ __launch_bounds__(1024) void row_index_kernel(const float* mask, int64_t M, int32_t* row_index, int32_t* n_rows) {
-    constexpr int NB = 16;
     __shared__ int wsum[16];
     __shared__ int wlast[16];
-    const int lane = threadIdx.x & 63, wave = threadIdx.x >> 6;
-    const int64_t per = ((M + 15) / 16 + 63) / 64 * 64;
-    const int64_t b = (int64_t)wave * per, e = b + per < M ? b + per : M;
-    uint64_t bal[NB];
-    auto ballots = [&](int64_t i0) __attribute__((always_inline)) {
-        float v[NB];
-        const float* p = mask + i0 + lane;
-        if (i0 + NB * 64 <= e) {
-#pragma unroll
-            for (int j = 0; j < NB; ++j) v[j] = p[j * 64];
-        } else {
-#pragma unroll
-            for (int j = 0; j < NB; ++j) v[j] = i0 + j * 64 + lane < e ? p[j * 64] : 0.f;
-        }
-#pragma unroll
-        for (int j = 0; j < NB; ++j) bal[j] = __ballot(v[j] != 0.f);
-    };
-    int cnt = 0, last = -1;
-    for (int64_t i0 = b; i0 < e; i0 += NB * 64) {
-        ballots(i0);
-#pragma unroll
-        for (int j = 0; j < NB; ++j) {
-            cnt += __popcll(bal[j]);
-            if (bal[j]) last = (int)(i0 + j * 64) + 63 - __clzll(bal[j]);
-        }
-    }
-    if (lane == 0) { wsum[wave] = cnt; wlast[wave] = last; }
-    __syncthreads();
-    int base = 0, total = 0, lastv = 0;
-    for (int w = 0; w < 16; ++w) {
-        if (w < wave) base += wsum[w];
-        total += wsum[w];
-        if (wlast[w] >= 0) lastv = wlast[w];
-    }
-    for (int64_t i0 = b; i0 < e; i0 += NB * 64) {
-        ballots(i0);
-#pragma unroll
-        for (int j = 0; j < NB; ++j) {
-            if ((bal[j] >> lane) & 1ull) row_index[base + __popcll(bal[j] & ((1ull << lane) - 1ull))] = (int32_t)(i0 + j * 64 + lane);
-            base += __popcll(bal[j]);
-        }
-    }
-    if (threadIdx.x == 0) n_rows[0] = total;
-    for (int64_t i = total + threadIdx.x; i < M; i += 1024) row_index[i] = lastv;
+    made_prep::row_index_body(made_prep::PlainMask{mask, M}, M, row_index, n_rows, wsum, wlast);
 }
 
 __global__ __launch_bounds__(1024) void batch_order_kernel(const float* mask, int B, int64_t T, int32_t* order) {
     __shared__ int len[8192];
-    const int lane = threadIdx.x & 63, wave = threadIdx.x >> 6;
-    for (int b0 = wave; b0 < B; b0 += 64) {
-        int cnt[4] = {0, 0, 0, 0};
-        for (int64_t i0 = 0; i0 < T; i0 += 512) {
-            float v[4][8];
-#pragma unroll
-            for (int s4 = 0; s4 < 4; ++s4) {
-                const int b = b0 + 16 * s4;
-                const float* m = mask + (int64_t)(b < B ? b : B - 1) * T;
-#pragma unroll
-                for (int j = 0; j < 8; ++j) {
-                    const int64_t i = i0 + j * 64 + lane;
-                    v[s4][j] = i < T ? m[i] : 0.f;
-                }
-            }
-#pragma unroll
-            for (int s4 = 0; s4 < 4; ++s4)
-#pragma unroll
-                for (int j = 0; j < 8; ++j) cnt[s4] += __popcll(__ballot(v[s4][j] != 0.f));
-        }
-#pragma unroll
-        for (int s4 = 0; s4 < 4; ++s4)
-            if (lane == 0 && b0 + 16 * s4 < B) len[b0 + 16 * s4] = cnt[s4];
-    }
-    __syncthreads();
-    for (int b = threadIdx.x; b < B; b += 1024) {
-        const int mine = len[b];
-        int rank = 0;
-        for (int j = 0; j < B; ++j) {
-            const int l = len[j];
-            rank += (l > mine || (l == mine && j < b)) ? 1 : 0;
-        }
-        order[rank] = b;
-    }
+    made_prep::batch_order_body(made_prep::PlainMask{mask, T}, B, T, order, len);
 }
 }
 
diff --git a/mgsv_amd/csrc/optimizer.hip b/mgsv_amd/csrc/optimizer.hip
--- a/mgsv_amd/csrc/optimizer.hip
+++ b/mgsv_amd/csrc/optimizer.hip
@@ -10,6 +10,8 @@
     float beta1, beta2, eps, bc1, bc2_sqrt, grad_scale;
     float* norm_sq;
     const MadeAdamDeviceState* st;
+    unsigned* ticket;
+    MadeAdamDeviceState* st_rw; int advance;
 };
 
 __device__ __forceinline__ int group_of(const AdamArgs& a, int64_t i) {
@@ -20,38 +22,7 @@
     return gi;
 }
 
-__global__ __launch_bounds__(OT) void grad_norm_kernel(const AdamArgs a) {
-    __shared__ float red[MADE_ADAM_MAX_GROUPS][OT / 64];
-    float acc[MADE_ADAM_MAX_GROUPS];
-#pragma unroll
-    for (int k = 0; k < MADE_ADAM_MAX_GROUPS; ++k) acc[k] = 0.f;
-    for (int64_t i = ((int64_t)blockIdx.x * OT + threadIdx.x) * 4; i < a.n; i += (int64_t)gridDim.x * OT * 4) {
-        if (group_of(a, i) < 0 && group_of(a, i + 3) < 0) continue;
-        const f32x4 g4 = *(const f32x4*)(a.grad + i);
-#pragma unroll
-        for (int j = 0; j < 4; ++j) {
-            const int gi = group_of(a, i + j);
-            const float g = g4[j] * a.grad_scale;
-#pragma unroll
-            for (int k = 0; k < MADE_ADAM_MAX_GROUPS; ++k) acc[k] += (gi == k) ? g * g : 0.f;
-        }
-    }
-    const int lane = threadIdx.x & 63, wave = threadIdx.x >> 6;
-#pragma unroll
-    for (int k = 0; k < MADE_ADAM_MAX_GROUPS; ++k) {
-        const float s = wave_sum(acc[k]);
-        if (lane == 0) red[k][wave] = s;
-    }
-    __syncthreads();
-    if (threadIdx.x < MADE_ADAM_MAX_GROUPS) {
-        float s = 0.f;
-        for (int w = 0; w < OT / 64; ++w) s += red[threadIdx.x][w];
-        a.norm_sq[MADE_ADAM_MAX_GROUPS + (int64_t)blockIdx.x * MADE_ADAM_MAX_GROUPS + threadIdx.x] = s;
-    }
-}
-
-__global__ __launch_bounds__(OT) void norm_finish_kernel(float* norm_ws, int nblocks, MadeAdamDeviceState* st, float beta1, float beta2, int advance) {
-    __shared__ float red[OT];
+__device__ __forceinline__ void norm_finish(float* norm_ws, int nblocks, MadeAdamDeviceState* st, float beta1, float beta2, int advance, float* red) {
     if (st && advance && threadIdx.x == 0) {
         const int64_t step = ++st->step;
         st->bc1 = (float)(1.0 - pow((double)beta1, (double)step));
@@ -71,59 +42,127 @@
     }
 }
 
+__global__ __launch_bounds__(OT) void norm_finish_kernel(float* norm_ws, int nblocks, MadeAdamDeviceState* st, float beta1, float beta2, int advance) {
+    __shared__ float red[OT];
+    norm_finish(norm_ws, nblocks, st, beta1, beta2, advance, red);
+}
+
+__global__ __launch_bounds__(OT) void grad_norm_kernel(const AdamArgs a) {
+    __shared__ float red[MADE_ADAM_MAX_GROUPS][OT / 64];
+    __shared__ float fin[OT];
+    __shared__ unsigned s_ticket;
+    float acc[MADE_ADAM_MAX_GROUPS];
+#pragma unroll
+    for (int k = 0; k < MADE_ADAM_MAX_GROUPS; ++k) acc[k] = 0.f;
+    for (int64_t i = ((int64_t)blockIdx.x * OT + threadIdx.x) * 4; i < a.n; i += (int64_t)gridDim.x * OT * 4) {
+        if (group_of(a, i) < 0 && group_of(a, i + 3) < 0) continue;
+        const f32x4 g4 = *(const f32x4*)(a.grad + i);
+#pragma unroll
+        for (int j = 0; j < 4; ++j) {
+            const int gi = group_of(a, i + j);
+            const float g = g4[j] * a.grad_scale;
+#pragma unroll
+            for (int k = 0; k < MADE_ADAM_MAX_GROUPS; ++k) acc[k] += (gi == k) ? g * g : 0.f;
+        }
+    }
+    const int lane = threadIdx.x & 63, wave = threadIdx.x >> 6;
+#pragma unroll
+    for (int k = 0; k < MADE_ADAM_MAX_GROUPS; ++k) {
+        const float s = wave_sum(acc[k]);
+        if (lane == 0) red[k][wave] = s;
+    }
+    __syncthreads();
+    if (threadIdx.x < MADE_ADAM_MAX_GROUPS) {
+        float s = 0.f;
+        for (int w = 0; w < OT / 64; ++w) s += red[threadIdx.x][w];
+        a.norm_sq[MADE_ADAM_MAX_GROUPS + (int64_t)blockIdx.x * MADE_ADAM_MAX_GROUPS + threadIdx.x] = s;
+    }
+    if (!a.ticket) return;
+    if (wave == 0) {
+        __threadfence();
+        if (lane == 0) s_ticket = atomicAdd(a.ticket, 1u);
+    }
+    __syncthreads();
+    if (s_ticket != gridDim.x - 1) return;
+    __threadfence();
+    norm_finish(a.norm_sq, (int)gridDim.x, a.st_rw, a.beta1, a.beta2, a.advance, fin);
+    if (threadIdx.x == 0) atomicExch(a.ticket, 0u);
+}
+
+struct AdamCoef { float coef[MADE_ADAM_MAX_GROUPS], lr[MADE_ADAM_MAX_GROUPS]; float bc1, bc2_sqrt; };
+
+__device__ __forceinline__ AdamCoef adam_coefs(const AdamArgs& a) {
+    AdamCoef c;
+#pragma unroll
+    for (int k = 0; k < MADE_ADAM_MAX_GROUPS; ++k) {
+        c.coef[k] = 1.f;
+        if (k < a.n_groups && a.g[k].max_norm > 0.f) {
+            const float q = a.g[k].max_norm / (sqrtf(a.norm_sq[k]) + 1e-6f);
+            c.coef[k] = q < 1.f ? q : 1.f;
+        }
+    }
+#pragma unroll
+    for (int k = 0; k < MADE_ADAM_MAX_GROUPS; ++k) c.lr[k] = a.st ? a.st->lr[k] : a.g[k].lr;
+    c.bc1 = a.st ? a.st->bc1 : a.bc1;
+    c.bc2_sqrt = a.st ? a.st->bc2_sqrt : a.bc2_sqrt;
+    return c;
+}
+
+__device__ __forceinline__ void adam_update_one(const AdamArgs& a, const AdamCoef& c, int gi, float g_raw, float& m, float& v, float& p) {
+    if (gi < 0) return;
+    float cf = 1.f, lr = 0.f;
+#pragma unroll
+    for (int k = 0; k < MADE_ADAM_MAX_GROUPS; ++k)
+        if (gi == k) { cf = c.coef[k]; lr = c.lr[k]; }
+    const float g = g_raw * a.grad_scale * cf;
+    m = __builtin_fmaf(a.beta1, m, (1.f - a.beta1) * g);
+    v = __builtin_fmaf(a.beta2, v, ((1.f - a.beta2) * g) * g);
+    const float denom = sqrtf(v) / c.bc2_sqrt + a.eps;
+    p = __builtin_fmaf(-(lr / c.bc1), m / denom, p);
+}
+
 __global__ __launch_bounds__(OT) void adam_update_kernel(const AdamArgs a) {
-    float coef[MADE_ADAM_MAX_GROUPS];
-#pragma unroll
-    for (int k = 0; k < MADE_ADAM_MAX_GROUPS; ++k) {
-        coef[k] = 1.f;
-        if (k < a.n_groups && a.g[k].max_norm > 0.f) {
-            const float c = a.g[k].max_norm / (sqrtf(a.norm_sq[k]) + 1e-6f);
-            coef[k] = c < 1.f ? c : 1.f;
-        }
-    }
-    float lrs[MADE_ADAM_MAX_GROUPS];
-#pragma unroll
-    for (int k = 0; k < MADE_ADAM_MAX_GROUPS; ++k) lrs[k] = a.st ? a.st->lr[k] : a.g[k].lr;
-    const float bc1 = a.st ? a.st->bc1 : a.bc1, bc2_sqrt = a.st ? a.st->bc2_sqrt : a.bc2_sqrt;
+    const AdamCoef cf = adam_coefs(a);
     for (int64_t i = ((int64_t)blockIdx.x * OT + threadIdx.x) * 4; i < a.n; i += (int64_t)gridDim.x * OT * 4) {
         const int g0 = group_of(a, i), g3 = group_of(a, i + 3);
         if (g0 < 0 && g3 < 0) continue;
         f32x4 g4 = *(const f32x4*)(a.grad + i), m4 = *(const f32x4*)(a.m + i), v4 = *(const f32x4*)(a.v + i), p4 = *(const f32x4*)(a.param + i);
 #pragma unroll
         for (int j = 0; j < 4; ++j) {
-            const int gi = group_of(a, i + j);
-            if (gi < 0) continue;
-            float cf = 1.f, lr = 0.f;
-#pragma unroll
-            for (int k = 0; k < MADE_ADAM_MAX_GROUPS; ++k)
-                if (gi == k) { cf = coef[k]; lr = lrs[k]; }
-            const float g = g4[j] * a.grad_scale * cf;
-            m4[j] = a.beta1 * m4[j] + (1.f - a.beta1) * g;
-            v4[j] = a.beta2 * v4[j] + (1.f - a.beta2) * g * g;
-            const float denom = sqrtf(v4[j]) / bc2_sqrt + a.eps;
-            p4[j] -= (lr / bc1) * (m4[j] / denom);
+            float m = m4[j], v = v4[j], p = p4[j];
+            adam_update_one(a, cf, group_of(a, i + j), g4[j], m, v, p);
+            m4[j] = m; v4[j] = v; p4[j] = p;
         }
         *(f32x4*)(a.m + i) = m4; *(f32x4*)(a.v + i) = v4; *(f32x4*)(a.param + i) = p4;
     }
 }
 
 constexpr int RPT = 64;
-__global__ __launch_bounds__(OT) void repack_kernel(const MadeRepackDesc* descs, int n_desc) {
-    __shared__ float tile[RPT][RPT + 1];
-    __shared__ int s_desc;
-    const int64_t t = blockIdx.x;
+
+__device__ __forceinline__ int64_t unit_begin(const MadeRepackDesc& d) { return d.tile_begin; }
+__device__ __forceinline__ int64_t unit_begin(const MadeAdamVecDesc& d) { return d.chunk_begin; }
+template <typename D> __device__ __forceinline__ int find_desc(const D* descs, int n_desc, int64_t t, int* s_desc) {
     for (int i = threadIdx.x; i < n_desc; i += OT) {
-        const int64_t b = descs[i].tile_begin;
-        const int64_t e = i + 1 < n_desc ? descs[i + 1].tile_begin : INT64_MAX;
-        if (b <= t && t < e) s_desc = i;
+        const int64_t b = unit_begin(descs[i]);
+        const int64_t e = i + 1 < n_desc ? unit_begin(descs[i + 1]) : INT64_MAX;
+        if (b <= t && t < e) *s_desc = i;
     }
     __syncthreads();
-    const MadeRepackDesc d = descs[s_desc];
-    const int64_t local = t - d.tile_begin;
+    return *s_desc;
+}
+
+template <bool FUSED> __device__ __forceinline__ void repack_tile(const MadeRepackDesc& d, int64_t local, float (*tile)[RPT + 1],
+                                                                  const AdamArgs* a, const AdamCoef* cf) {
     const int64_t tc_n = (d.cols + RPT - 1) / RPT;
     const int64_t r0 = (local / tc_n) * RPT, c0 = (local % tc_n) * RPT;
     const int tx = threadIdx.x & 15, ty = threadIdx.x >> 4;
     const bool bf = d.dtype == MADE_BF16;
+    int64_t off0 = 0;
+    bool owned = false;
+    if (FUSED) {
+        off0 = d.src - a->param;
+        owned = off0 >= 0 && off0 + d.rows * d.cols <= a->n;
+    }
 #pragma unroll
     for (int k = 0; k < RPT / 16; ++k) {
         const int rr = ty + 16 * k;
@@ -131,7 +170,38 @@
         float v[4] = {0.f, 0.f, 0.f, 0.f};
         if (r < d.rows && c < d.cols) {
             const float* sp = d.src + r * d.cols + c;
-            if (c + 4 <= d.cols && (((uintptr_t)sp & 15) == 0)) {
+            const bool vec = c + 4 <= d.cols && (((uintptr_t)sp & 15) == 0);
+            if (FUSED && owned) {
+                const int64_t e = off0 + r * d.cols + c;
+                if (vec && ((e & 3) == 0)) {
+                    const int g0 = group_of(*a, e), g3 = group_of(*a, e + 3);
+                    f32x4 p4 = *(const f32x4*)(a->param + e);
+                    if (g0 >= 0 || g3 >= 0) {
+                        f32x4 g4 = *(const f32x4*)(a->grad + e), m4 = *(const f32x4*)(a->m + e), v4 = *(const f32x4*)(a->v + e);
+#pragma unroll
+                        for (int j = 0; j < 4; ++j) {
+                            float m_ = m4[j], v_ = v4[j], p_ = p4[j];
+                            adam_update_one(*a, *cf, group_of(*a, e + j), g4[j], m_, v_, p_);
+                            m4[j] = m_; v4[j] = v_; p4[j] = p_;
+                        }
+                        *(f32x4*)(a->m + e) = m4; *(f32x4*)(a->v + e) = v4; *(f32x4*)(a->param + e) = p4;
+                    }
+                    v[0] = p4[0]; v[1] = p4[1]; v[2] = p4[2]; v[3] = p4[3];
+                } else {
+#pragma unroll
+                    for (int j = 0; j < 4; ++j) {
+                        if (c + j >= d.cols) continue;
+                        float p_ = a->param[e + j];
+                        const int gi = group_of(*a, e + j);
+                        if (gi >= 0) {
+                            float m_ = a->m[e + j], v_ = a->v[e + j];
+                            adam_update_one(*a, *cf, gi, a->grad[e + j], m_, v_, p_);
+                            a->m[e + j] = m_; a->v[e + j] = v_; a->param[e + j] = p_;
+                        }
+                        v[j] = p_;
+                    }
+                }
+            } else if (vec) {
                 const f32x4 q = *(const f32x4*)sp;
                 v[0] = q[0]; v[1] = q[1]; v[2] = q[2]; v[3] = q[3];
             } else {
@@ -173,11 +243,70 @@
     }
 }
 
-}
+__global__ __launch_bounds__(OT) void repack_kernel(const MadeRepackDesc* descs, int n_desc) {
+    __shared__ float tile[RPT][RPT + 1];
+    __shared__ int s_desc;
+    const int64_t t = blockIdx.x;
+    const MadeRepackDesc d = descs[find_desc(descs, n_desc, t, &s_desc)];
+    repack_tile<false>(d, t - d.tile_begin, tile, nullptr, nullptr);
+}
+
+constexpr int VCH = OT * 4;
+struct FusedArgs {
+    AdamArgs a;
+    const MadeRepackDesc* descs; int n_desc; int64_t total_tiles;
+    const MadeAdamVecDesc* vecs; int n_vec;
+};
+
+__global__ __launch_bounds__(OT) void adam_repack_kernel(const FusedArgs f) {
+    __shared__ float tile[RPT][RPT + 1];
+    __shared__ int s_desc;
+    const AdamArgs& a = f.a;
+    const AdamCoef cf = adam_coefs(a);
+    const int64_t t = blockIdx.x;
+    if (t < f.total_tiles) {
+        const MadeRepackDesc d = f.descs[find_desc(f.descs, f.n_desc, t, &s_desc)];
+        repack_tile<true>(d, t - d.tile_begin, tile, &a, &cf);
+        return;
+    }
+    const int64_t ch = t - f.total_tiles;
+    const MadeAdamVecDesc d = f.vecs[find_desc(f.vecs, f.n_vec, ch, &s_desc)];
+    const int64_t begin = d.begin < 0 ? 0 : d.begin, end = d.end > a.n ? a.n : d.end;
+    const int64_t i = begin + (ch - d.chunk_begin) * VCH + threadIdx.x * 4;
+    if (i >= end) return;
+    if (i + 4 <= end && (i & 3) == 0) {
+        const int g0 = group_of(a, i), g3 = group_of(a, i + 3);
+        if (g0 < 0 && g3 < 0) return;
+        f32x4 g4 = *(const f32x4*)(a.grad + i), m4 = *(const f32x4*)(a.m + i), v4 = *(const f32x4*)(a.v + i), p4 = *(const f32x4*)(a.param + i);
+#pragma unroll
+        for (int j = 0; j < 4; ++j) {
+            float m = m4[j], v = v4[j], p = p4[j];
+            adam_update_one(a, cf, group_of(a, i + j), g4[j], m, v, p);
+            m4[j] = m; v4[j] = v; p4[j] = p;
+        }
+        *(f32x4*)(a.m + i) = m4; *(f32x4*)(a.v + i) = v4; *(f32x4*)(a.param + i) = p4;
+    } else {
+        for (int64_t e = i; e < i + 4 && e < end; ++e) {
+            const int gi = group_of(a, e);
+            if (gi < 0) continue;
+            float m = a.m[e], v = a.v[e], p = a.param[e];
+            adam_update_one(a, cf, gi, a.grad[e], m, v, p);
+            a.m[e] = m; a.v[e] = v; a.param[e] = p;
+        }
+    }
+}
+
+}
+
+struct FusedPlan {
+    const MadeRepackDesc* descs; int n_desc; int64_t total_tiles;
+    const MadeAdamVecDesc* vecs; int n_vec; int64_t total_chunks;
+    int fold_finish;
+};
 
 static int adam_launch(float* param, const float* grad, float* exp_avg, float* exp_avg_sq, int64_t n, const MadeAdamGroup* groups,
                        int32_t n_groups, float beta1, float beta2, float eps, int64_t step, MadeAdamDeviceState* state_device, int advance,
-                       float grad_scale, float* norm_ws, void* stream, const char* what) {
+                       float grad_scale, float* norm_ws, void* stream, const char* what, const FusedPlan* plan = nullptr) {
     AdamArgs a;
     a.param = param; a.grad = grad; a.m = exp_avg; a.v = exp_avg_sq; a.n = n; a.n_groups = n_groups;
     for (int k = 0; k < MADE_ADAM_MAX_GROUPS; ++k) {
@@ -189,12 +318,21 @@
     a.bc2_sqrt = state_device ? 1.f : (float)sqrt(1.0 - pow((double)beta2, (double)step));
     a.norm_sq = norm_ws;
     a.st = state_device;
+    const bool fold = plan && plan->fold_finish;
+    a.ticket = fold ? (unsigned*)(norm_ws + MADE_ADAM_MAX_GROUPS * (1 + MADE_ADAM_NORM_BLOCKS)) : nullptr;
+    a.st_rw = state_device; a.advance = advance;
     hipStream_t st = (hipStream_t)stream;
     int64_t nb = (n / 4 + OT - 1) / OT;
     if (nb > MADE_ADAM_NORM_BLOCKS) nb = MADE_ADAM_NORM_BLOCKS;
     hipLaunchKernelGGL(grad_norm_kernel, dim3((unsigned)nb), dim3(OT), 0, st, a);
-    hipLaunchKernelGGL(norm_finish_kernel, dim3(1), dim3(OT), 0, st, norm_ws, (int)nb, state_device, beta1, beta2, advance);
-    hipLaunchKernelGGL(adam_update_kernel, dim3((unsigned)nb), dim3(OT), 0, st, a);
+    if (!fold) hipLaunchKernelGGL(norm_finish_kernel, dim3(1), dim3(OT), 0, st, norm_ws, (int)nb, state_device, beta1, beta2, advance);
+    if (!plan) {
+        hipLaunchKernelGGL(adam_update_kernel, dim3((unsigned)nb), dim3(OT), 0, st, a);
+    } else if (plan->total_tiles + plan->total_chunks > 0) {
+        FusedArgs f;
+        f.a = a; f.descs = plan->descs; f.n_desc = plan->n_desc; f.total_tiles = plan->total_tiles; f.vecs = plan->vecs; f.n_vec = plan->n_vec;
+        hipLaunchKernelGGL(adam_repack_kernel, dim3((unsigned)(plan->total_tiles + plan->total_chunks)), dim3(OT), 0, st, f);
+    }
     return made_check_launch(what);
 }
 
@@ -218,6 +356,23 @@
                        "made_adam_step_device");
 }
 
+extern "C" int made_adam_repack_step(float* param, const float* grad, float* exp_avg, float* exp_avg_sq, int64_t n,
+                                     const MadeAdamGroup* groups, int32_t n_groups, float beta1, float beta2, float eps, int64_t step,
+                                     MadeAdamDeviceState* state_device, int32_t advance_state, float grad_scale, float* norm_ws,
+                                     const MadeRepackDesc* descs_device, int32_t n_desc, int64_t total_tiles,
+                                     const MadeAdamVecDesc* vecs_device, int32_t n_vec, int64_t total_chunks, int32_t fold_finish, void* stream) {
+    MADE_REQUIRE(param && grad && exp_avg && exp_avg_sq && groups && norm_ws, "made_adam_repack_step: null pointer");
+    MADE_REQUIRE(n_groups >= 1 && n_groups <= MADE_ADAM_MAX_GROUPS, "made_adam_repack_step: n_groups=%d out of range", n_groups);
+    MADE_REQUIRE(n > 0 && n % 4 == 0 && (state_device || step >= 1), "made_adam_repack_step: n must be a positive multiple of 4 and step >= 1");
+    MADE_REQUIRE(n_desc >= 0 && n_vec >= 0 && total_tiles >= 0 && total_chunks >= 0 && (n_desc == 0) == (total_tiles == 0) &&
+                 (n_vec == 0) == (total_chunks == 0) && (n_desc == 0 || descs_device) && (n_vec == 0 || vecs_device),
+                 "made_adam_repack_step: descriptor tables and unit counts do not agree");
+    MADE_UNSUPPORTED(total_tiles + total_chunks < (1LL << 31), "made_adam_repack_step: too many workgroups");
+    FusedPlan plan = {descs_device, (int)n_desc, total_tiles, vecs_device, (int)n_vec, total_chunks, fold_finish != 0};
+    return adam_launch(param, grad, exp_avg, exp_avg_sq, n, groups, n_groups, beta1, beta2, eps, state_device ? 0 : step, state_device,
+                       state_device ? advance_state != 0 : 0, grad_scale, norm_ws, stream, "made_adam_repack_step", &plan);
+}
+
 extern "C" int made_repack(const MadeRepackDesc* descs_device, int32_t n_desc, int64_t total_tiles, void* stream) {
     MADE_REQUIRE(descs_device != nullptr && n_desc >= 1 && total_tiles >= 1, "made_repack: bad arguments");
     MADE_UNSUPPORTED(total_tiles < (1LL << 31), "made_repack: too many tiles");
diff --git a/mgsv_amd/ops.py b/mgsv_amd/ops.py
--- a/mgsv_amd/ops.py
+++ b/mgsv_amd/ops.py
@@ -245,6 +245,27 @@
     return out
 
 
+def batch_prep(jobs) -> None:
+    arr = (_lib.MadeBatchPrepJob * len(jobs))()
+    for j, (kind, masks, out, *rest) in zip(arr, jobs):
+        m1, m2 = masks if isinstance(masks, (tuple, list)) else (None, masks)
+        assert m2.dim() == 2 and m2.is_contiguous() and (m1 is None or (m1.dim() == 2 and m1.is_contiguous() and m1.shape[0] == m2.shape[0]))
+        B, T1 = m2.shape[0], (m1.shape[1] if m1 is not None else 0)
+        j.mask1, j.mask2 = (_p(_f32(m1, "mask")) if m1 is not None else None), _p(_f32(m2, "mask"))
+        j.B, j.T1, j.T = B, T1, T1 + m2.shape[1]
+        if kind == "rows":
+            idx, n = out
+            assert idx.dtype == torch.int32 and idx.numel() >= B * j.T and n.dtype == torch.int32
+            j.kind, j.out, j.out2 = _lib.PREP_ROWS, _p(idx), _p(n)
+        elif kind == "order":
+            assert out.dtype == torch.int32 and out.numel() == B
+            j.kind, j.out = _lib.PREP_ORDER, _p(out)
+        else:
+            assert kind == "plan" and out.dtype == torch.int32 and out.is_contiguous()
+            j.kind, j.out, j.out_words, j.n_slots, j.max_slices = _lib.PREP_PLAN, _p(out), out.numel(), rest[0], rest[1]
+    check(lib().made_batch_prep(arr, len(jobs), _stream()), "made_batch_prep")
+
+
 def linear_splitk(A: Tensor, W: Tensor, bias: Optional[Tensor], ws: Tensor, split_k: int, *, A2: Optional[Tensor] = None,
                   a2_row_mod: int = 0, act: int = ACT_NONE, R: Optional[Tensor] = None, r_row_mod: int = 0,
                   out: Optional[Tensor] = None, ln1=None, ln1_out: Optional[Tensor] = None, ln2=None,
diff --git a/mgsv_amd/trainer.py b/mgsv_amd/trainer.py
--- a/mgsv_amd/trainer.py
+++ b/mgsv_amd/trainer.py
@@ -19,6 +19,34 @@
 
 
 HEAD_PAD = 64
+
+
+ADAM_CHUNK = 1024
+
+
+def adam_vec_ranges(mats: List[Tuple[int, int]], lo: int, hi: int) -> List[Tuple[int, int, int]]:
+    out: List[Tuple[int, int, int]] = []
+    chunks = 0
+
+    def add(b, e):
+        nonlocal chunks
+        if e <= b:
+            return
+        a4 = min(e, -(-b // 4) * 4)
+        for bb, ee in ((b, a4), (a4, e)):
+            if ee > bb:
+                out.append((bb, ee, chunks))
+                chunks += -(-(ee - bb) // ADAM_CHUNK)
+    pos = lo
+    for off, cnt in sorted(mats):
+        if off + cnt <= lo or off >= hi:
+            continue
+        if off < pos or off + cnt > hi:
+            raise ValueError(f"adam_vec_ranges: matrix [{off}, {off + cnt}) overlaps a neighbour or straddles [{lo}, {hi})")
+        add(pos, off)
+        pos = off + cnt
+    add(pos, hi)
+    return out
 
 
 class MadeTrainer(MadeEngine):
@@ -212,7 +240,7 @@
         self.exp_avg = torch.zeros_like(self.flat_param)
         self.exp_avg_sq = torch.zeros_like(self.flat_param)
         self.opt_step = 0
-        self._norm_ws = torch.zeros(2 * 4 * (1 + 1024), device=dev, dtype=torch.float32)
+        self._norm_ws = torch.zeros(2 * _lib.ADAM_WS_FLOATS, device=dev, dtype=torch.float32)
 
     def _view(self, store: Dict[str, Tensor], ref) -> Tensor:
         if isinstance(ref, tuple):
@@ -223,7 +251,7 @@
             return flat[o:o + a.numel() + b.numel()].view((rows,) + tuple(a.shape[1:]))
         return store[ref]
 
-    def repack(self, part: Optional[str] = None):
+    def repack(self, part: Optional[str] = None, only=False):
         import ctypes as C
         if getattr(self, "_pack_desc", None) is None:
             P, tc, dev = self.P, self.tc, self.device
@@ -277,7 +305,21 @@
                 return torch.from_numpy(np.frombuffer(bytes(arr), dtype=np.uint8).copy()).to(dev), len(out), t0
             self._pack_desc = {None: pack(descs), "early": pack([d for d, q in zip(descs, part_of) if q == "early"]),
                                "rest": pack([d for d, q in zip(descs, part_of) if q == "rest"])}
-        pk = self._pack_desc[part]
+            base, n = self.flat_param.data_ptr(), self.flat_param.numel()
+            self._fused_plan = {}
+            for prt, lo, hi in ((None, 0, n), ("early", cut, n), ("rest", 0, cut)):
+                seen, first, again = set(), [], []
+                for d, q in zip(descs, part_of):
+                    if prt is not None and q != prt:
+                        continue
+                    (again if d.src in seen else first).append(d)
+                    seen.add(d.src)
+                vr = adam_vec_ranges([((d.src - base) // 4, d.rows * d.cols) for d in first], lo, hi)
+                varr = (_lib.MadeAdamVecDesc * max(len(vr), 1))(*[_lib.MadeAdamVecDesc(*r) for r in vr])
+                vt = torch.from_numpy(np.frombuffer(bytes(varr), dtype=np.uint8).copy()).to(dev)
+                vchunks = (vr[-1][2] + -(-(vr[-1][1] - vr[-1][0]) // ADAM_CHUNK)) if vr else 0
+                self._fused_plan[prt] = (pack(first), (vt, len(vr), vchunks), pack(again))
+        pk = self._pack_desc[part] if only is False else only
         if pk is not None:
             _lib.check(_lib.lib().made_repack(pk[0].data_ptr(), pk[1], pk[2], torch.cuda.current_stream().cuda_stream), "made_repack")
         if self.cfg.agg_module == "mlp" and part != "early":
@@ -305,6 +347,17 @@
                 groups[i].end = groups[i].begin
             groups[i].lr, groups[i].max_norm = float(lr), float(max_grad_norm)
         ws = self._norm_ws[:self._norm_ws.numel() // 2] if part != "early" else self._norm_ws[self._norm_ws.numel() // 2:]
+        if _lib.variant_env("MADE_ADAM_FUSED", "1") != "0":
+            tiles, (vt, n_vec, vchunks), again = self._fused_plan[part]
+            fold = 1 if _lib.variant_env("MADE_NORM_FOLD", "1") != "0" else 0
+            _lib.check(_lib.lib().made_adam_repack_step(
+                self.flat_param.data_ptr(), self.flat_grad.data_ptr(), self.exp_avg.data_ptr(), self.exp_avg_sq.data_ptr(),
+                self.flat_param.numel(), groups, 3, float(betas[0]), float(betas[1]), float(eps), self.opt_step,
+                device_state.data_ptr() if device_state is not None else None, 0 if part == "rest" else 1, float(grad_scale), ws.data_ptr(),
+                tiles[0].data_ptr() if tiles else None, tiles[1] if tiles else 0, tiles[2] if tiles else 0,
+                vt.data_ptr() if n_vec else None, n_vec, vchunks, fold, torch.cuda.current_stream().cuda_stream), "made_adam_repack_step")
+            self.repack(part, only=again)
+            return
         if device_state is not None:
             _lib.check(_lib.lib().made_adam_step_device(self.flat_param.data_ptr(), self.flat_grad.data_ptr(), self.exp_avg.data_ptr(),
                                                         self.exp_avg_sq.data_ptr(), self.flat_param.numel(), groups, 3, float(betas[0]),
@@ -521,18 +574,31 @@
         fus, fus_mask = ws["fus"], ws["fus_mask"]
         self._groups = {}
         cur, side = torch.cuda.current_stream(), self._side_stream()
-        side.wait_stream(cur)
-        self._rows = {sm.data_ptr(): ops.row_index(sm, out=tw["rows_a"])}
-        self._order = {sm.data_ptr(): ops.batch_order(sm, out=tw["order_a"])}
+        plan_ok = "regression" not in c.mml_localization and self._wide_planned_ok(B, H * Q, D)
+        if _lib.variant_env("MADE_BATCH_PREP", "1") != "0":
+            fus_src = (fm, sm) if concat else sm
+            jobs = [("rows", sm, tw["rows_a"]), ("order", sm, tw["order_a"]), ("rows", fm, tw["rows_v"]), ("order", fm, tw["order_v"]),
+                    ("rows", fus_src, tw["rows_f"]), ("order", fus_src, tw["order_f"])]
+            if plan_ok:
+                jobs.append(("plan", fus_src, tw["wide_plan"], self._wide_slots(), WIDE_SLICES))
+            ops.batch_prep(jobs)
+            side.wait_stream(cur)
+            self._rows = {sm.data_ptr(): tw["rows_a"], fm.data_ptr(): tw["rows_v"], fus_mask.data_ptr(): tw["rows_f"]}
+            self._order = {sm.data_ptr(): tw["order_a"], fm.data_ptr(): tw["order_v"], fus_mask.data_ptr(): tw["order_f"]}
+            self._wide_plan = ops.WidePlan(tw["wide_plan"], B, fus_mask.shape[1], self._wide_slots(), WIDE_SLICES) if plan_ok else None
+        else:
+            side.wait_stream(cur)
+            self._rows = {sm.data_ptr(): ops.row_index(sm, out=tw["rows_a"])}
+            self._order = {sm.data_ptr(): ops.batch_order(sm, out=tw["order_a"])}
         with torch.cuda.stream(side):
             ops.concat_cols(fm if concat else None, sm, fus_mask)
-            self._rows[fm.data_ptr()] = ops.row_index(fm, out=tw["rows_v"])
-            self._order[fm.data_ptr()] = ops.batch_order(fm, out=tw["order_v"])
-            self._rows[fus_mask.data_ptr()] = ops.row_index(fus_mask, out=tw["rows_f"])
-            self._order[fus_mask.data_ptr()] = ops.batch_order(fus_mask, out=tw["order_f"])
-            self._wide_plan = (ops.wide_slice_plan(fus_mask, n_slots=self._wide_slots(), max_slices=WIDE_SLICES,
-                                                   order=self._order[fus_mask.data_ptr()], out=tw["wide_plan"])
-                               if "regression" not in c.mml_localization and self._wide_planned_ok(B, H * Q, D) else None)
+            if _lib.variant_env("MADE_BATCH_PREP", "1") == "0":
+                self._rows[fm.data_ptr()] = ops.row_index(fm, out=tw["rows_v"])
+                self._order[fm.data_ptr()] = ops.batch_order(fm, out=tw["order_v"])
+                self._rows[fus_mask.data_ptr()] = ops.row_index(fus_mask, out=tw["rows_f"])
+                self._order[fus_mask.data_ptr()] = ops.batch_order(fus_mask, out=tw["order_f"])
+                self._wide_plan = (ops.wide_slice_plan(fus_mask, n_slots=self._wide_slots(), max_slices=WIDE_SLICES,
+                                                       order=self._order[fus_mask.data_ptr()], out=tw["wide_plan"]) if plan_ok else None)
             pos = ops.sine_pe(fus_mask, P["dim_t"], out=ws["pos"])
             self._encode_train(self._inputs[0], fm, "video", ws, tw, 0)
         self._encode_train(self._inputs[1], sm, "audio", ws, tw, Tv)
@@ -1131,7 +1197,8 @@
                 tr.l2norm_bwd(ws["pv_raw"], tw["dvid_sum"], dx_alt=tw["dpv_raw"], dy_rows_per=Tv)
                 heads_dw.append(lambda: tr.gemm_tn(tw["dpv_raw"][:Tv], frame[0], G["proj_v.w"], accumulate=True, colsum=G["proj_v.b"], batch=(B, 1),
                                                    a_zs=(Tv * Dc, 0), b_zs=(frame.stride(0), 0), colsum_zs=(0, 0)))
-                ops.linear(tw["dpv_raw"], P["proj_v.wt"], None, out=tw["dframe_x"])
+                if _lib.variant_env("MADE_PROJV_DX_LATE", "1") == "0":
+                    ops.linear(tw["dpv_raw"], P["proj_v.wt"], None, out=tw["dframe_x"])
 
             qp = P["query_embed"]
             mem3, mempos3 = tw["mem"].view(B, L, D), tw["mempos"].view(B, L, D)
@@ -1446,6 +1513,8 @@
         side.wait_stream(cur)
         with torch.cuda.stream(side):
             dxv = tw["dframe_x"] if (c.contrastive_align_loss and not regression) else None
+            if dxv is not None and _lib.variant_env("MADE_PROJV_DX_LATE", "1") != "0":
+                ops.linear(tw["dpv_raw"], P["proj_v.wt"], None, out=dxv)
             if "video" in c.vmr_fusion:
                 dxv = tw["ydseg"] if dxv is None else tr.add3(tw["dframe_sum"], dxv, tw["ydseg"])
             self._encode_bwd("video", ws, tw, dl_v, dxv.view(B, Tv, D) if dxv is not None else None, dvideo, fm, feats_v)
```

Result: no change. 14040 pairs/s (-0.6%).
